# SzymonKnopp/morfem

Hardware: NVIDIA B200
Metric: reduced-sweep freq points/sec (higher is better)
Workload: dtype c128

## Files before the change

### include/morfem_b200.h

```cpp
#ifndef MORFEM_B200_H
#define MORFEM_B200_H

#include <stddef.h>
#include <stdint.h>

#ifdef __cplusplus
extern "C" {
#endif

typedef struct { double re, im; } mf_c128;

#define MF_VERSION 100
#define MF_MAX_PORTS 16

int mf_version(void);
const char* mf_last_error(void);
int64_t mf_launch_count(void);

size_t mf_gemm_tn_ws_bytes(int ra, int rb, int64_t n);
int mf_gemm_tn_c128(const mf_c128* A, int64_t lda, int ra, const mf_c128* B, int64_t ldb, int rb, int64_t n,
                    int conj_a, mf_c128* C, int64_t ldc, void* ws, size_t ws_bytes, void* stream);

int mf_gemm_nn_c128(const mf_c128* A, int64_t lda, int64_t n, int ra, const mf_c128* W, int64_t ldw, int rb,
                    mf_c128* Out, int64_t ldo, void* stream);
int mf_trmm_nn_c128(const mf_c128* A, int64_t lda, int64_t n, int r, const mf_c128* W, int64_t ldw,
                    mf_c128* Out, int64_t ldo, void* stream);

int mf_equilibrate_c128(mf_c128* G, int64_t ld, int r, double shift, double* d, double* stats, void* stream);
int mf_potrf_upper_c128(mf_c128* G, int64_t ld, int r, int* info, void* stream);
int mf_trtri_upper_c128(const mf_c128* R, int64_t ldr, int r, mf_c128* Rinv, int64_t ldi, void* stream);
size_t mf_chol_inv_ws_bytes(int r);
int mf_chol_inv_upper_c128(mf_c128* G, int64_t ldg, int r, mf_c128* Rinv, int64_t ldi, int* info,
                           void* ws, size_t ws_bytes, void* stream);
int mf_scale_cols_c128(mf_c128* X, int64_t ld, int rows, int cols, const double* d, int power, void* stream);
int mf_scale_rows_c128(mf_c128* X, int64_t ld, int rows, int cols, const double* d, int power, void* stream);
size_t mf_jacobi_svd_ws_bytes(int r);
int mf_jacobi_svd_c128(mf_c128* X, int64_t ld, int r, mf_c128* U, int64_t ldu, double* sigma, int max_sweeps,
                       double tol, int* sweeps_done, void* ws, size_t ws_bytes, void* stream);

int mf_spmm_csr_c128(const int32_t* rowptr, const int32_t* colidx, const void* vals, int val_is_real,
                     int64_t nrows, const mf_c128* Q, int64_t ldq, int r, mf_c128* Y, int64_t ldy, void* stream);
int mf_spmm_csr2_c128(const int32_t* rowptr, const int32_t* colidx, const void* vals0, const void* vals1, int val_is_real,
                      int64_t nrows, const mf_c128* Q, int64_t ldq, int r, mf_c128* Y0, int64_t ldy0, mf_c128* Y1, int64_t ldy1,
                      void* stream);
int mf_spmm_csr2_f64(const int32_t* rowptr, const int32_t* colidx, const double* vals0, const double* vals1, int64_t nrows,
                     const double* Q, int64_t ldq, int r, double* Y0, int64_t ldy0, double* Y1, int64_t ldy1, void* stream);

int mf_spmm_group_size(int r);
int mf_spmm_group_size_f64(int r);
int mf_spmm_group_count(const int32_t* rowptr, const int32_t* colidx, int64_t nrows, int G, int32_t* counts, void* stream);
int mf_spmm_group_fill(const int32_t* rowptr, const int32_t* colidx, const double* vals, int64_t nrows, int G,
                       const int64_t* ustart, int32_t* ucols, double* uvals, void* stream);
int mf_spmm_grouped_c128(const int64_t* ustart, const int32_t* ucols, const double* uvals, int64_t nrows, int G,
                         const mf_c128* Q, int64_t ldq, int r, mf_c128* Y, int64_t ldy, void* stream);

int mf_spmm_window_rows_per_block(void);
int mf_spmm_window_max_nnz_per_row(void);
int mf_spmm_window_max_rows(void);
int mf_spmm_window_c128(const int32_t* rowptr, const uint8_t* slot, const double* vals, const int32_t* wstart, const int32_t* ucol,
                        int64_t nrows, int wmax, const mf_c128* Q, int64_t ldq, int r, mf_c128* Y, int64_t ldy, void* stream);
int mf_spmm_window_f64(const int32_t* rowptr, const uint8_t* slot, const double* vals, const int32_t* wstart, const int32_t* ucol,
                       int64_t nrows, int wmax, const double* Q, int64_t ldq, int r, double* Y, int64_t ldy, void* stream);

int mf_project_rhs_c128(const int32_t* colptr, const int32_t* rowidx, const void* vals, int val_is_real, int m,
                        const mf_c128* Q, int64_t ldq, int r, int64_t row0, int64_t nlocal, int conj_q,
                        mf_c128* Br, int64_t ldb, void* stream);

size_t mf_gemm_tn_f64_ws_bytes(int ra, int rb, int64_t n);
int mf_gemm_tn_f64(const double* A, int64_t lda, int ra, const double* B, int64_t ldb, int rb, int64_t n,
                   double* C, int64_t ldc, void* ws, size_t ws_bytes, void* stream);
int mf_gemm_nn_f64(const double* A, int64_t lda, int64_t n, int ra, const double* W, int64_t ldw, int rb,
                   double* Out, int64_t ldo, void* stream);
int mf_trmm_nn_f64(const double* A, int64_t lda, int64_t n, int r, const double* W, int64_t ldw,
                   double* Out, int64_t ldo, void* stream);
int mf_spmm_csr_f64(const int32_t* rowptr, const int32_t* colidx, const double* vals, int64_t nrows,
                    const double* Q, int64_t ldq, int r, double* Y, int64_t ldy, void* stream);
int mf_spmm_grouped_f64(const int64_t* ustart, const int32_t* ucols, const double* uvals, int64_t nrows, int G,
                        const double* Q, int64_t ldq, int r, double* Y, int64_t ldy, void* stream);
int mf_sweep_f64_supported(int r, int m);
int mf_sweep_f64_variant_supported(int r, int m, int variant);
size_t mf_sweep_f64_ws_bytes(int r, int m, int64_t F, int variant);
int mf_sweep_lu_gsm_f64(const double* A0, const double* A1, const double* A2, int64_t lda, const double* Br, int64_t ldb, int r, int m,
                        const double* c0, const double* c1, const double* c2, const double* cb, const double* zscale, int64_t F,
                        double* X, mf_c128* S, int* info, int variant, void* ws, size_t ws_bytes, void* stream);
int mf_jacobi_svd_f64_supported(int r);
int mf_jacobi_svd_f64(const double* X, int64_t ld, int r, double* U, int64_t ldu, double* sigma, int max_sweeps,
                      double tol, int* sweeps_done, void* stream);
int mf_project_rhs_f64(const int32_t* colptr, const int32_t* rowidx, const double* vals, int m,
                       const double* Q, int64_t ldq, int r, int64_t row0, int64_t nlocal, double* Br, int64_t ldb, void* stream);

int mf_symmetrize_c128(const mf_c128* A, int64_t lda, int r, mf_c128* As, int64_t lds, void* stream);

size_t mf_sweep_ws_bytes(int r, int m, int64_t F, int variant);
int mf_sweep_variant_supported(int r, int m, int variant);
int mf_sweep_lu_gsm_c128(const mf_c128* A0, const mf_c128* A1, const mf_c128* A2, int64_t lda,
                         const mf_c128* Br, int64_t ldb, int r, int m,
                         const double* c0, const double* c1, const double* c2, const double* cb,
                         const double* zscale, int64_t F,
                         mf_c128* X, mf_c128* S, int* info, int variant,
                         void* ws, size_t ws_bytes, void* stream);

int mf_gsm_c128(const mf_c128* X, const mf_c128* Bmat, int64_t ldb, int r, int m, const double* cb,
                const double* zscale, int64_t F, mf_c128* S, void* stream);

int mf_estimator_c128(const mf_c128* X, int r, int m, int64_t F, const mf_c128* const* G_host,
                      const mf_c128* const* H_host, const mf_c128* BB,
                      const double* c0, const double* c1, const double* c2, const double* cb,
                      double* err, void* stream);

int mf_peak_dmma_tflops(int iters, double* tflops_host, void* stream);

#ifdef __cplusplus
}
#endif
#endif
```

### morfem_b200/_ffi.py

```python
from __future__ import annotations

import ctypes
import os
from ctypes import c_char_p, c_double, c_int, c_int64, c_size_t, c_void_p

_HERE = os.path.dirname(os.path.abspath(__file__))
LIB_PATH = os.path.join(_HERE, "libmorfem_b200.so")


class MorfemB200Error(RuntimeError):
    """A C-ABI call returned a non-zero status."""


SIGNATURES = {
    "mf_version": (c_int, []),
    "mf_last_error": (c_char_p, []),
    "mf_launch_count": (c_int64, []),
    "mf_gemm_tn_ws_bytes": (c_size_t, [c_int, c_int, c_int64]),
    "mf_gemm_tn_c128": (c_int, [c_void_p, c_int64, c_int, c_void_p, c_int64, c_int, c_int64, c_int, c_void_p, c_int64,
                                c_void_p, c_size_t, c_void_p]),
    "mf_gemm_nn_c128": (c_int, [c_void_p, c_int64, c_int64, c_int, c_void_p, c_int64, c_int, c_void_p, c_int64, c_void_p]),
    "mf_trmm_nn_c128": (c_int, [c_void_p, c_int64, c_int64, c_int, c_void_p, c_int64, c_void_p, c_int64, c_void_p]),
    "mf_trmm_nn_f64": (c_int, [c_void_p, c_int64, c_int64, c_int, c_void_p, c_int64, c_void_p, c_int64, c_void_p]),
    "mf_equilibrate_c128": (c_int, [c_void_p, c_int64, c_int, c_double, c_void_p, c_void_p, c_void_p]),
    "mf_potrf_upper_c128": (c_int, [c_void_p, c_int64, c_int, c_void_p, c_void_p]),
    "mf_trtri_upper_c128": (c_int, [c_void_p, c_int64, c_int, c_void_p, c_int64, c_void_p]),
    "mf_chol_inv_ws_bytes": (c_size_t, [c_int]),
    "mf_chol_inv_upper_c128": (c_int, [c_void_p, c_int64, c_int, c_void_p, c_int64, c_void_p, c_void_p, c_size_t, c_void_p]),
    "mf_scale_cols_c128": (c_int, [c_void_p, c_int64, c_int, c_int, c_void_p, c_int, c_void_p]),
    "mf_scale_rows_c128": (c_int, [c_void_p, c_int64, c_int, c_int, c_void_p, c_int, c_void_p]),
    "mf_jacobi_svd_ws_bytes": (c_size_t, [c_int]),
    "mf_jacobi_svd_c128": (c_int, [c_void_p, c_int64, c_int, c_void_p, c_int64, c_void_p, c_int, c_double, c_void_p,
                                   c_void_p, c_size_t, c_void_p]),
    "mf_spmm_csr_c128": (c_int, [c_void_p, c_void_p, c_void_p, c_int, c_int64, c_void_p, c_int64, c_int, c_void_p, c_int64,
                                 c_void_p]),
    "mf_spmm_csr2_c128": (c_int, [c_void_p, c_void_p, c_void_p, c_void_p, c_int, c_int64, c_void_p, c_int64, c_int, c_void_p, c_int64,
                                  c_void_p, c_int64, c_void_p]),
    "mf_spmm_csr2_f64": (c_int, [c_void_p, c_void_p, c_void_p, c_void_p, c_int64, c_void_p, c_int64, c_int, c_void_p, c_int64,
                                 c_void_p, c_int64, c_void_p]),
    "mf_spmm_group_size": (c_int, [c_int]),
    "mf_spmm_group_size_f64": (c_int, [c_int]),
    "mf_spmm_group_count": (c_int, [c_void_p, c_void_p, c_int64, c_int, c_void_p, c_void_p]),
    "mf_spmm_group_fill": (c_int, [c_void_p, c_void_p, c_void_p, c_int64, c_int, c_void_p, c_void_p, c_void_p, c_void_p]),
    "mf_spmm_grouped_c128": (c_int, [c_void_p, c_void_p, c_void_p, c_int64, c_int, c_void_p, c_int64, c_int, c_void_p, c_int64,
                                     c_void_p]),
    "mf_spmm_window_rows_per_block": (c_int, []),
    "mf_spmm_window_max_nnz_per_row": (c_int, []),
    "mf_spmm_window_max_rows": (c_int, []),
    "mf_spmm_window_c128": (c_int, [c_void_p, c_void_p, c_void_p, c_void_p, c_void_p, c_int64, c_int, c_void_p, c_int64, c_int, c_void_p, c_int64,
                                    c_void_p]),
    "mf_spmm_window_f64": (c_int, [c_void_p, c_void_p, c_void_p, c_void_p, c_void_p, c_int64, c_int, c_void_p, c_int64, c_int, c_void_p, c_int64,
                                   c_void_p]),
    "mf_project_rhs_c128": (c_int, [c_void_p, c_void_p, c_void_p, c_int, c_int, c_void_p, c_int64, c_int, c_int64, c_int64,
                                    c_int, c_void_p, c_int64, c_void_p]),
    "mf_gemm_tn_f64_ws_bytes": (c_size_t, [c_int, c_int, c_int64]),
    "mf_gemm_tn_f64": (c_int, [c_void_p, c_int64, c_int, c_void_p, c_int64, c_int, c_int64, c_void_p, c_int64, c_void_p, c_size_t, c_void_p]),
    "mf_gemm_nn_f64": (c_int, [c_void_p, c_int64, c_int64, c_int, c_void_p, c_int64, c_int, c_void_p, c_int64, c_void_p]),
    "mf_spmm_csr_f64": (c_int, [c_void_p, c_void_p, c_void_p, c_int64, c_void_p, c_int64, c_int, c_void_p, c_int64, c_void_p]),
    "mf_spmm_grouped_f64": (c_int, [c_void_p, c_void_p, c_void_p, c_int64, c_int, c_void_p, c_int64, c_int, c_void_p, c_int64, c_void_p]),
    "mf_sweep_f64_supported": (c_int, [c_int, c_int]),
    "mf_sweep_f64_variant_supported": (c_int, [c_int, c_int, c_int]),
    "mf_sweep_f64_ws_bytes": (c_size_t, [c_int, c_int, c_int64, c_int]),
    "mf_sweep_lu_gsm_f64": (c_int, [c_void_p, c_void_p, c_void_p, c_int64, c_void_p, c_int64, c_int, c_int,
                                    c_void_p, c_void_p, c_void_p, c_void_p, c_void_p, c_int64, c_void_p, c_void_p, c_void_p,
                                    c_int, c_void_p, c_size_t, c_void_p]),
    "mf_jacobi_svd_f64_supported": (c_int, [c_int]),
    "mf_jacobi_svd_f64": (c_int, [c_void_p, c_int64, c_int, c_void_p, c_int64, c_void_p, c_int, c_double, c_void_p, c_void_p]),
    "mf_project_rhs_f64": (c_int, [c_void_p, c_void_p, c_void_p, c_int, c_void_p, c_int64, c_int, c_int64, c_int64, c_void_p, c_int64,
                                   c_void_p]),
    "mf_symmetrize_c128": (c_int, [c_void_p, c_int64, c_int, c_void_p, c_int64, c_void_p]),
    "mf_sweep_ws_bytes": (c_size_t, [c_int, c_int, c_int64, c_int]),
    "mf_sweep_variant_supported": (c_int, [c_int, c_int, c_int]),
    "mf_sweep_lu_gsm_c128": (c_int, [c_void_p, c_void_p, c_void_p, c_int64, c_void_p, c_int64, c_int, c_int,
                                     c_void_p, c_void_p, c_void_p, c_void_p, c_void_p, c_int64,
                                     c_void_p, c_void_p, c_void_p, c_int, c_void_p, c_size_t, c_void_p]),
    "mf_gsm_c128": (c_int, [c_void_p, c_void_p, c_int64, c_int, c_int, c_void_p, c_void_p, c_int64, c_void_p, c_void_p]),
    "mf_peak_dmma_tflops": (c_int, [c_int, c_void_p, c_void_p]),
    "mf_estimator_c128": (c_int, [c_void_p, c_int, c_int, c_int64, c_void_p, c_void_p, c_void_p, c_void_p,
                                  c_void_p, c_void_p, c_void_p, c_void_p, c_void_p]),
}

_lib = None


def load() -> ctypes.CDLL:
    global _lib
    if _lib is not None:
        return _lib
    if not os.path.exists(LIB_PATH):
        raise MorfemB200Error(
            f"{LIB_PATH} not found: build it with `python -c 'import __graft_entry__ as g; g.build()'` "
            "(or `make -C morfem_b200/csrc`).  morfem_b200 has no CPU fallback.")
    lib = ctypes.CDLL(LIB_PATH)
    for name, (restype, argtypes) in SIGNATURES.items():
        fn = getattr(lib, name)
        fn.restype = restype
        fn.argtypes = argtypes
    _lib = lib
    return lib


def check(status: int, what: str = "") -> None:
    if status != 0:
        msg = load().mf_last_error()
        raise MorfemB200Error(f"{what or 'morfem_b200 call'} failed with status {status}: "
                              f"{msg.decode(errors='replace') if msg else ''}")


def launch_count() -> int:
    return int(load().mf_launch_count())
```

### morfem_b200/csrc/dense_gemm.cu

```cuda
#include "common.cuh"

namespace {

constexpr int KC = 16;
constexpr int STAGES = 3;

constexpr int TN_TI = 64, TN_TJ = 64, TN_THREADS = 128;
constexpr int TN_LDA = TN_TI + 2, TN_LDB = TN_TJ + 2;
constexpr int TN_STAGE_ELEMS = KC * (TN_LDA + TN_LDB);

__global__ void __launch_bounds__(TN_THREADS, 2)
gemm_tn_kernel(const cplx* __restrict__ A, long long lda, int ra, const cplx* __restrict__ B, long long ldb, int rb,
               long long n, long long rows_per_split, int conj_a, cplx* __restrict__ part, int herm) {
    extern __shared__ __align__(16) cplx smem[];
    const int tid = threadIdx.x, lane = tid & 31, warp = tid >> 5;
    const int g = lane >> 2, t = lane & 3;
    const int wi = warp >> 1, wj = warp & 1;
    const int ntj = (rb + TN_TJ - 1) / TN_TJ;
    const int ti = blockIdx.x / ntj, tj = blockIdx.x - ti * ntj;
    if (herm && ti > tj) return;
    const int i0 = ti * TN_TI, j0 = tj * TN_TJ;
    const long long n0 = (long long)blockIdx.y * rows_per_split;
    long long n1 = n0 + rows_per_split; if (n1 > n) n1 = n;
    const int nchunks = n1 > n0 ? (int)((n1 - n0 + KC - 1) / KC) : 0;

    auto load_stage = [&](int stage, int chunk) {
        cplx* As = smem + stage * TN_STAGE_ELEMS;
        cplx* Bs = As + KC * TN_LDA;
        const long long row_base = n0 + (long long)chunk * KC;
#pragma unroll
        for (int q = 0; q < (KC * TN_TI) / TN_THREADS; ++q) {
            int idx = tid + q * TN_THREADS;
            int rr = idx / TN_TI, cc = idx - rr * TN_TI;
            long long row = row_base + rr;
            bool ok = row < n1 && (i0 + cc) < ra;
            const cplx* src = A + (ok ? row * lda + i0 + cc : 0);
            cp_async16(As + rr * TN_LDA + cc, src, ok);
        }
#pragma unroll
        for (int q = 0; q < (KC * TN_TJ) / TN_THREADS; ++q) {
            int idx = tid + q * TN_THREADS;
            int rr = idx / TN_TJ, cc = idx - rr * TN_TJ;
            long long row = row_base + rr;
            bool ok = row < n1 && (j0 + cc) < rb;
            const cplx* src = B + (ok ? row * ldb + j0 + cc : 0);
            cp_async16(Bs + rr * TN_LDB + cc, src, ok);
        }
    };

    double cre[4][4][2], cim[4][4][2];
#pragma unroll
    for (int i = 0; i < 4; ++i)
#pragma unroll
        for (int j = 0; j < 4; ++j) { cre[i][j][0] = cre[i][j][1] = 0.0; cim[i][j][0] = cim[i][j][1] = 0.0; }

    for (int s = 0; s < STAGES - 1; ++s) { if (s < nchunks) load_stage(s, s); cp_async_commit(); }
    const double sgn = conj_a ? -1.0 : 1.0;
    for (int c = 0; c < nchunks; ++c) {
        cp_async_wait<STAGES - 2>();
        __syncthreads();
        { int nc = c + STAGES - 1; if (nc < nchunks) load_stage(nc % STAGES, nc); cp_async_commit(); }
        const cplx* As = smem + (c % STAGES) * TN_STAGE_ELEMS;
        const cplx* Bs = As + KC * TN_LDA;
#pragma unroll
        for (int kk = 0; kk < KC / 4; ++kk) {
            cplx a[4], b[4];
#pragma unroll
            for (int i = 0; i < 4; ++i) { a[i] = As[(kk * 4 + t) * TN_LDA + wi * 32 + i * 8 + g]; a[i].y *= sgn; }
#pragma unroll
            for (int j = 0; j < 4; ++j) b[j] = Bs[(kk * 4 + t) * TN_LDB + wj * 32 + j * 8 + g];
#pragma unroll
            for (int i = 0; i < 4; ++i)
#pragma unroll
                for (int j = 0; j < 4; ++j) {
                    dmma884(cre[i][j][0], cre[i][j][1], a[i].x, b[j].x);
                    dmma884(cre[i][j][0], cre[i][j][1], -a[i].y, b[j].y);
                    dmma884(cim[i][j][0], cim[i][j][1], a[i].x, b[j].y);
                    dmma884(cim[i][j][0], cim[i][j][1], a[i].y, b[j].x);
                }
        }
    }
    cp_async_wait<0>();
    cplx* out = part + (long long)blockIdx.y * ra * rb;
#pragma unroll
    for (int i = 0; i < 4; ++i)
#pragma unroll
        for (int j = 0; j < 4; ++j) {
            int row = i0 + wi * 32 + i * 8 + g;
            int col = j0 + wj * 32 + j * 8 + 2 * t;
            if (row < ra) {
                if (col < rb) out[(long long)row * rb + col] = cmake(cre[i][j][0], cim[i][j][0]);
                if (col + 1 < rb) out[(long long)row * rb + col + 1] = cmake(cre[i][j][1], cim[i][j][1]);
            }
        }
}

constexpr int RED_WARPS = 8;
__global__ void __launch_bounds__(RED_WARPS * 32)
reduce_partials_kernel(const cplx* __restrict__ part, int nsplit, int ra, int rb, cplx* __restrict__ C, long long ldc, int herm) {
    __shared__ cplx red[RED_WARPS][32];
    const int lane = threadIdx.x & 31, warp = threadIdx.x >> 5;
    const long long total = (long long)ra * rb;
    const long long oidx = (long long)blockIdx.x * 32 + lane;
    long long idx = oidx;
    bool mirror = false;
    if (herm && oidx < total) {
        const int i = (int)(oidx / rb), j = (int)(oidx - (long long)i * rb);
        if (i / TN_TI > j / TN_TJ) { idx = (long long)j * rb + i; mirror = true; }
    }
    cplx acc0 = cmake(0.0, 0.0), acc1 = cmake(0.0, 0.0);
    if (idx < total) {
        int s = warp;
        for (; s + RED_WARPS < nsplit; s += 2 * RED_WARPS) {
            const cplx v0 = part[(long long)s * total + idx], v1 = part[(long long)(s + RED_WARPS) * total + idx];
            acc0 = cadd(acc0, v0); acc1 = cadd(acc1, v1);
        }
        if (s < nsplit) acc0 = cadd(acc0, part[(long long)s * total + idx]);
    }
    red[warp][lane] = cadd(acc0, acc1);
    __syncthreads();
    if (warp == 0 && oidx < total) {
        cplx acc = red[0][lane];
#pragma unroll
        for (int w = 1; w < RED_WARPS; ++w) acc = cadd(acc, red[w][lane]);
        if (mirror) acc.y = -acc.y;
        const int i = (int)(oidx / rb), j = (int)(oidx - (long long)i * rb);
        C[i * ldc + j] = acc;
    }
}

void tn_plan(int ra, int rb, long long n, int& tiles, int& nsplit, long long& rows_per_split, bool symm = false) {
    tiles = ((ra + TN_TI - 1) / TN_TI) * ((rb + TN_TJ - 1) / TN_TJ);
    const int nt = (ra + TN_TI - 1) / TN_TI;
    const int work_tiles = symm ? nt * (nt + 1) / 2 : tiles;
    const int target = 148 * 2 * 2;
    long long max_split = (n + (long long)KC * 8 - 1) / ((long long)KC * 8);
    if (max_split < 1) max_split = 1;
    long long s = target / work_tiles; if (s < 1) s = 1; if (s > max_split) s = max_split;
    rows_per_split = (n + s - 1) / s;
    rows_per_split = (rows_per_split + KC - 1) / KC * KC;
    if (rows_per_split < KC) rows_per_split = KC;
    nsplit = (int)((n + rows_per_split - 1) / rows_per_split); if (nsplit < 1) nsplit = 1;
}

constexpr int NN_TM = 128, NN_TN = 64, NN_THREADS = 256;
constexpr int NN_LDA = KC + 4;
constexpr int NN_LDW = NN_TN + 2;
constexpr int NN_STAGE_ELEMS = NN_TM * NN_LDA + KC * NN_LDW;

__global__ void __launch_bounds__(NN_THREADS, 1)
gemm_nn_kernel(const cplx* __restrict__ A, long long lda, long long n, int ra, const cplx* __restrict__ W, long long ldw, int rb,
               cplx* __restrict__ Out, long long ldo, int w_upper) {
    extern __shared__ __align__(16) cplx smem[];
    const int tid = threadIdx.x, lane = tid & 31, warp = tid >> 5;
    const int g = lane >> 2, t = lane & 3;
    const int wm = warp >> 1, wn = warp & 1;
    const int ntn = (rb + NN_TN - 1) / NN_TN;
    const long long tm = blockIdx.x / ntn; const int tn = (int)(blockIdx.x - tm * ntn);
    const long long m0 = tm * NN_TM; const int j0 = tn * NN_TN;
    const int kmax = (w_upper && j0 + NN_TN < ra) ? j0 + NN_TN : ra;
    const int nchunks = (kmax + KC - 1) / KC;

    auto load_stage = [&](int stage, int chunk) {
        cplx* As = smem + stage * NN_STAGE_ELEMS;
        cplx* Ws = As + NN_TM * NN_LDA;
        const int k0 = chunk * KC;
#pragma unroll
        for (int q = 0; q < (NN_TM * KC) / NN_THREADS; ++q) {
            int idx = tid + q * NN_THREADS;
            int rr = idx / KC, cc = idx - rr * KC;
            bool ok = (m0 + rr) < n && (k0 + cc) < ra;
            const cplx* src = A + (ok ? (m0 + rr) * lda + k0 + cc : 0);
            cp_async16(As + rr * NN_LDA + cc, src, ok);
        }
#pragma unroll
        for (int q = 0; q < (KC * NN_TN) / NN_THREADS; ++q) {
            int idx = tid + q * NN_THREADS;
            int rr = idx / NN_TN, cc = idx - rr * NN_TN;
            bool ok = (k0 + rr) < ra && (j0 + cc) < rb;
            const cplx* src = W + (ok ? (long long)(k0 + rr) * ldw + j0 + cc : 0);
            cp_async16(Ws + rr * NN_LDW + cc, src, ok);
        }
    };

    double cre[4][4][2], cim[4][4][2];
#pragma unroll
    for (int i = 0; i < 4; ++i)
#pragma unroll
        for (int j = 0; j < 4; ++j) { cre[i][j][0] = cre[i][j][1] = 0.0; cim[i][j][0] = cim[i][j][1] = 0.0; }

    for (int s = 0; s < STAGES - 1; ++s) { if (s < nchunks) load_stage(s, s); cp_async_commit(); }
    for (int c = 0; c < nchunks; ++c) {
        cp_async_wait<STAGES - 2>();
        __syncthreads();
        { int nc = c + STAGES - 1; if (nc < nchunks) load_stage(nc % STAGES, nc); cp_async_commit(); }
        const cplx* As = smem + (c % STAGES) * NN_STAGE_ELEMS;
        const cplx* Ws = As + NN_TM * NN_LDA;
#pragma unroll
        for (int kk = 0; kk < KC / 4; ++kk) {
            cplx a[4], b[4];
#pragma unroll
            for (int i = 0; i < 4; ++i) a[i] = As[(wm * 32 + i * 8 + g) * NN_LDA + kk * 4 + t];
#pragma unroll
            for (int j = 0; j < 4; ++j) b[j] = Ws[(kk * 4 + t) * NN_LDW + wn * 32 + j * 8 + g];
#pragma unroll
            for (int i = 0; i < 4; ++i)
#pragma unroll
                for (int j = 0; j < 4; ++j) {
                    dmma884(cre[i][j][0], cre[i][j][1], a[i].x, b[j].x);
                    dmma884(cre[i][j][0], cre[i][j][1], -a[i].y, b[j].y);
                    dmma884(cim[i][j][0], cim[i][j][1], a[i].x, b[j].y);
                    dmma884(cim[i][j][0], cim[i][j][1], a[i].y, b[j].x);
                }
        }
    }
    cp_async_wait<0>();
#pragma unroll
    for (int i = 0; i < 4; ++i)
#pragma unroll
        for (int j = 0; j < 4; ++j) {
            long long row = m0 + wm * 32 + i * 8 + g;
            int col = j0 + wn * 32 + j * 8 + 2 * t;
            if (row < n) {
                if (col + 1 < rb) {
                    double4 v = make_double4(cre[i][j][0], cim[i][j][0], cre[i][j][1], cim[i][j][1]);
                    cplx* dst = Out + row * ldo + col;
                    if ((reinterpret_cast<uintptr_t>(dst) & 31) == 0) *reinterpret_cast<double4*>(dst) = v;
                    else { dst[0] = cmake(v.x, v.y); dst[1] = cmake(v.z, v.w); }
                } else if (col < rb) {
                    Out[row * ldo + col] = cmake(cre[i][j][0], cim[i][j][0]);
                }
            }
        }
}

}

extern "C" size_t mf_gemm_tn_ws_bytes(int ra, int rb, int64_t n) {
    if (ra <= 0 || rb <= 0 || n <= 0) return 16;
    int tiles, nsplit, nsplit2 = 0; long long rps;
    tn_plan(ra, rb, n, tiles, nsplit, rps);
    if (ra == rb) tn_plan(ra, rb, n, tiles, nsplit2, rps, true);
    return sizeof(cplx) * (size_t)(nsplit > nsplit2 ? nsplit : nsplit2) * ra * rb;
}

extern "C" int mf_gemm_tn_c128(const mf_c128* A, int64_t lda, int ra, const mf_c128* B, int64_t ldb, int rb, int64_t n,
                               int conj_a, mf_c128* C, int64_t ldc, void* ws, size_t ws_bytes, void* stream) {
    if (!A) MF_FAIL_ARG(1, "A is NULL");
    if (ra <= 0 || lda < ra) MF_FAIL_ARG(3, "need 0 < ra <= lda");
    if (!B) MF_FAIL_ARG(4, "B is NULL");
    if (rb <= 0 || ldb < rb) MF_FAIL_ARG(6, "need 0 < rb <= ldb");
    if (n < 0) MF_FAIL_ARG(7, "n < 0");
    if (!C || ldc < rb) MF_FAIL_ARG(9, "C is NULL or ldc < rb");
    if (!ws || ws_bytes < mf_gemm_tn_ws_bytes(ra, rb, n)) MF_FAIL_ARG(11, "workspace too small (mf_gemm_tn_ws_bytes)");
    cudaStream_t st = (cudaStream_t)stream;
    int tiles, nsplit; long long rps;
    const int herm = (conj_a && (const void*)A == (const void*)B && lda == ldb && ra == rb) ? 1 : 0;
    tn_plan(ra, rb, n > 0 ? n : 1, tiles, nsplit, rps, herm != 0);
    const size_t smem = sizeof(cplx) * STAGES * TN_STAGE_ELEMS;
    MF_CHECK_CUDA(cudaFuncSetAttribute(gemm_tn_kernel, cudaFuncAttributeMaxDynamicSharedMemorySize, (int)smem));
    dim3 grid(tiles, nsplit);
    gemm_tn_kernel<<<grid, TN_THREADS, smem, st>>>((const cplx*)A, lda, ra, (const cplx*)B, ldb, rb, n, rps, conj_a, (cplx*)ws, herm);
    MF_CHECK_LAUNCH();
    long long total = (long long)ra * rb;
    reduce_partials_kernel<<<(unsigned)((total + 31) / 32), RED_WARPS * 32, 0, st>>>((const cplx*)ws, nsplit, ra, rb, (cplx*)C, ldc, herm);
    MF_CHECK_LAUNCH();
    return 0;
}

static int gemm_nn_c128_impl(const mf_c128* A, int64_t lda, int64_t n, int ra, const mf_c128* W, int64_t ldw, int rb,
                            mf_c128* Out, int64_t ldo, void* stream, int w_upper) {
    if (!A) MF_FAIL_ARG(1, "A is NULL");
    if (ra <= 0 || lda < ra) MF_FAIL_ARG(4, "need 0 < ra <= lda");
    if (n < 0) MF_FAIL_ARG(3, "n < 0");
    if (!W || ldw < rb) MF_FAIL_ARG(5, "W is NULL or ldw < rb");
    if (rb <= 0) MF_FAIL_ARG(7, "rb <= 0");
    if (!Out || ldo < rb) MF_FAIL_ARG(8, "Out is NULL or ldo < rb");
    if ((const void*)Out == (const void*)A) MF_FAIL_ARG(8, "Out must not alias A");
    if (n == 0) return 0;
    cudaStream_t st = (cudaStream_t)stream;
    const size_t smem = sizeof(cplx) * STAGES * NN_STAGE_ELEMS;
    MF_CHECK_CUDA(cudaFuncSetAttribute(gemm_nn_kernel, cudaFuncAttributeMaxDynamicSharedMemorySize, (int)smem));
    long long tiles_m = (n + NN_TM - 1) / NN_TM;
    int tiles_n = (rb + NN_TN - 1) / NN_TN;
    long long grid = tiles_m * tiles_n;
    if (grid > 0x7fffffffLL) MF_FAIL_ARG(3, "n too large for one launch");
    gemm_nn_kernel<<<(unsigned)grid, NN_THREADS, smem, st>>>((const cplx*)A, lda, n, ra, (const cplx*)W, ldw, rb, (cplx*)Out, ldo, w_upper);
    MF_CHECK_LAUNCH();
    return 0;
}

extern "C" int mf_gemm_nn_c128(const mf_c128* A, int64_t lda, int64_t n, int ra, const mf_c128* W, int64_t ldw, int rb,
                               mf_c128* Out, int64_t ldo, void* stream) {
    return gemm_nn_c128_impl(A, lda, n, ra, W, ldw, rb, Out, ldo, stream, 0);
}

extern "C" int mf_trmm_nn_c128(const mf_c128* A, int64_t lda, int64_t n, int r, const mf_c128* W, int64_t ldw,
                               mf_c128* Out, int64_t ldo, void* stream) {
    return gemm_nn_c128_impl(A, lda, n, r, W, ldw, r, Out, ldo, stream, 1);
}
```

### morfem_b200/csrc/dense_gemm_f64.cu

```cuda
#include "common.cuh"

namespace {

constexpr int KC = 16;
constexpr int STAGES = 3;

constexpr int TN_TI = 64, TN_TJ = 64, TN_THREADS = 128;
constexpr int TN_LDA = TN_TI + 8, TN_LDB = TN_TJ + 8;
constexpr int TN_STAGE_ELEMS = KC * (TN_LDA + TN_LDB);

__device__ __forceinline__ void cp_async8(void* smem_dst, const void* gmem_src, bool valid) {
    unsigned s = (unsigned)__cvta_generic_to_shared(smem_dst);
    int bytes = valid ? 8 : 0;
    asm volatile("cp.async.ca.shared.global [%0], [%1], 8, %2;\n" :: "r"(s), "l"(gmem_src), "r"(bytes));
}

__global__ void __launch_bounds__(TN_THREADS, 2)
gemm_tn_f64_kernel(const double* __restrict__ A, long long lda, int ra, const double* __restrict__ B, long long ldb, int rb,
                   long long n, long long rows_per_split, double* __restrict__ part, int vec_ok, int symm) {
    extern __shared__ __align__(16) double smem_d[];
    const int tid = threadIdx.x, lane = tid & 31, warp = tid >> 5;
    const int g = lane >> 2, t = lane & 3;
    const int wi = warp >> 1, wj = warp & 1;
    const int ntj = (rb + TN_TJ - 1) / TN_TJ;
    const int ti = blockIdx.x / ntj, tj = blockIdx.x - ti * ntj;
    if (symm && ti > tj) return;
    const int i0 = ti * TN_TI, j0 = tj * TN_TJ;
    const long long n0 = (long long)blockIdx.y * rows_per_split;
    long long n1 = n0 + rows_per_split; if (n1 > n) n1 = n;
    const int nchunks = n1 > n0 ? (int)((n1 - n0 + KC - 1) / KC) : 0;

    auto load_stage = [&](int stage, int chunk) {
        double* As = smem_d + stage * TN_STAGE_ELEMS;
        double* Bs = As + KC * TN_LDA;
        const long long row_base = n0 + (long long)chunk * KC;
        if (vec_ok) {
#pragma unroll
            for (int q = 0; q < (KC * TN_TI / 2) / TN_THREADS; ++q) {
                const int idx = tid + q * TN_THREADS;
                const int rr = idx / (TN_TI / 2), cc = 2 * (idx - rr * (TN_TI / 2));
                const long long row = row_base + rr;
                const bool ok = row < n1 && (i0 + cc) < ra;
                cp_async16(As + rr * TN_LDA + cc, A + (ok ? row * lda + i0 + cc : 0), ok);
            }
#pragma unroll
            for (int q = 0; q < (KC * TN_TJ / 2) / TN_THREADS; ++q) {
                const int idx = tid + q * TN_THREADS;
                const int rr = idx / (TN_TJ / 2), cc = 2 * (idx - rr * (TN_TJ / 2));
                const long long row = row_base + rr;
                const bool ok = row < n1 && (j0 + cc) < rb;
                cp_async16(Bs + rr * TN_LDB + cc, B + (ok ? row * ldb + j0 + cc : 0), ok);
            }
        } else {
#pragma unroll
            for (int q = 0; q < (KC * TN_TI) / TN_THREADS; ++q) {
                const int idx = tid + q * TN_THREADS;
                const int rr = idx / TN_TI, cc = idx - rr * TN_TI;
                const long long row = row_base + rr;
                const bool ok = row < n1 && (i0 + cc) < ra;
                cp_async8(As + rr * TN_LDA + cc, A + (ok ? row * lda + i0 + cc : 0), ok);
            }
#pragma unroll
            for (int q = 0; q < (KC * TN_TJ) / TN_THREADS; ++q) {
                const int idx = tid + q * TN_THREADS;
                const int rr = idx / TN_TJ, cc = idx - rr * TN_TJ;
                const long long row = row_base + rr;
                const bool ok = row < n1 && (j0 + cc) < rb;
                cp_async8(Bs + rr * TN_LDB + cc, B + (ok ? row * ldb + j0 + cc : 0), ok);
            }
        }
    };

    double c[4][4][2];
#pragma unroll
    for (int i = 0; i < 4; ++i)
#pragma unroll
        for (int j = 0; j < 4; ++j) { c[i][j][0] = 0.0; c[i][j][1] = 0.0; }

    for (int s = 0; s < STAGES - 1; ++s) { if (s < nchunks) load_stage(s, s); cp_async_commit(); }
    for (int ch = 0; ch < nchunks; ++ch) {
        cp_async_wait<STAGES - 2>();
        __syncthreads();
        { const int nc = ch + STAGES - 1; if (nc < nchunks) load_stage(nc % STAGES, nc); cp_async_commit(); }
        const double* As = smem_d + (ch % STAGES) * TN_STAGE_ELEMS;
        const double* Bs = As + KC * TN_LDA;
#pragma unroll
        for (int kk = 0; kk < KC / 4; ++kk) {
            double a[4], b[4];
#pragma unroll
            for (int i = 0; i < 4; ++i) a[i] = As[(kk * 4 + t) * TN_LDA + wi * 32 + i * 8 + g];
#pragma unroll
            for (int j = 0; j < 4; ++j) b[j] = Bs[(kk * 4 + t) * TN_LDB + wj * 32 + j * 8 + g];
#pragma unroll
            for (int i = 0; i < 4; ++i)
#pragma unroll
                for (int j = 0; j < 4; ++j) dmma884(c[i][j][0], c[i][j][1], a[i], b[j]);
        }
    }
    cp_async_wait<0>();
    double* out = part + (long long)blockIdx.y * ra * rb;
#pragma unroll
    for (int i = 0; i < 4; ++i)
#pragma unroll
        for (int j = 0; j < 4; ++j) {
            const int row = i0 + wi * 32 + i * 8 + g;
            const int col = j0 + wj * 32 + j * 8 + 2 * t;
            if (row < ra) {
                if (col < rb) out[(long long)row * rb + col] = c[i][j][0];
                if (col + 1 < rb) out[(long long)row * rb + col + 1] = c[i][j][1];
            }
        }
}

constexpr int RED_WARPS = 8;
__global__ void __launch_bounds__(RED_WARPS * 32)
reduce_partials_f64_kernel(const double* __restrict__ part, int nsplit, int ra, int rb, double* __restrict__ C, long long ldc, int symm) {
    __shared__ double red[RED_WARPS][32];
    const int lane = threadIdx.x & 31, warp = threadIdx.x >> 5;
    const long long total = (long long)ra * rb;
    const long long oidx = (long long)blockIdx.x * 32 + lane;
    long long idx = oidx;
    if (symm && oidx < total) {
        const int i = (int)(oidx / rb), j = (int)(oidx - (long long)i * rb);
        if (i / TN_TI > j / TN_TJ) idx = (long long)j * rb + i;
    }
    double acc0 = 0.0, acc1 = 0.0;
    if (idx < total) {
        int s = warp;
        for (; s + RED_WARPS < nsplit; s += 2 * RED_WARPS) { acc0 += part[(long long)s * total + idx]; acc1 += part[(long long)(s + RED_WARPS) * total + idx]; }
        if (s < nsplit) acc0 += part[(long long)s * total + idx];
    }
    red[warp][lane] = acc0 + acc1;
    __syncthreads();
    if (warp == 0 && oidx < total) {
        double acc = red[0][lane];
#pragma unroll
        for (int w = 1; w < RED_WARPS; ++w) acc += red[w][lane];
        const int i = (int)(oidx / rb), j = (int)(oidx - (long long)i * rb);
        C[i * ldc + j] = acc;
    }
}

void tn_plan(int ra, int rb, long long n, int& tiles, int& nsplit, long long& rows_per_split, bool symm = false) {
    tiles = ((ra + TN_TI - 1) / TN_TI) * ((rb + TN_TJ - 1) / TN_TJ);
    const int nt = (ra + TN_TI - 1) / TN_TI;
    const int work_tiles = symm ? nt * (nt + 1) / 2 : tiles;
    const int target = 148 * 2 * 2;
    long long max_split = (n + (long long)KC * 8 - 1) / ((long long)KC * 8);
    if (max_split < 1) max_split = 1;
    long long s = target / work_tiles; if (s < 1) s = 1; if (s > max_split) s = max_split;
    rows_per_split = (n + s - 1) / s;
    rows_per_split = (rows_per_split + KC - 1) / KC * KC;
    if (rows_per_split < KC) rows_per_split = KC;
    nsplit = (int)((n + rows_per_split - 1) / rows_per_split); if (nsplit < 1) nsplit = 1;
}

constexpr int NN_TM = 128, NN_TN = 64, NN_THREADS = 256;
constexpr int NN_LDA = KC + 4;
constexpr int NN_LDW = NN_TN + 8;
constexpr int NN_STAGE_ELEMS = NN_TM * NN_LDA + KC * NN_LDW;

__global__ void __launch_bounds__(NN_THREADS, 2)
gemm_nn_f64_kernel(const double* __restrict__ A, long long lda, long long n, int ra, const double* __restrict__ W, long long ldw, int rb,
                   double* __restrict__ Out, long long ldo, int w_upper) {
    extern __shared__ __align__(16) double smem_d[];
    const int tid = threadIdx.x, lane = tid & 31, warp = tid >> 5;
    const int g = lane >> 2, t = lane & 3;
    const int wm = warp >> 1, wn = warp & 1;
    const int ntn = (rb + NN_TN - 1) / NN_TN;
    const long long tm = blockIdx.x / ntn; const int tn = (int)(blockIdx.x - tm * ntn);
    const long long m0 = tm * NN_TM; const int j0 = tn * NN_TN;
    const int kmax = (w_upper && j0 + NN_TN < ra) ? j0 + NN_TN : ra;
    const int nchunks = (kmax + KC - 1) / KC;

    auto load_stage = [&](int stage, int chunk) {
        double* As = smem_d + stage * NN_STAGE_ELEMS;
        double* Ws = As + NN_TM * NN_LDA;
        const int k0 = chunk * KC;
#pragma unroll
        for (int q = 0; q < (NN_TM * KC) / NN_THREADS; ++q) {
            const int idx = tid + q * NN_THREADS;
            const int rr = idx / KC, cc = idx - rr * KC;
            const bool ok = (m0 + rr) < n && (k0 + cc) < ra;
            cp_async8(As + rr * NN_LDA + cc, A + (ok ? (m0 + rr) * lda + k0 + cc : 0), ok);
        }
#pragma unroll
        for (int q = 0; q < (KC * NN_TN) / NN_THREADS; ++q) {
            const int idx = tid + q * NN_THREADS;
            const int rr = idx / NN_TN, cc = idx - rr * NN_TN;
            const bool ok = (k0 + rr) < ra && (j0 + cc) < rb;
            cp_async8(Ws + rr * NN_LDW + cc, W + (ok ? (long long)(k0 + rr) * ldw + j0 + cc : 0), ok);
        }
    };

    double c[4][4][2];
#pragma unroll
    for (int i = 0; i < 4; ++i)
#pragma unroll
        for (int j = 0; j < 4; ++j) { c[i][j][0] = 0.0; c[i][j][1] = 0.0; }

    for (int s = 0; s < STAGES - 1; ++s) { if (s < nchunks) load_stage(s, s); cp_async_commit(); }
    for (int ch = 0; ch < nchunks; ++ch) {
        cp_async_wait<STAGES - 2>();
        __syncthreads();
        { const int nc = ch + STAGES - 1; if (nc < nchunks) load_stage(nc % STAGES, nc); cp_async_commit(); }
        const double* As = smem_d + (ch % STAGES) * NN_STAGE_ELEMS;
        const double* Ws = As + NN_TM * NN_LDA;
#pragma unroll
        for (int kk = 0; kk < KC / 4; ++kk) {
            double a[4], b[4];
#pragma unroll
            for (int i = 0; i < 4; ++i) a[i] = As[(wm * 32 + i * 8 + g) * NN_LDA + kk * 4 + t];
#pragma unroll
            for (int j = 0; j < 4; ++j) b[j] = Ws[(kk * 4 + t) * NN_LDW + wn * 32 + j * 8 + g];
#pragma unroll
            for (int i = 0; i < 4; ++i)
#pragma unroll
                for (int j = 0; j < 4; ++j) dmma884(c[i][j][0], c[i][j][1], a[i], b[j]);
        }
    }
    cp_async_wait<0>();
#pragma unroll
    for (int i = 0; i < 4; ++i)
#pragma unroll
        for (int j = 0; j < 4; ++j) {
            const long long row = m0 + wm * 32 + i * 8 + g;
            const int col = j0 + wn * 32 + j * 8 + 2 * t;
            if (row < n) {
                double* dst = Out + row * ldo + col;
                if (col + 1 < rb && (reinterpret_cast<uintptr_t>(dst) & 15) == 0) *reinterpret_cast<double2*>(dst) = make_double2(c[i][j][0], c[i][j][1]);
                else { if (col < rb) dst[0] = c[i][j][0]; if (col + 1 < rb) dst[1] = c[i][j][1]; }
            }
        }
}

}

extern "C" size_t mf_gemm_tn_f64_ws_bytes(int ra, int rb, int64_t n) {
    if (ra <= 0 || rb <= 0 || n <= 0) return 16;
    int tiles, nsplit, nsplit2 = 0; long long rps;
    tn_plan(ra, rb, n, tiles, nsplit, rps);
    if (ra == rb) tn_plan(ra, rb, n, tiles, nsplit2, rps, true);
    return sizeof(double) * (size_t)(nsplit > nsplit2 ? nsplit : nsplit2) * ra * rb;
}

extern "C" int mf_gemm_tn_f64(const double* A, int64_t lda, int ra, const double* B, int64_t ldb, int rb, int64_t n,
                              double* C, int64_t ldc, void* ws, size_t ws_bytes, void* stream) {
    if (!A) MF_FAIL_ARG(1, "A is NULL");
    if (ra <= 0 || lda < ra) MF_FAIL_ARG(3, "need 0 < ra <= lda");
    if (!B) MF_FAIL_ARG(4, "B is NULL");
    if (rb <= 0 || ldb < rb) MF_FAIL_ARG(6, "need 0 < rb <= ldb");
    if (n < 0) MF_FAIL_ARG(7, "n < 0");
    if (!C || ldc < rb) MF_FAIL_ARG(8, "C is NULL or ldc < rb");
    if (!ws || ws_bytes < mf_gemm_tn_f64_ws_bytes(ra, rb, n)) MF_FAIL_ARG(10, "workspace too small (mf_gemm_tn_f64_ws_bytes)");
    cudaStream_t st = (cudaStream_t)stream;
    int tiles, nsplit; long long rps;
    const int symm = (A == B && lda == ldb && ra == rb) ? 1 : 0;
    tn_plan(ra, rb, n > 0 ? n : 1, tiles, nsplit, rps, symm != 0);
    const size_t smem = sizeof(double) * STAGES * TN_STAGE_ELEMS;
    MF_CHECK_CUDA(cudaFuncSetAttribute(gemm_tn_f64_kernel, cudaFuncAttributeMaxDynamicSharedMemorySize, (int)smem));
    const int vec_ok = ((reinterpret_cast<uintptr_t>(A) | reinterpret_cast<uintptr_t>(B)) & 15) == 0 && (lda % 2) == 0 && (ldb % 2) == 0 &&
                       (ra % 2) == 0 && (rb % 2) == 0;
    dim3 grid(tiles, nsplit);
    gemm_tn_f64_kernel<<<grid, TN_THREADS, smem, st>>>(A, lda, ra, B, ldb, rb, n, rps, (double*)ws, vec_ok, symm);
    MF_CHECK_LAUNCH();
    const long long total = (long long)ra * rb;
    reduce_partials_f64_kernel<<<(unsigned)((total + 31) / 32), RED_WARPS * 32, 0, st>>>((const double*)ws, nsplit, ra, rb, C, ldc, symm);
    MF_CHECK_LAUNCH();
    return 0;
}

static int gemm_nn_f64_impl(const double* A, int64_t lda, int64_t n, int ra, const double* W, int64_t ldw, int rb,
                           double* Out, int64_t ldo, void* stream, int w_upper) {
    if (!A) MF_FAIL_ARG(1, "A is NULL");
    if (ra <= 0 || lda < ra) MF_FAIL_ARG(4, "need 0 < ra <= lda");
    if (n < 0) MF_FAIL_ARG(3, "n < 0");
    if (!W || ldw < rb) MF_FAIL_ARG(5, "W is NULL or ldw < rb");
    if (rb <= 0) MF_FAIL_ARG(7, "rb <= 0");
    if (!Out || ldo < rb) MF_FAIL_ARG(8, "Out is NULL or ldo < rb");
    if ((const void*)Out == (const void*)A) MF_FAIL_ARG(8, "Out must not alias A");
    if (n == 0) return 0;
    cudaStream_t st = (cudaStream_t)stream;
    const size_t smem = sizeof(double) * STAGES * NN_STAGE_ELEMS;
    MF_CHECK_CUDA(cudaFuncSetAttribute(gemm_nn_f64_kernel, cudaFuncAttributeMaxDynamicSharedMemorySize, (int)smem));
    const long long tiles_m = (n + NN_TM - 1) / NN_TM;
    const int tiles_n = (rb + NN_TN - 1) / NN_TN;
    const long long grid = tiles_m * tiles_n;
    if (grid > 0x7fffffffLL) MF_FAIL_ARG(3, "n too large for one launch");
    gemm_nn_f64_kernel<<<(unsigned)grid, NN_THREADS, smem, st>>>(A, lda, n, ra, W, ldw, rb, Out, ldo, w_upper);
    MF_CHECK_LAUNCH();
    return 0;
}

extern "C" int mf_gemm_nn_f64(const double* A, int64_t lda, int64_t n, int ra, const double* W, int64_t ldw, int rb,
                              double* Out, int64_t ldo, void* stream) {
    return gemm_nn_f64_impl(A, lda, n, ra, W, ldw, rb, Out, ldo, stream, 0);
}

extern "C" int mf_trmm_nn_f64(const double* A, int64_t lda, int64_t n, int r, const double* W, int64_t ldw,
                              double* Out, int64_t ldo, void* stream) {
    return gemm_nn_f64_impl(A, lda, n, r, W, ldw, r, Out, ldo, stream, 1);
}
```

### morfem_b200/csrc/sparse.cu

```cuda
#include <stdlib.h>
#include "common.cuh"

namespace {

__device__ __forceinline__ cplx ldg_q(const cplx* p) {
    return __ldg(reinterpret_cast<const double2*>(p));
}

template <int CPL, bool REAL>
__global__ void __launch_bounds__(256)
spmm_csr_kernel(const int* __restrict__ rowptr, const int* __restrict__ colidx, const void* __restrict__ vals_v,
                long long nrows, const cplx* __restrict__ Q, long long ldq, int r, cplx* __restrict__ Y, long long ldy) {
    const long long row = ((long long)blockIdx.x * blockDim.x + threadIdx.x) >> 5;
    const int lane = threadIdx.x & 31;
    if (row >= nrows) return;
    const int s = rowptr[row], e = rowptr[row + 1];
    cplx acc[CPL];
#pragma unroll
    for (int c = 0; c < CPL; ++c) acc[c] = cmake(0.0, 0.0);
    for (int base = s; base < e; base += 32) {
        const int cnt = min(32, e - base);
        int my_col = 0; cplx my_val = cmake(0.0, 0.0);
        if (lane < cnt) {
            my_col = colidx[base + lane];
            if (REAL) my_val = cmake(reinterpret_cast<const double*>(vals_v)[base + lane], 0.0);
            else my_val = reinterpret_cast<const cplx*>(vals_v)[base + lane];
        }
        for (int k = 0; k < cnt; ++k) {
            const int col = __shfl_sync(0xffffffffu, my_col, k);
            cplx v;
            v.x = __shfl_sync(0xffffffffu, my_val.x, k);
            if (!REAL) v.y = __shfl_sync(0xffffffffu, my_val.y, k); else v.y = 0.0;
            const cplx* q = Q + (long long)col * ldq;
            cplx qv[CPL];
#pragma unroll
            for (int c = 0; c < CPL; ++c) { int idx = lane + 32 * c; qv[c] = idx < r ? ldg_q(q + idx) : cmake(0.0, 0.0); }
#pragma unroll
            for (int c = 0; c < CPL; ++c) {
                if (REAL) { acc[c].x = fma(v.x, qv[c].x, acc[c].x); acc[c].y = fma(v.x, qv[c].y, acc[c].y); }
                else cfma(acc[c], v, qv[c]);
            }
        }
    }
    cplx* y = Y + row * ldy;
#pragma unroll
    for (int c = 0; c < CPL; ++c) { int idx = lane + 32 * c; if (idx < r) y[idx] = acc[c]; }
}

template <bool REAL>
int spmm_dispatch(const int* rowptr, const int* colidx, const void* vals, long long nrows, const cplx* Q, long long ldq, int r,
                  cplx* Y, long long ldy, cudaStream_t st) {
    const int threads = 256;
    const long long warps = nrows;
    const long long blocks = (warps * 32 + threads - 1) / threads;
    if (blocks > 0x7fffffffLL) return -5;
#define SPMM_LAUNCH(C) spmm_csr_kernel<C, REAL><<<(unsigned)blocks, threads, 0, st>>>(rowptr, colidx, vals, nrows, Q, ldq, r, Y, ldy)
    if (r <= 32) SPMM_LAUNCH(1);
    else if (r <= 64) SPMM_LAUNCH(2);
    else if (r <= 128) SPMM_LAUNCH(4);
    else if (r <= 256) SPMM_LAUNCH(8);
    else if (r <= 512) SPMM_LAUNCH(16);
    else return -9;
#undef SPMM_LAUNCH
    return 0;
}

template <int CPL, bool REAL>
__global__ void __launch_bounds__(256)
spmm_csr2_kernel(const int* __restrict__ rowptr, const int* __restrict__ colidx, const void* __restrict__ vals0_v,
                 const void* __restrict__ vals1_v, long long nrows, const cplx* __restrict__ Q, long long ldq, int r,
                 cplx* __restrict__ Y0, long long ldy0, cplx* __restrict__ Y1, long long ldy1) {
    const long long row = ((long long)blockIdx.x * blockDim.x + threadIdx.x) >> 5;
    const int lane = threadIdx.x & 31;
    if (row >= nrows) return;
    const int s = rowptr[row], e = rowptr[row + 1];
    cplx acc0[CPL], acc1[CPL];
#pragma unroll
    for (int c = 0; c < CPL; ++c) { acc0[c] = cmake(0.0, 0.0); acc1[c] = cmake(0.0, 0.0); }
    for (int base = s; base < e; base += 32) {
        const int cnt = min(32, e - base);
        int my_col = 0; cplx my_v0 = cmake(0.0, 0.0), my_v1 = cmake(0.0, 0.0);
        if (lane < cnt) {
            my_col = colidx[base + lane];
            if (REAL) {
                my_v0 = cmake(reinterpret_cast<const double*>(vals0_v)[base + lane], 0.0);
                my_v1 = cmake(reinterpret_cast<const double*>(vals1_v)[base + lane], 0.0);
            } else {
                my_v0 = reinterpret_cast<const cplx*>(vals0_v)[base + lane];
                my_v1 = reinterpret_cast<const cplx*>(vals1_v)[base + lane];
            }
        }
#pragma unroll 2
        for (int k = 0; k < cnt; ++k) {
            const int col = __shfl_sync(0xffffffffu, my_col, k);
            cplx v0, v1;
            v0.x = __shfl_sync(0xffffffffu, my_v0.x, k); v1.x = __shfl_sync(0xffffffffu, my_v1.x, k);
            if (!REAL) { v0.y = __shfl_sync(0xffffffffu, my_v0.y, k); v1.y = __shfl_sync(0xffffffffu, my_v1.y, k); }
            else { v0.y = 0.0; v1.y = 0.0; }
            const cplx* q = Q + (long long)col * ldq;
            cplx qv[CPL];
#pragma unroll
            for (int c = 0; c < CPL; ++c) { const int idx = lane + 32 * c; qv[c] = idx < r ? ldg_q(q + idx) : cmake(0.0, 0.0); }
#pragma unroll
            for (int c = 0; c < CPL; ++c) {
                if (REAL) {
                    acc0[c].x = fma(v0.x, qv[c].x, acc0[c].x); acc0[c].y = fma(v0.x, qv[c].y, acc0[c].y);
                    acc1[c].x = fma(v1.x, qv[c].x, acc1[c].x); acc1[c].y = fma(v1.x, qv[c].y, acc1[c].y);
                } else { cfma(acc0[c], v0, qv[c]); cfma(acc1[c], v1, qv[c]); }
            }
        }
    }
    cplx* y0 = Y0 + row * ldy0; cplx* y1 = Y1 + row * ldy1;
#pragma unroll
    for (int c = 0; c < CPL; ++c) { const int idx = lane + 32 * c; if (idx < r) { y0[idx] = acc0[c]; y1[idx] = acc1[c]; } }
}

template <int CPL>
__global__ void __launch_bounds__(256)
spmm_csr2_f64_kernel(const int* __restrict__ rowptr, const int* __restrict__ colidx, const double* __restrict__ vals0,
                     const double* __restrict__ vals1, long long nrows, const double* __restrict__ Q, long long ldq, int r,
                     double* __restrict__ Y0, long long ldy0, double* __restrict__ Y1, long long ldy1) {
    const long long row = ((long long)blockIdx.x * blockDim.x + threadIdx.x) >> 5;
    const int lane = threadIdx.x & 31;
    if (row >= nrows) return;
    const int s = rowptr[row], e = rowptr[row + 1];
    double acc0[CPL], acc1[CPL];
#pragma unroll
    for (int c = 0; c < CPL; ++c) { acc0[c] = 0.0; acc1[c] = 0.0; }
    for (int base = s; base < e; base += 32) {
        const int cnt = min(32, e - base);
        int my_col = 0; double my_v0 = 0.0, my_v1 = 0.0;
        if (lane < cnt) { my_col = colidx[base + lane]; my_v0 = vals0[base + lane]; my_v1 = vals1[base + lane]; }
#pragma unroll 4
        for (int k = 0; k < cnt; ++k) {
            const int col = __shfl_sync(0xffffffffu, my_col, k);
            const double v0 = __shfl_sync(0xffffffffu, my_v0, k), v1 = __shfl_sync(0xffffffffu, my_v1, k);
            const double* q = Q + (long long)col * ldq;
#pragma unroll
            for (int c = 0; c < CPL; ++c) {
                const int idx = lane + 32 * c;
                if (idx < r) { const double qv = __ldg(q + idx); acc0[c] = fma(v0, qv, acc0[c]); acc1[c] = fma(v1, qv, acc1[c]); }
            }
        }
    }
    double* y0 = Y0 + row * ldy0; double* y1 = Y1 + row * ldy1;
#pragma unroll
    for (int c = 0; c < CPL; ++c) { const int idx = lane + 32 * c; if (idx < r) { y0[idx] = acc0[c]; y1[idx] = acc1[c]; } }
}


template <int G>
__device__ __forceinline__ int group_merge(const int* __restrict__ rowptr, const int* __restrict__ colidx, const double* __restrict__ vals,
                                           long long nrows, long long g, long long out0, int* __restrict__ ucols, double* __restrict__ uvals) {
    int p[G], e[G];
#pragma unroll
    for (int i = 0; i < G; ++i) {
        const long long row = g * G + i;
        p[i] = row < nrows ? rowptr[row] : 0;
        e[i] = row < nrows ? rowptr[row + 1] : 0;
    }
    int n = 0;
    while (true) {
        int c = 0x7fffffff;
#pragma unroll
        for (int i = 0; i < G; ++i) if (p[i] < e[i]) c = min(c, colidx[p[i]]);
        if (c == 0x7fffffff) break;
#pragma unroll
        for (int i = 0; i < G; ++i) {
            double v = 0.0;
            if (p[i] < e[i] && colidx[p[i]] == c) { if (uvals) v = vals[p[i]]; ++p[i]; }
            if (uvals) uvals[(out0 + n) * G + i] = v;
        }
        if (ucols) ucols[out0 + n] = c;
        ++n;
    }
    return n;
}

template <int G>
__global__ void spmm_group_count_kernel(const int* __restrict__ rowptr, const int* __restrict__ colidx, long long nrows, long long ngroups,
                                        int* __restrict__ counts) {
    const long long g = (long long)blockIdx.x * blockDim.x + threadIdx.x;
    if (g < ngroups) counts[g] = group_merge<G>(rowptr, colidx, nullptr, nrows, g, 0, nullptr, nullptr);
}

template <int G>
__global__ void spmm_group_fill_kernel(const int* __restrict__ rowptr, const int* __restrict__ colidx, const double* __restrict__ vals,
                                       long long nrows, long long ngroups, const long long* __restrict__ ustart, int* __restrict__ ucols,
                                       double* __restrict__ uvals) {
    const long long g = (long long)blockIdx.x * blockDim.x + threadIdx.x;
    if (g < ngroups) group_merge<G>(rowptr, colidx, vals, nrows, g, ustart[g], ucols, uvals);
}

template <int G, int CPL>
__global__ void __launch_bounds__(256)
spmm_grouped_kernel(const long long* __restrict__ ustart, const int* __restrict__ ucols, const double* __restrict__ uvals, long long nrows,
                    const cplx* __restrict__ Q, long long ldq, int r, cplx* __restrict__ Y, long long ldy) {
    const long long g = ((long long)blockIdx.x * blockDim.x + threadIdx.x) >> 5;
    const int lane = threadIdx.x & 31;
    Q += (long long)blockIdx.y * 32 * CPL; Y += (long long)blockIdx.y * 32 * CPL; r -= (int)blockIdx.y * 32 * CPL;
    __shared__ __align__(16) double cstage[8][32 * G];
    double* cw = cstage[(threadIdx.x >> 5) & 7];
    if (g * G >= nrows) return;
    const long long s = ustart[g], e = ustart[g + 1];
    cplx acc[G][CPL];
#pragma unroll
    for (int i = 0; i < G; ++i)
#pragma unroll
        for (int c = 0; c < CPL; ++c) acc[i][c] = cmake(0.0, 0.0);
    for (long long base = s; base < e; base += 32) {
        const int cnt = (int)min((long long)32, e - base);
        int my_col = 0;
        if (lane < cnt) {
            my_col = ucols[base + lane];
            const double2* src = reinterpret_cast<const double2*>(uvals + (base + lane) * G);
            double2* dst = reinterpret_cast<double2*>(cw + lane * G);
            dst[0] = src[0];
            if (G == 4) dst[1] = src[1];
        }
        __syncwarp();
#pragma unroll 4
        for (int k = 0; k < cnt; ++k) {
            const int col = __shfl_sync(0xffffffffu, my_col, k);
            const cplx* q = Q + (long long)col * ldq;
            cplx qv[CPL];
#pragma unroll
            for (int c = 0; c < CPL; ++c) { const int idx = lane + 32 * c; qv[c] = idx < r ? ldg_q(q + idx) : cmake(0.0, 0.0); }
            double v[G];
            {
                const double2* vp = reinterpret_cast<const double2*>(cw + k * G);
                const double2 t0 = vp[0];
                v[0] = t0.x; v[1] = t0.y;
                if (G == 4) { const double2 t1 = vp[1]; v[G > 2 ? 2 : 0] = t1.x; v[G > 3 ? 3 : 0] = t1.y; }
            }
#pragma unroll
            for (int i = 0; i < G; ++i) {
                if (v[i] != 0.0) {
#pragma unroll
                    for (int c = 0; c < CPL; ++c) { acc[i][c].x = fma(v[i], qv[c].x, acc[i][c].x); acc[i][c].y = fma(v[i], qv[c].y, acc[i][c].y); }
                }
            }
        }
        __syncwarp();
    }
#pragma unroll
    for (int i = 0; i < G; ++i) {
        const long long row = g * G + i;
        if (row < nrows) {
            cplx* y = Y + row * ldy;
#pragma unroll
            for (int c = 0; c < CPL; ++c) { const int idx = lane + 32 * c; if (idx < r) y[idx] = acc[i][c]; }
        }
    }
}

template <bool REAL>
__global__ void project_rhs_kernel(const int* __restrict__ colptr, const int* __restrict__ rowidx, const void* __restrict__ vals_v,
                                   const cplx* __restrict__ Q, long long ldq, int r, long long row0, long long nlocal, int conj_q,
                                   cplx* __restrict__ Br, long long ldb) {
    const int col = blockIdx.x;
    const int s = colptr[col], e = colptr[col + 1];
    for (int i = threadIdx.x; i < r; i += blockDim.x) {
        cplx acc = cmake(0.0, 0.0);
        for (int p = s; p < e; ++p) {
            long long row = rowidx[p];
            if (row < row0 || row >= row0 + nlocal) continue;
            cplx v = REAL ? cmake(reinterpret_cast<const double*>(vals_v)[p], 0.0) : reinterpret_cast<const cplx*>(vals_v)[p];
            cplx q = Q[(row - row0) * ldq + i];
            if (conj_q) q.y = -q.y;
            cfma(acc, q, v);
        }
        Br[i * ldb + col] = acc;
    }
}


template <int CPL>
__global__ void __launch_bounds__(256)
spmm_csr_f64_kernel(const int* __restrict__ rowptr, const int* __restrict__ colidx, const double* __restrict__ vals,
                    long long nrows, const double* __restrict__ Q, long long ldq, int r, double* __restrict__ Y, long long ldy) {
    const long long row = ((long long)blockIdx.x * blockDim.x + threadIdx.x) >> 5;
    const int lane = threadIdx.x & 31;
    if (row >= nrows) return;
    const int s = rowptr[row], e = rowptr[row + 1];
    double acc[CPL];
#pragma unroll
    for (int c = 0; c < CPL; ++c) acc[c] = 0.0;
    for (int base = s; base < e; base += 32) {
        const int cnt = min(32, e - base);
        int my_col = 0; double my_val = 0.0;
        if (lane < cnt) { my_col = colidx[base + lane]; my_val = vals[base + lane]; }
#pragma unroll 4
        for (int k = 0; k < cnt; ++k) {
            const int col = __shfl_sync(0xffffffffu, my_col, k);
            const double v = __shfl_sync(0xffffffffu, my_val, k);
            const double* q = Q + (long long)col * ldq;
#pragma unroll
            for (int c = 0; c < CPL; ++c) { const int idx = lane + 32 * c; if (idx < r) acc[c] = fma(v, __ldg(q + idx), acc[c]); }
        }
    }
    double* y = Y + row * ldy;
#pragma unroll
    for (int c = 0; c < CPL; ++c) { const int idx = lane + 32 * c; if (idx < r) y[idx] = acc[c]; }
}

template <int G, int CPL>
__global__ void __launch_bounds__(256)
spmm_grouped_f64_kernel(const long long* __restrict__ ustart, const int* __restrict__ ucols, const double* __restrict__ uvals, long long nrows,
                        const double* __restrict__ Q, long long ldq, int r, double* __restrict__ Y, long long ldy) {
    const long long g = ((long long)blockIdx.x * blockDim.x + threadIdx.x) >> 5;
    const int lane = threadIdx.x & 31;
    Q += (long long)blockIdx.y * 32 * CPL; Y += (long long)blockIdx.y * 32 * CPL; r -= (int)blockIdx.y * 32 * CPL;
    __shared__ __align__(16) double cstage[8][32 * G];
    double* cw = cstage[(threadIdx.x >> 5) & 7];
    if (g * G >= nrows) return;
    const long long s = ustart[g], e = ustart[g + 1];
    double acc[G][CPL];
#pragma unroll
    for (int i = 0; i < G; ++i)
#pragma unroll
        for (int c = 0; c < CPL; ++c) acc[i][c] = 0.0;
    for (long long base = s; base < e; base += 32) {
        const int cnt = (int)min((long long)32, e - base);
        int my_col = 0;
        if (lane < cnt) {
            my_col = ucols[base + lane];
            const double2* src = reinterpret_cast<const double2*>(uvals + (base + lane) * G);
            double2* dst = reinterpret_cast<double2*>(cw + lane * G);
            dst[0] = src[0];
            if (G == 4) dst[1] = src[1];
        }
        __syncwarp();
#pragma unroll 4
        for (int k = 0; k < cnt; ++k) {
            const int col = __shfl_sync(0xffffffffu, my_col, k);
            const double* q = Q + (long long)col * ldq;
            double qv[CPL];
#pragma unroll
            for (int c = 0; c < CPL; ++c) { const int idx = lane + 32 * c; qv[c] = idx < r ? __ldg(q + idx) : 0.0; }
            double v[G];
            {
                const double2* vp = reinterpret_cast<const double2*>(cw + k * G);
                const double2 t0 = vp[0];
                v[0] = t0.x; v[1] = t0.y;
                if (G == 4) { const double2 t1 = vp[1]; v[G > 2 ? 2 : 0] = t1.x; v[G > 3 ? 3 : 0] = t1.y; }
            }
#pragma unroll
            for (int i = 0; i < G; ++i) {
                if (v[i] != 0.0) {
#pragma unroll
                    for (int c = 0; c < CPL; ++c) acc[i][c] = fma(v[i], qv[c], acc[i][c]);
                }
            }
        }
        __syncwarp();
    }
#pragma unroll
    for (int i = 0; i < G; ++i) {
        const long long row = g * G + i;
        if (row < nrows) {
            double* y = Y + row * ldy;
#pragma unroll
            for (int c = 0; c < CPL; ++c) { const int idx = lane + 32 * c; if (idx < r) y[idx] = acc[i][c]; }
        }
    }
}

__global__ void project_rhs_f64_kernel(const int* __restrict__ colptr, const int* __restrict__ rowidx, const double* __restrict__ vals,
                                       const double* __restrict__ Q, long long ldq, int r, long long row0, long long nlocal,
                                       double* __restrict__ Br, long long ldb) {
    const int col = blockIdx.x;
    const int s = colptr[col], e = colptr[col + 1];
    for (int i = threadIdx.x; i < r; i += blockDim.x) {
        double acc = 0.0;
        for (int p = s; p < e; ++p) {
            const long long row = rowidx[p];
            if (row < row0 || row >= row0 + nlocal) continue;
            acc = fma(Q[(row - row0) * ldq + i], vals[p], acc);
        }
        Br[i * ldb + col] = acc;
    }
}

}

extern "C" int mf_spmm_csr_c128(const int32_t* rowptr, const int32_t* colidx, const void* vals, int val_is_real,
                                int64_t nrows, const mf_c128* Q, int64_t ldq, int r, mf_c128* Y, int64_t ldy, void* stream) {
    if (!rowptr) MF_FAIL_ARG(1, "rowptr is NULL");
    if (!colidx) MF_FAIL_ARG(2, "colidx is NULL");
    if (!vals) MF_FAIL_ARG(3, "vals is NULL");
    if (nrows < 0) MF_FAIL_ARG(5, "nrows < 0");
    if (!Q || ldq < r) MF_FAIL_ARG(6, "Q is NULL or ldq < r");
    if (r <= 0 || r > 512) MF_FAIL_ARG(8, "need 0 < r <= 512");
    if (!Y || ldy < r) MF_FAIL_ARG(9, "Y is NULL or ldy < r");
    if (nrows == 0) return 0;
    cudaStream_t st = (cudaStream_t)stream;
    int rc = val_is_real ? spmm_dispatch<true>(rowptr, colidx, vals, nrows, (const cplx*)Q, ldq, r, (cplx*)Y, ldy, st)
                         : spmm_dispatch<false>(rowptr, colidx, vals, nrows, (const cplx*)Q, ldq, r, (cplx*)Y, ldy, st);
    if (rc != 0) MF_FAIL_ARG(-rc, "size out of range for one launch");
    MF_CHECK_LAUNCH();
    return 0;
}

extern "C" int mf_project_rhs_c128(const int32_t* colptr, const int32_t* rowidx, const void* vals, int val_is_real, int m,
                                   const mf_c128* Q, int64_t ldq, int r, int64_t row0, int64_t nlocal, int conj_q,
                                   mf_c128* Br, int64_t ldb, void* stream) {
    if (!colptr) MF_FAIL_ARG(1, "colptr is NULL");
    if (!rowidx) MF_FAIL_ARG(2, "rowidx is NULL");
    if (!vals) MF_FAIL_ARG(3, "vals is NULL");
    if (m <= 0) MF_FAIL_ARG(5, "m <= 0");
    if (!Q || ldq < r) MF_FAIL_ARG(6, "Q is NULL or ldq < r");
    if (r <= 0) MF_FAIL_ARG(8, "r <= 0");
    if (!Br || ldb < m) MF_FAIL_ARG(12, "Br is NULL or ldb < m");
    cudaStream_t st = (cudaStream_t)stream;
    if (val_is_real) project_rhs_kernel<true><<<m, 256, 0, st>>>(colptr, rowidx, vals, (const cplx*)Q, ldq, r, row0, nlocal, conj_q, (cplx*)Br, ldb);
    else project_rhs_kernel<false><<<m, 256, 0, st>>>(colptr, rowidx, vals, (const cplx*)Q, ldq, r, row0, nlocal, conj_q, (cplx*)Br, ldb);
    MF_CHECK_LAUNCH();
    return 0;
}

extern "C" int mf_spmm_group_size(int r) { return r <= 128 ? 4 : 2; }
extern "C" int mf_spmm_group_size_f64(int r) { return r <= 256 ? 4 : 2; }

extern "C" int mf_spmm_group_count(const int32_t* rowptr, const int32_t* colidx, int64_t nrows, int G, int32_t* counts, void* stream) {
    if (!rowptr) MF_FAIL_ARG(1, "rowptr is NULL");
    if (!colidx) MF_FAIL_ARG(2, "colidx is NULL");
    if (nrows < 0) MF_FAIL_ARG(3, "nrows < 0");
    if (G != 2 && G != 4) MF_FAIL_ARG(4, "group size must be 2 or 4");
    if (!counts) MF_FAIL_ARG(5, "counts is NULL");
    if (nrows == 0) return 0;
    const long long ngroups = (nrows + G - 1) / G;
    const unsigned blocks = (unsigned)((ngroups + 127) / 128);
    if (G == 4) spmm_group_count_kernel<4><<<blocks, 128, 0, (cudaStream_t)stream>>>(rowptr, colidx, nrows, ngroups, counts);
    else spmm_group_count_kernel<2><<<blocks, 128, 0, (cudaStream_t)stream>>>(rowptr, colidx, nrows, ngroups, counts);
    MF_CHECK_LAUNCH();
    return 0;
}

extern "C" int mf_spmm_group_fill(const int32_t* rowptr, const int32_t* colidx, const double* vals, int64_t nrows, int G,
                                  const int64_t* ustart, int32_t* ucols, double* uvals, void* stream) {
    if (!rowptr) MF_FAIL_ARG(1, "rowptr is NULL");
    if (!colidx) MF_FAIL_ARG(2, "colidx is NULL");
    if (!vals) MF_FAIL_ARG(3, "vals is NULL");
    if (nrows < 0) MF_FAIL_ARG(4, "nrows < 0");
    if (G != 2 && G != 4) MF_FAIL_ARG(5, "group size must be 2 or 4");
    if (!ustart) MF_FAIL_ARG(6, "ustart is NULL");
    if (!ucols) MF_FAIL_ARG(7, "ucols is NULL");
    if (!uvals) MF_FAIL_ARG(8, "uvals is NULL");
    if (nrows == 0) return 0;
    const long long ngroups = (nrows + G - 1) / G;
    const unsigned blocks = (unsigned)((ngroups + 127) / 128);
    if (G == 4) spmm_group_fill_kernel<4><<<blocks, 128, 0, (cudaStream_t)stream>>>(rowptr, colidx, vals, nrows, ngroups, (const long long*)ustart, ucols, uvals);
    else spmm_group_fill_kernel<2><<<blocks, 128, 0, (cudaStream_t)stream>>>(rowptr, colidx, vals, nrows, ngroups, (const long long*)ustart, ucols, uvals);
    MF_CHECK_LAUNCH();
    return 0;
}

extern "C" int mf_spmm_grouped_c128(const int64_t* ustart, const int32_t* ucols, const double* uvals, int64_t nrows, int G,
                                    const mf_c128* Q, int64_t ldq, int r, mf_c128* Y, int64_t ldy, void* stream) {
    if (!ustart) MF_FAIL_ARG(1, "ustart is NULL");
    if (!ucols) MF_FAIL_ARG(2, "ucols is NULL");
    if (!uvals) MF_FAIL_ARG(3, "uvals is NULL");
    if (nrows < 0) MF_FAIL_ARG(4, "nrows < 0");
    if (r <= 0 || r > 512) MF_FAIL_ARG(8, "need 0 < r <= 512");
    if (G != mf_spmm_group_size(r)) MF_FAIL_ARG(5, "group size must equal mf_spmm_group_size(r)");
    if (!Q || ldq < r) MF_FAIL_ARG(6, "Q is NULL or ldq < r");
    if (!Y || ldy < r) MF_FAIL_ARG(9, "Y is NULL or ldy < r");
    if (nrows == 0) return 0;
    cudaStream_t st = (cudaStream_t)stream;
    const long long ngroups = (nrows + G - 1) / G;
    const long long blocks = (ngroups * 32 + 255) / 256;
    if (blocks > 0x7fffffffLL) MF_FAIL_ARG(4, "nrows too large for one launch");
#define GSPMM(GG, C, NY) spmm_grouped_kernel<GG, C><<<dim3((unsigned)blocks, NY), 256, 0, st>>>((const long long*)ustart, ucols, uvals, nrows, (const cplx*)Q, ldq, r, (cplx*)Y, ldy)
    if (r <= 32) GSPMM(4, 1, 1);
    else if (r <= 64) GSPMM(4, 2, 1);
    else if (r <= 128) GSPMM(4, 4, 1);
    else if (G == 4) GSPMM(4, 4, (r + 127) / 128);
    else if (r <= 256) GSPMM(2, 8, 1);
    else GSPMM(2, 16, 1);
#undef GSPMM
    MF_CHECK_LAUNCH();
    return 0;
}

extern "C" int mf_spmm_csr_f64(const int32_t* rowptr, const int32_t* colidx, const double* vals, int64_t nrows,
                               const double* Q, int64_t ldq, int r, double* Y, int64_t ldy, void* stream) {
    if (!rowptr) MF_FAIL_ARG(1, "rowptr is NULL");
    if (!colidx) MF_FAIL_ARG(2, "colidx is NULL");
    if (!vals) MF_FAIL_ARG(3, "vals is NULL");
    if (nrows < 0) MF_FAIL_ARG(4, "nrows < 0");
    if (!Q || ldq < r) MF_FAIL_ARG(5, "Q is NULL or ldq < r");
    if (r <= 0 || r > 512) MF_FAIL_ARG(7, "need 0 < r <= 512");
    if (!Y || ldy < r) MF_FAIL_ARG(8, "Y is NULL or ldy < r");
    if (nrows == 0) return 0;
    cudaStream_t st = (cudaStream_t)stream;
    const long long blocks = (nrows * 32 + 255) / 256;
    if (blocks > 0x7fffffffLL) MF_FAIL_ARG(4, "nrows too large for one launch");
#define RSPMM(C) spmm_csr_f64_kernel<C><<<(unsigned)blocks, 256, 0, st>>>(rowptr, colidx, vals, nrows, Q, ldq, r, Y, ldy)
    if (r <= 32) RSPMM(1); else if (r <= 64) RSPMM(2); else if (r <= 128) RSPMM(4); else if (r <= 256) RSPMM(8); else RSPMM(16);
#undef RSPMM
    MF_CHECK_LAUNCH();
    return 0;
}

extern "C" int mf_spmm_grouped_f64(const int64_t* ustart, const int32_t* ucols, const double* uvals, int64_t nrows, int G,
                                   const double* Q, int64_t ldq, int r, double* Y, int64_t ldy, void* stream) {
    if (!ustart) MF_FAIL_ARG(1, "ustart is NULL");
    if (!ucols) MF_FAIL_ARG(2, "ucols is NULL");
    if (!uvals) MF_FAIL_ARG(3, "uvals is NULL");
    if (nrows < 0) MF_FAIL_ARG(4, "nrows < 0");
    if (r <= 0 || r > 512) MF_FAIL_ARG(8, "need 0 < r <= 512");
    if (G != mf_spmm_group_size_f64(r)) MF_FAIL_ARG(5, "group size must equal mf_spmm_group_size_f64(r)");
    if (!Q || ldq < r) MF_FAIL_ARG(6, "Q is NULL or ldq < r");
    if (!Y || ldy < r) MF_FAIL_ARG(9, "Y is NULL or ldy < r");
    if (nrows == 0) return 0;
    cudaStream_t st = (cudaStream_t)stream;
    const long long ngroups = (nrows + G - 1) / G;
    const long long blocks = (ngroups * 32 + 255) / 256;
    if (blocks > 0x7fffffffLL) MF_FAIL_ARG(4, "nrows too large for one launch");
#define GRSPMM(GG, C, NY) spmm_grouped_f64_kernel<GG, C><<<dim3((unsigned)blocks, NY), 256, 0, st>>>((const long long*)ustart, ucols, uvals, nrows, Q, ldq, r, Y, ldy)
    if (r <= 32) GRSPMM(4, 1, 1); else if (r <= 64) GRSPMM(4, 2, 1); else if (r <= 128) GRSPMM(4, 4, 1);
    else if (G == 4) GRSPMM(4, 8, (r + 255) / 256);
    else if (r <= 256) GRSPMM(2, 8, 1); else GRSPMM(2, 16, 1);
#undef GRSPMM
    MF_CHECK_LAUNCH();
    return 0;
}

extern "C" int mf_project_rhs_f64(const int32_t* colptr, const int32_t* rowidx, const double* vals, int m,
                                  const double* Q, int64_t ldq, int r, int64_t row0, int64_t nlocal, double* Br, int64_t ldb, void* stream) {
    if (!colptr) MF_FAIL_ARG(1, "colptr is NULL");
    if (!rowidx) MF_FAIL_ARG(2, "rowidx is NULL");
    if (!vals) MF_FAIL_ARG(3, "vals is NULL");
    if (m <= 0) MF_FAIL_ARG(4, "m <= 0");
    if (!Q || ldq < r) MF_FAIL_ARG(5, "Q is NULL or ldq < r");
    if (r <= 0) MF_FAIL_ARG(7, "r <= 0");
    if (!Br || ldb < m) MF_FAIL_ARG(10, "Br is NULL or ldb < m");
    project_rhs_f64_kernel<<<m, 256, 0, (cudaStream_t)stream>>>(colptr, rowidx, vals, Q, ldq, r, row0, nlocal, Br, ldb);
    MF_CHECK_LAUNCH();
    return 0;
}

extern "C" int mf_spmm_csr2_c128(const int32_t* rowptr, const int32_t* colidx, const void* vals0, const void* vals1, int val_is_real,
                                 int64_t nrows, const mf_c128* Q, int64_t ldq, int r, mf_c128* Y0, int64_t ldy0, mf_c128* Y1, int64_t ldy1,
                                 void* stream) {
    if (!rowptr) MF_FAIL_ARG(1, "rowptr is NULL");
    if (!colidx) MF_FAIL_ARG(2, "colidx is NULL");
    if (!vals0) MF_FAIL_ARG(3, "vals0 is NULL");
    if (!vals1) MF_FAIL_ARG(4, "vals1 is NULL");
    if (nrows < 0) MF_FAIL_ARG(6, "nrows < 0");
    if (!Q || ldq < r) MF_FAIL_ARG(7, "Q is NULL or ldq < r");
    if (r <= 0 || r > 512) MF_FAIL_ARG(9, "need 0 < r <= 512");
    if (!Y0 || ldy0 < r) MF_FAIL_ARG(10, "Y0 is NULL or ldy0 < r");
    if (!Y1 || ldy1 < r) MF_FAIL_ARG(12, "Y1 is NULL or ldy1 < r");
    if (nrows == 0) return 0;
    cudaStream_t st = (cudaStream_t)stream;
    const long long blocks = (nrows * 32 + 255) / 256;
    if (blocks > 0x7fffffffLL) MF_FAIL_ARG(6, "nrows too large for one launch");
#define SPMM2(C, RL) spmm_csr2_kernel<C, RL><<<(unsigned)blocks, 256, 0, st>>>(rowptr, colidx, vals0, vals1, nrows, (const cplx*)Q, ldq, r, (cplx*)Y0, ldy0, (cplx*)Y1, ldy1)
#define SPMM2_R(RL) do { if (r <= 32) SPMM2(1, RL); else if (r <= 64) SPMM2(2, RL); else if (r <= 128) SPMM2(4, RL); else if (r <= 256) SPMM2(8, RL); else SPMM2(16, RL); } while (0)
    if (val_is_real) SPMM2_R(true); else SPMM2_R(false);
#undef SPMM2_R
#undef SPMM2
    MF_CHECK_LAUNCH();
    return 0;
}

extern "C" int mf_spmm_csr2_f64(const int32_t* rowptr, const int32_t* colidx, const double* vals0, const double* vals1, int64_t nrows,
                                const double* Q, int64_t ldq, int r, double* Y0, int64_t ldy0, double* Y1, int64_t ldy1, void* stream) {
    if (!rowptr) MF_FAIL_ARG(1, "rowptr is NULL");
    if (!colidx) MF_FAIL_ARG(2, "colidx is NULL");
    if (!vals0) MF_FAIL_ARG(3, "vals0 is NULL");
    if (!vals1) MF_FAIL_ARG(4, "vals1 is NULL");
    if (nrows < 0) MF_FAIL_ARG(5, "nrows < 0");
    if (!Q || ldq < r) MF_FAIL_ARG(6, "Q is NULL or ldq < r");
    if (r <= 0 || r > 512) MF_FAIL_ARG(8, "need 0 < r <= 512");
    if (!Y0 || ldy0 < r) MF_FAIL_ARG(9, "Y0 is NULL or ldy0 < r");
    if (!Y1 || ldy1 < r) MF_FAIL_ARG(11, "Y1 is NULL or ldy1 < r");
    if (nrows == 0) return 0;
    cudaStream_t st = (cudaStream_t)stream;
    const long long blocks = (nrows * 32 + 255) / 256;
    if (blocks > 0x7fffffffLL) MF_FAIL_ARG(5, "nrows too large for one launch");
#define RSPMM2(C) spmm_csr2_f64_kernel<C><<<(unsigned)blocks, 256, 0, st>>>(rowptr, colidx, vals0, vals1, nrows, Q, ldq, r, Y0, ldy0, Y1, ldy1)
    if (r <= 32) RSPMM2(1); else if (r <= 64) RSPMM2(2); else if (r <= 128) RSPMM2(4); else if (r <= 256) RSPMM2(8); else RSPMM2(16);
#undef RSPMM2
    MF_CHECK_LAUNCH();
    return 0;
}
```

### morfem_b200/device.py

```python
from __future__ import annotations

import ctypes
from dataclasses import dataclass
from typing import Optional

import numpy as np
import torch

from . import _ffi

C128 = torch.complex128


def require_cuda() -> torch.device:
    if not torch.cuda.is_available():
        raise _ffi.MorfemB200Error("morfem_b200 needs a CUDA device (sm_100a); there is no CPU fallback")
    return torch.device("cuda", torch.cuda.current_device())


def _ptr(t: Optional[torch.Tensor]):
    return None if t is None else ctypes.c_void_p(t.data_ptr())


def _stream():
    return ctypes.c_void_p(torch.cuda.current_stream().cuda_stream)


F64 = torch.float64


def _check_mat(t: torch.Tensor, name: str):
    if t.dtype not in (C128, F64) or not t.is_cuda or t.dim() != 2 or t.stride(1) != 1:
        raise ValueError(f"{name}: expected a row-major complex128 or float64 CUDA matrix, got {t.dtype} {tuple(t.shape)} strides {t.stride()}")


def _same_dtype(a: torch.Tensor, b: torch.Tensor, what: str) -> bool:
    if a.dtype != b.dtype:
        raise ValueError(f"{what}: operands must share a dtype (float64 or complex128), got {a.dtype} and {b.dtype}")
    return a.dtype == F64


def to_device_c128(a, device=None) -> torch.Tensor:
    device = device or require_cuda()
    arr = np.ascontiguousarray(np.asarray(a), dtype=np.complex128)
    return upload(arr, device)


def real_or_complex_to_device(a, device=None, widen: bool = False) -> torch.Tensor:
    device = device or require_cuda()
    if isinstance(a, torch.Tensor):
        t = a.to(device, non_blocking=True)
        if t.dtype == C128 or (t.dtype == F64 and not widen):
            return t
        return t.to(C128) if (widen or t.is_complex()) else t.to(F64)
    arr = np.asarray(a)
    if np.iscomplexobj(arr):
        return to_device_c128(arr, device)
    t = upload(np.ascontiguousarray(arr, dtype=np.float64), device)
    return t.to(C128) if widen else t


class _Workspaces:

    def __init__(self):
        self._bufs = {}
        self._pinned = set()
        self._retired = []

    def get(self, key: str, nbytes: int, device) -> torch.Tensor:
        k = (key, str(device))
        buf = self._bufs.get(k)
        if buf is None or buf.numel() < nbytes:
            if buf is not None and k in self._pinned:
                self._retired.append(buf)
                self._pinned.discard(k)
            buf = torch.empty(max(int(nbytes), 256), dtype=torch.uint8, device=device)
            self._bufs[k] = buf
        return buf

    def pin_all(self):
        self._pinned.update(self._bufs.keys())

    def clear(self):
        self._bufs.clear()
        self._pinned.clear()
        self._retired.clear()


workspaces = _Workspaces()


class KernelTimer:

    def __init__(self):
        self.records = []

    def summary(self):
        torch.cuda.synchronize()
        agg = {}
        for name, e0, e1, nbytes, flops in self.records:
            a = agg.setdefault(name, {"calls": 0, "ms": 0.0, "bytes": 0.0, "flops": 0.0})
            a["calls"] += 1
            a["ms"] += e0.elapsed_time(e1)
            a["bytes"] += nbytes
            a["flops"] += flops
        return agg


timer: Optional[KernelTimer] = None


class _timed:
    def __init__(self, name, nbytes=0.0, flops=0.0):
        self.name, self.nbytes, self.flops = name, float(nbytes), float(flops)

    def __enter__(self):
        if timer is not None:
            self.e0 = torch.cuda.Event(enable_timing=True)
            self.e0.record()
        return self

    def __exit__(self, *exc):
        if timer is not None and exc[0] is None:
            e1 = torch.cuda.Event(enable_timing=True)
            e1.record()
            timer.records.append((self.name, self.e0, e1, self.nbytes, self.flops))
        return False


def gemm_tn(a: torch.Tensor, b: torch.Tensor, conj: bool = False, out: Optional[torch.Tensor] = None) -> torch.Tensor:
    lib = _ffi.load()
    _check_mat(a, "a"); _check_mat(b, "b")
    real = _same_dtype(a, b, "gemm_tn")
    n, ra = a.shape
    rb = b.shape[1]
    if b.shape[0] != n:
        raise ValueError("gemm_tn: row counts differ")
    if out is None:
        out = torch.empty((ra, rb), dtype=a.dtype, device=a.device)
    same = a.data_ptr() == b.data_ptr() and ra == rb
    if real:
        nbytes = lib.mf_gemm_tn_f64_ws_bytes(ra, rb, n)
        ws = workspaces.get("gemm_tn", nbytes, a.device)
        with _timed("gemm_tn", nbytes=8.0 * n * (ra if same else ra + rb) + 8.0 * ra * rb, flops=2.0 * n * ra * rb):
            _ffi.check(lib.mf_gemm_tn_f64(_ptr(a), a.stride(0), ra, _ptr(b), b.stride(0), rb, n, _ptr(out), out.stride(0),
                                          _ptr(ws), ws.numel(), _stream()), "mf_gemm_tn_f64")
        return out
    nbytes = lib.mf_gemm_tn_ws_bytes(ra, rb, n)
    ws = workspaces.get("gemm_tn", nbytes, a.device)
    with _timed("gemm_tn", nbytes=16.0 * n * (ra if same else ra + rb) + 16.0 * ra * rb, flops=8.0 * n * ra * rb):
        _ffi.check(lib.mf_gemm_tn_c128(_ptr(a), a.stride(0), ra, _ptr(b), b.stride(0), rb, n, int(conj), _ptr(out), out.stride(0),
                                       _ptr(ws), ws.numel(), _stream()), "mf_gemm_tn_c128")
    return out


def gemm_nn(a: torch.Tensor, w: torch.Tensor, out: Optional[torch.Tensor] = None, w_upper: bool = False) -> torch.Tensor:
    lib = _ffi.load()
    _check_mat(a, "a"); _check_mat(w, "w")
    real = _same_dtype(a, w, "gemm_nn")
    n, ra = a.shape
    if w.shape[0] != ra:
        raise ValueError("gemm_nn: inner dimensions differ")
    rb = w.shape[1]
    if out is None:
        out = torch.empty((n, rb), dtype=a.dtype, device=a.device)
    if w_upper:
        if rb != ra:
            raise ValueError("gemm_nn: w_upper needs a square w")
        tiles = (ra + 63) // 64
        frac = (tiles + 1) / (2.0 * tiles)
        if real:
            with _timed("gemm_nn", nbytes=8.0 * n * (ra + rb) + 8.0 * ra * rb, flops=2.0 * n * ra * rb * frac):
                _ffi.check(lib.mf_trmm_nn_f64(_ptr(a), a.stride(0), n, ra, _ptr(w), w.stride(0), _ptr(out), out.stride(0), _stream()),
                           "mf_trmm_nn_f64")
        else:
            with _timed("gemm_nn", nbytes=16.0 * n * (ra + rb) + 16.0 * ra * rb, flops=8.0 * n * ra * rb * frac):
                _ffi.check(lib.mf_trmm_nn_c128(_ptr(a), a.stride(0), n, ra, _ptr(w), w.stride(0), _ptr(out), out.stride(0), _stream()),
                           "mf_trmm_nn_c128")
        return out
    if real:
        with _timed("gemm_nn", nbytes=8.0 * n * (ra + rb) + 8.0 * ra * rb, flops=2.0 * n * ra * rb):
            _ffi.check(lib.mf_gemm_nn_f64(_ptr(a), a.stride(0), n, ra, _ptr(w), w.stride(0), rb, _ptr(out), out.stride(0), _stream()),
                       "mf_gemm_nn_f64")
        return out
    with _timed("gemm_nn", nbytes=16.0 * n * (ra + rb) + 16.0 * ra * rb, flops=8.0 * n * ra * rb):
        _ffi.check(lib.mf_gemm_nn_c128(_ptr(a), a.stride(0), n, ra, _ptr(w), w.stride(0), rb, _ptr(out), out.stride(0), _stream()),
                   "mf_gemm_nn_c128")
    return out


def symmetrize(a: torch.Tensor) -> torch.Tensor:
    lib = _ffi.load()
    _check_mat(a, "a")
    r = a.shape[0]
    if a.dtype == F64:
        return ((a + a.T) * 0.5).contiguous()
    out = torch.empty((r, r), dtype=C128, device=a.device)
    _ffi.check(lib.mf_symmetrize_c128(_ptr(a), a.stride(0), r, _ptr(out), out.stride(0), _stream()), "mf_symmetrize_c128")
    return out


@dataclass
class DeviceCSR:
    rowptr: torch.Tensor
    colidx: torch.Tensor
    vals: torch.Tensor
    nrows: int
    ncols: int
    row0: int = 0
    grouped: Optional[tuple] = None
    sorted_indices: bool = False
    pattern_id: Optional[int] = None

    @property
    def nnz(self) -> int:
        return int(self.colidx.numel())

    @property
    def is_real(self) -> bool:
        return self.vals.dtype == torch.float64


transfer_bytes = {"h2d": 0, "d2h": 0}


def upload(arr: np.ndarray, device) -> torch.Tensor:
    t = torch.from_numpy(arr)
    transfer_bytes["h2d"] += t.numel() * t.element_size()
    return t.to(device, non_blocking=True)


def download(t: torch.Tensor, out: Optional[torch.Tensor] = None) -> np.ndarray:
    transfer_bytes["d2h"] += t.numel() * t.element_size()
    if out is not None:
        out.copy_(t, non_blocking=False)
        return out.numpy()
    return t.cpu().numpy()


def csr_of_transpose(a_csc, device=None, row_range=None, col_offset: int = 0, group_for_r: Optional[int] = None) -> DeviceCSR:
    import scipy.sparse as sp
    device = device or require_cuda()
    a = a_csc if sp.issparse(a_csc) and a_csc.format == "csc" else sp.csc_array(a_csc)
    n_rows_t = a.shape[1]
    lo, hi = (0, n_rows_t) if row_range is None else row_range
    indptr = np.asarray(a.indptr)
    s, e = int(indptr[lo]), int(indptr[hi])
    if e - s >= 2 ** 31 or a.shape[0] >= 2 ** 31:
        raise ValueError("operator too large for int32 indices")
    if lo == 0 and indptr.dtype == np.int32:
        rowptr = indptr[:hi + 1]
    else:
        rowptr = (indptr[lo:hi + 1] - indptr[lo]).astype(np.int32)
    colidx = np.ascontiguousarray(a.indices[s:e], dtype=np.int32)
    data = np.asarray(a.data[s:e])
    vals = np.ascontiguousarray(data, dtype=np.complex128 if np.iscomplexobj(data) else np.float64)
    if col_offset:
        colidx = colidx - np.int32(col_offset)
    csr = DeviceCSR(upload(np.ascontiguousarray(rowptr), device), upload(colidx, device), upload(vals, device),
                    hi - lo, a.shape[0], lo, None, bool(a.has_sorted_indices))
    if group_for_r is not None:
        group_rows(csr, group_for_r)
    return csr


def _group_size(r: int, real: bool) -> int:
    lib = _ffi.load()
    return int(lib.mf_spmm_group_size_f64(r) if real else lib.mf_spmm_group_size(r))


def group_rows(a: DeviceCSR, r: int, real: bool = False) -> None:
    lib = _ffi.load()
    g = _group_size(r, real)
    if not a.is_real or not a.sorted_indices or a.nrows == 0 or (a.grouped is not None and a.grouped[0] == g):
        return
    dev = a.colidx.device
    ngroups = (a.nrows + g - 1) // g
    counts = torch.empty(ngroups, dtype=torch.int32, device=dev)
    _ffi.check(lib.mf_spmm_group_count(_ptr(a.rowptr), _ptr(a.colidx), a.nrows, g, _ptr(counts), _stream()), "mf_spmm_group_count")
    ustart = torch.zeros(ngroups + 1, dtype=torch.int64, device=dev)
    torch.cumsum(counts, 0, out=ustart[1:])
    total = a.nnz
    ucols = torch.empty(total, dtype=torch.int32, device=dev)
    uvals = torch.empty(total * g, dtype=torch.float64, device=dev)
    _ffi.check(lib.mf_spmm_group_fill(_ptr(a.rowptr), _ptr(a.colidx), _ptr(a.vals), a.nrows, g, _ptr(ustart), _ptr(ucols), _ptr(uvals),
                                      _stream()), "mf_spmm_group_fill")
    a.grouped = (g, ustart, ucols, uvals)


def spmm(a: DeviceCSR, q: torch.Tensor, out: Optional[torch.Tensor] = None, col_offset: int = 0) -> torch.Tensor:
    lib = _ffi.load()
    _check_mat(q, "q")
    r = q.shape[1]
    real = q.dtype == F64
    if real and not a.is_real:
        raise ValueError("spmm: a real float64 Q needs a real operator (convert Q to complex128 for complex operators)")
    if out is None:
        out = torch.empty((a.nrows, r), dtype=q.dtype, device=q.device)
    w = 8.0 if real else 16.0
    if a.grouped is not None and col_offset == 0 and a.grouped[0] == _group_size(r, real):
        g, ustart, ucols, uvals = a.grouped
        nunion = (int(ustart[-1].item()) if timer is not None else 0)
        if real:
            nbytes = nunion * (4.0 + 8.0 * g) + 8.0 * ustart.numel() + w * r * (a.nrows + q.shape[0])
            with _timed("spmm_csr", nbytes=nbytes, flops=2.0 * a.nnz * r):
                _ffi.check(lib.mf_spmm_grouped_f64(_ptr(ustart), _ptr(ucols), _ptr(uvals), a.nrows, g, _ptr(q), q.stride(0), r,
                                                   _ptr(out), out.stride(0), _stream()), "mf_spmm_grouped_f64")
            return out
        nbytes = nunion * (4.0 + 8.0 * g) + 8.0 * ustart.numel() + 16.0 * r * (a.nrows + q.shape[0])
        with _timed("spmm_csr", nbytes=nbytes, flops=4.0 * a.nnz * r):
            _ffi.check(lib.mf_spmm_grouped_c128(_ptr(ustart), _ptr(ucols), _ptr(uvals), a.nrows, g, _ptr(q), q.stride(0), r,
                                                _ptr(out), out.stride(0), _stream()), "mf_spmm_grouped_c128")
        return out
    colidx = a.colidx if col_offset == 0 else a.colidx - col_offset
    if real:
        with _timed("spmm_csr", nbytes=a.nnz * 12.0 + 4.0 * (a.nrows + 1) + w * r * (a.nrows + q.shape[0]), flops=2.0 * a.nnz * r):
            _ffi.check(lib.mf_spmm_csr_f64(_ptr(a.rowptr), _ptr(colidx), _ptr(a.vals), a.nrows, _ptr(q), q.stride(0), r,
                                           _ptr(out), out.stride(0), _stream()), "mf_spmm_csr_f64")
        return out
    valb = 8.0 if a.is_real else 16.0
    with _timed("spmm_csr", nbytes=a.nnz * (valb + 4.0) + 4.0 * (a.nrows + 1) + 16.0 * r * (a.nrows + q.shape[0]),
                flops=(4.0 if a.is_real else 8.0) * a.nnz * r):
        _ffi.check(lib.mf_spmm_csr_c128(_ptr(a.rowptr), _ptr(colidx), _ptr(a.vals), int(a.is_real), a.nrows, _ptr(q), q.stride(0), r,
                                        _ptr(out), out.stride(0), _stream()), "mf_spmm_csr_c128")
    return out


@dataclass
class DeviceWindows:
    rowptr: torch.Tensor
    slot: torch.Tensor
    vals: torch.Tensor
    wstart: torch.Tensor
    ucol: torch.Tensor
    nrows: int
    wmax: int
    nnz: int


def build_windows(a_csc, device=None, row_range=None, col_offset: int = 0) -> Optional[DeviceWindows]:
    import scipy.sparse as sp
    lib = _ffi.load()
    device = device or require_cuda()
    a = a_csc if sp.issparse(a_csc) and a_csc.format == "csc" else sp.csc_array(a_csc)
    if np.iscomplexobj(a.data):
        return None
    rb = int(lib.mf_spmm_window_rows_per_block())
    lo, hi = (0, a.shape[1]) if row_range is None else row_range
    indptr = np.asarray(a.indptr)
    s, e = int(indptr[lo]), int(indptr[hi])
    rowptr = (indptr[lo:hi + 1] - indptr[lo]).astype(np.int64)
    cols = np.asarray(a.indices[s:e]).astype(np.int64) - col_offset
    nrows = hi - lo
    counts = np.diff(rowptr)
    if nrows == 0 or counts.max(initial=0) > int(lib.mf_spmm_window_max_nnz_per_row()):
        return None
    nblocks = (nrows + rb - 1) // rb
    blk = np.repeat(np.arange(nrows, dtype=np.int64) // rb, counts)
    ncols = int(a.shape[0])
    key = blk * ncols + cols
    ukey, inv = np.unique(key, return_inverse=True)
    ublk = ukey // ncols
    wstart = np.searchsorted(ublk, np.arange(nblocks + 1, dtype=np.int64)).astype(np.int64)
    wmax = int(np.diff(wstart).max(initial=0))
    if wmax > int(lib.mf_spmm_window_max_rows()):
        return None
    slot = (inv - wstart[blk]).astype(np.uint8)
    return DeviceWindows(upload(np.ascontiguousarray(rowptr.astype(np.int32)), device), upload(np.ascontiguousarray(slot), device),
                         upload(np.ascontiguousarray(a.data[s:e], dtype=np.float64), device),
                         upload(np.ascontiguousarray(wstart.astype(np.int32)), device),
                         upload(np.ascontiguousarray((ukey % ncols).astype(np.int32)), device), nrows, max(wmax, 1), int(e - s))


def spmm_window(a: DeviceWindows, q: torch.Tensor, out: Optional[torch.Tensor] = None) -> torch.Tensor:
    lib = _ffi.load()
    _check_mat(q, "q")
    r = q.shape[1]
    real = q.dtype == F64
    if out is None:
        out = torch.empty((a.nrows, r), dtype=q.dtype, device=q.device)
    w = 8.0 if real else 16.0
    fn = lib.mf_spmm_window_f64 if real else lib.mf_spmm_window_c128
    with _timed("spmm_window", nbytes=a.nnz * 9.0 + 4.0 * (a.nrows + 1) + 4.0 * a.ucol.numel() + w * r * (a.nrows + q.shape[0]),
                flops=(2.0 if real else 4.0) * a.nnz * r):
        _ffi.check(fn(_ptr(a.rowptr), _ptr(a.slot), _ptr(a.vals), _ptr(a.wstart), _ptr(a.ucol), a.nrows, a.wmax, _ptr(q), q.stride(0), r,
                      _ptr(out), out.stride(0), _stream()), "mf_spmm_window")
    return out


SPMM2_MAX_R = 128


def same_pattern(a: DeviceCSR, b: DeviceCSR) -> bool:
    return a is not b and a.pattern_id is not None and a.pattern_id == b.pattern_id


def mark_same_pattern(a: DeviceCSR, b: DeviceCSR, a_host, b_host, row_range=None) -> bool:
    if a is None or b is None or a.nrows != b.nrows or a.nnz != b.nnz or a.is_real != b.is_real:
        return False
    lo, hi = (0, a_host.shape[1]) if row_range is None else row_range
    pa, pb = np.asarray(a_host.indptr), np.asarray(b_host.indptr)
    if not np.array_equal(pa[lo:hi + 1], pb[lo:hi + 1]):
        return False
    s0, e0 = int(pa[lo]), int(pa[hi])
    if not np.array_equal(np.asarray(a_host.indices)[s0:e0], np.asarray(b_host.indices)[s0:e0]):
        return False
    a.pattern_id = b.pattern_id = id(a)
    return True


def spmm2(a0: DeviceCSR, a1: DeviceCSR, q: torch.Tensor, col_offset: int = 0):
    lib = _ffi.load()
    _check_mat(q, "q")
    if not same_pattern(a0, a1):
        raise ValueError("spmm2: the operands were not marked as sharing a sparsity pattern")
    r = q.shape[1]
    real = q.dtype == F64
    if real and not a0.is_real:
        raise ValueError("spmm2: a real float64 Q needs real operators")
    y0 = torch.empty((a0.nrows, r), dtype=q.dtype, device=q.device)
    y1 = torch.empty((a0.nrows, r), dtype=q.dtype, device=q.device)
    colidx = a0.colidx if col_offset == 0 else a0.colidx - col_offset
    w = 8.0 if real else 16.0
    valb = 8.0 if a0.is_real else 16.0
    nbytes = a0.nnz * (2 * valb + 4.0) + 4.0 * (a0.nrows + 1) + w * r * (2 * a0.nrows + q.shape[0])
    flops = 2 * (2.0 if real else (4.0 if a0.is_real else 8.0)) * a0.nnz * r
    with _timed("spmm_csr", nbytes=nbytes, flops=flops):
        if real:
            _ffi.check(lib.mf_spmm_csr2_f64(_ptr(a0.rowptr), _ptr(colidx), _ptr(a0.vals), _ptr(a1.vals), a0.nrows, _ptr(q), q.stride(0), r,
                                            _ptr(y0), y0.stride(0), _ptr(y1), y1.stride(0), _stream()), "mf_spmm_csr2_f64")
        else:
            _ffi.check(lib.mf_spmm_csr2_c128(_ptr(a0.rowptr), _ptr(colidx), _ptr(a0.vals), _ptr(a1.vals), int(a0.is_real), a0.nrows,
                                             _ptr(q), q.stride(0), r, _ptr(y0), y0.stride(0), _ptr(y1), y1.stride(0), _stream()),
                       "mf_spmm_csr2_c128")
    return y0, y1


@dataclass
class DeviceCSC:
    colptr: torch.Tensor
    rowidx: torch.Tensor
    vals: torch.Tensor
    nrows: int
    ncols: int

    @property
    def is_real(self) -> bool:
        return self.vals.dtype == torch.float64


def csc_to_device(b_csc, device=None) -> DeviceCSC:
    import scipy.sparse as sp
    device = device or require_cuda()
    b = b_csc if sp.issparse(b_csc) and b_csc.format == "csc" else sp.csc_array(b_csc)
    data = np.asarray(b.data)
    vals = np.ascontiguousarray(data, dtype=np.complex128 if np.iscomplexobj(data) else np.float64)
    return DeviceCSC(upload(np.ascontiguousarray(b.indptr, dtype=np.int32), device),
                     upload(np.ascontiguousarray(b.indices, dtype=np.int32), device),
                     upload(vals, device), b.shape[0], b.shape[1])


def project_rhs(b: DeviceCSC, q: torch.Tensor, row0: int = 0, conj: bool = False) -> torch.Tensor:
    lib = _ffi.load()
    _check_mat(q, "q")
    r = q.shape[1]
    if q.dtype == F64:
        if not b.is_real:
            raise ValueError("project_rhs: a real float64 Q needs a real port matrix")
        out = torch.empty((r, b.ncols), dtype=F64, device=q.device)
        _ffi.check(lib.mf_project_rhs_f64(_ptr(b.colptr), _ptr(b.rowidx), _ptr(b.vals), b.ncols, _ptr(q), q.stride(0), r,
                                          row0, q.shape[0], _ptr(out), out.stride(0), _stream()), "mf_project_rhs_f64")
        return out
    out = torch.empty((r, b.ncols), dtype=C128, device=q.device)
    _ffi.check(lib.mf_project_rhs_c128(_ptr(b.colptr), _ptr(b.rowidx), _ptr(b.vals), int(b.is_real), b.ncols, _ptr(q), q.stride(0), r,
                                       row0, q.shape[0], int(conj), _ptr(out), out.stride(0), _stream()), "mf_project_rhs_c128")
    return out


def _allreduce(t: torch.Tensor, group) -> None:
    if group is None:
        return
    import torch.distributed as dist
    dist.all_reduce(torch.view_as_real(t) if t.is_complex() else t, op=dist.ReduceOp.SUM, group=group)


def _small_c128(t: torch.Tensor) -> torch.Tensor:
    return t if t.dtype == C128 else t.to(C128)


def _like_block(small: torch.Tensor, x: torch.Tensor) -> torch.Tensor:
    return small if x.dtype == C128 else small.real.contiguous()


class BasisInfo:

    def __init__(self, sigma, passes, shifts, jacobi_sweeps, kept):
        self._sigma = sigma
        self.passes = passes
        self.shifts = shifts
        self._sweeps = jacobi_sweeps
        self.kept = kept
        self.flags = None
        self.converged = True
        self.departure = None
        self.q_ready = None
        self.keepalive = None

    @property
    def sigma(self) -> np.ndarray:
        if isinstance(self._sigma, torch.Tensor):
            self._sigma = self._sigma.cpu().numpy()
        return self._sigma

    @property
    def jacobi_sweeps(self) -> int:
        if isinstance(self._sweeps, torch.Tensor):
            self._sweeps = int(self._sweeps.item())
        return self._sweeps



_SMALL_NB = 64


_FUSED_CHOL_MIN_R = 113


def _potrf_upper(g: torch.Tensor, info: torch.Tensor, want_inverse: bool = False) -> Optional[torch.Tensor]:
    lib = _ffi.load()
    r = g.shape[0]
    if r < _FUSED_CHOL_MIN_R:
        _ffi.check(lib.mf_potrf_upper_c128(_ptr(g), g.stride(0), r, _ptr(info), _stream()), "mf_potrf_upper_c128")
        return None
    rinv = torch.empty((r, r), dtype=C128, device=g.device)
    nbytes = lib.mf_chol_inv_ws_bytes(r)
    ws = workspaces.get("chol_inv", nbytes, g.device)
    _ffi.check(lib.mf_chol_inv_upper_c128(_ptr(g), g.stride(0), r, _ptr(rinv), rinv.stride(0), _ptr(info), _ptr(ws), nbytes, _stream()),
               "mf_chol_inv_upper_c128")
    return rinv if want_inverse else None


def _unequilibrate(g: torch.Tensor, d: torch.Tensor, rinv_eq: Optional[torch.Tensor]) -> torch.Tensor:
    lib = _ffi.load()
    r = g.shape[0]
    _ffi.check(lib.mf_scale_cols_c128(_ptr(g), g.stride(0), r, r, _ptr(d), -1, _stream()), "mf_scale_cols_c128")
    if rinv_eq is None:
        return _trtri_upper(g)
    _ffi.check(lib.mf_scale_rows_c128(_ptr(rinv_eq), rinv_eq.stride(0), r, r, _ptr(d), 1, _stream()), "mf_scale_rows_c128")
    return rinv_eq


def _trtri_upper(rm: torch.Tensor) -> torch.Tensor:
    lib = _ffi.load()
    r = rm.shape[0]
    out = torch.zeros((r, r), dtype=C128, device=rm.device)

    def rec(lo: int, hi: int) -> None:
        n = hi - lo
        if n <= 96:
            blk = rm[lo:hi, lo:hi]
            tgt = out[lo:hi, lo:hi]
            _ffi.check(lib.mf_trtri_upper_c128(_ptr(blk), rm.stride(0), n, _ptr(tgt), out.stride(0), _stream()), "mf_trtri_upper_c128")
            return
        mid = lo + (n // 2 + _SMALL_NB - 1) // _SMALL_NB * _SMALL_NB
        rec(lo, mid)
        rec(mid, hi)
        t = gemm_nn(out[lo:mid, lo:mid].contiguous(), rm[lo:mid, mid:hi].contiguous())
        out[lo:mid, mid:hi] = -gemm_nn(t, out[mid:hi, mid:hi].contiguous())

    if r <= 96:
        _ffi.check(lib.mf_trtri_upper_c128(_ptr(rm), rm.stride(0), r, _ptr(out), out.stride(0), _stream()), "mf_trtri_upper_c128")
    else:
        rec(0, r)
    return out

@dataclass
class CholQR:
    x: torch.Tensor
    r_tot: torch.Tensor
    rinv: torch.Tensor
    passes: int
    shifts: list
    flags: Optional[torch.Tensor] = None
    converged: bool = True
    departure: Optional[float] = None


def flags_ok(flags_host: torch.Tensor) -> bool:
    ok = True
    n = flags_host.shape[0]
    for p in range(n):
        ok = ok and int(flags_host[p, 16:20].view(torch.int32)[0]) == 0
    dep = float(flags_host[n - 1, :8].view(torch.float64)[0])
    return ok and dep < 0.1


def _cholesky_qr2_optimistic(s: torch.Tensor, group=None) -> CholQR:
    lib = _ffi.load()
    dev = s.device
    n_loc, r = s.shape
    d = torch.empty(r, dtype=torch.float64, device=dev)
    flags = torch.zeros((2, 32), dtype=torch.uint8, device=dev)
    x, r_tot, rinv = s, None, None
    for p in range(2):
        g = gemm_tn(x, x, conj=True)
        _allreduce(g, group)
        g = _small_c128(g)
        stats = flags[p, :16].view(torch.float64)
        info = flags[p, 16:20].view(torch.int32)
        _ffi.check(lib.mf_equilibrate_c128(_ptr(g), g.stride(0), r, 0.0, _ptr(d), _ptr(stats), _stream()), "mf_equilibrate_c128")
        rinv = _unequilibrate(g, d, _potrf_upper(g, info, want_inverse=True))
        r_tot = g if r_tot is None else gemm_nn(g, r_tot)
        if p == 0:
            x = gemm_nn(x, _like_block(rinv, x), w_upper=True)
    return CholQR(x, r_tot, rinv, 2, [0.0, 0.0], flags)


def cholesky_qr(s: torch.Tensor, group=None, max_passes: int = 6, optimistic: bool = False) -> CholQR:
    lib = _ffi.load()
    _check_mat(s, "s")
    if optimistic:
        return _cholesky_qr2_optimistic(s, group)
    dev = s.device
    n_loc, r = s.shape
    eps = np.finfo(np.float64).eps
    d = torch.empty(r, dtype=torch.float64, device=dev)
    flags = torch.zeros(32, dtype=torch.uint8, device=dev)
    stats = flags[:16].view(torch.float64)
    info = flags[16:20].view(torch.int32)
    x = s
    r_tot = None
    shifts = []
    bufs = [None, None]
    for p in range(max_passes):
        g = gemm_tn(x, x, conj=True)
        _allreduce(g, group)
        g = _small_c128(g)
        shift = 0.0
        while True:
            gw = g.clone()
            _ffi.check(lib.mf_equilibrate_c128(_ptr(gw), gw.stride(0), r, shift, _ptr(d), _ptr(stats), _stream()), "mf_equilibrate_c128")
            rinv_eq = _potrf_upper(gw, info, want_inverse=True)
            host_flags = flags.cpu()
            if int(host_flags[16:20].view(torch.int32)[0]) == 0:
                break
            shift = 64.0 * eps * r if shift == 0.0 else shift * 100.0
            if shift > 1e-2:
                raise _ffi.MorfemB200Error("orthonormalize: Cholesky breakdown persists (snapshot block numerically rank deficient "
                                           "beyond what shifted CholeskyQR can repair)")
        shifts.append(shift)
        departure = float(host_flags[:8].view(torch.float64)[0])
        rinv = _unequilibrate(gw, d, rinv_eq)
        r_tot = gw if r_tot is None else gemm_nn(gw, r_tot)
        converged = departure < 0.1 and shift == 0.0
        if converged or p == max_passes - 1:
            if not converged:
                import warnings
                warnings.warn(f"orthonormalize: the Cholesky-QR passes did not reach a near-orthonormal block after {max_passes} passes "
                              f"(departure {departure:.2e}, last shift {shift:.1e}); the basis may be less orthonormal than the reference's SVD "
                              "(snapshot block numerically rank deficient)", RuntimeWarning, stacklevel=3)
            return CholQR(x, r_tot, rinv, p + 1, shifts, None, converged, departure)
        tgt = p % 2
        if bufs[tgt] is None:
            bufs[tgt] = torch.empty((n_loc, r), dtype=s.dtype, device=dev)
        x = gemm_nn(x, _like_block(rinv, x), out=bufs[tgt], w_upper=True)
    raise AssertionError("unreachable")


def basis_rotation(cq: CholQR, truncation_tol: float = 0.0) -> tuple[torch.Tensor, BasisInfo]:
    lib = _ffi.load()
    r_tot = cq.r_tot
    dev = r_tot.device
    r = r_tot.shape[0]
    eps = np.finfo(np.float64).eps
    u = torch.empty((r, r), dtype=C128, device=dev)
    sigma = torch.empty(r, dtype=torch.float64, device=dev)
    sweeps = torch.zeros(1, dtype=torch.int32, device=dev)
    nbytes = lib.mf_jacobi_svd_ws_bytes(r)
    ws = workspaces.get("jacobi", nbytes, dev)
    if cq.x.dtype == F64 and lib.mf_jacobi_svd_f64_supported(r):
        r_real = r_tot.real.contiguous()
        u_real = torch.empty((r, r), dtype=F64, device=dev)
        with _timed("jacobi_svd"):
            _ffi.check(lib.mf_jacobi_svd_f64(_ptr(r_real), r_real.stride(0), r, _ptr(u_real), u_real.stride(0), _ptr(sigma), 40, 4.0 * eps,
                                             _ptr(sweeps), _stream()), "mf_jacobi_svd_f64")
        u = u_real.to(C128)
    else:
        r_work = r_tot.clone()
        with _timed("jacobi_svd"):
            _ffi.check(lib.mf_jacobi_svd_c128(_ptr(r_work), r_work.stride(0), r, _ptr(u), u.stride(0), _ptr(sigma), 40, 4.0 * eps,
                                              _ptr(sweeps), _ptr(ws), ws.numel(), _stream()), "mf_jacobi_svd_c128")
    keep = r
    if truncation_tol > 0.0:
        sig = sigma.cpu().numpy()
        if sig[0] > 0.0:
            keep = max(1, int(np.count_nonzero(sig > truncation_tol * sig[0])))
    w = gemm_nn(cq.rinv, u[:, :keep] if keep < r else u)
    info = BasisInfo(sigma, cq.passes, cq.shifts, sweeps, keep)
    info.converged, info.departure = cq.converged, cq.departure
    return w, info


def orthonormalize(s: torch.Tensor, truncation_tol: float = 0.0, group=None, n_global: Optional[int] = None,
                   max_passes: int = 6) -> tuple[torch.Tensor, BasisInfo]:
    cq = cholesky_qr(s, group=group, max_passes=max_passes)
    w, info = basis_rotation(cq, truncation_tol)
    q = gemm_nn(cq.x, _like_block(w, cq.x))
    return q, info


_side_streams = {}
_upload_streams = {}


def upload_stream(dev) -> "torch.cuda.Stream":
    st = _upload_streams.get(str(dev))
    if st is None:
        st = _upload_streams[str(dev)] = torch.cuda.Stream(device=dev)
    return st



def basis_and_projection(s: torch.Tensor, project_block, group=None, truncation_tol: float = 0.0, optimistic: bool = False,
                         defer_q: bool = False, want_q: bool = True):
    dev = s.device
    cq = cholesky_qr(s, group=group, optimistic=optimistic)
    main = torch.cuda.current_stream()
    side = _side_streams.get(str(dev))
    if side is None:
        side = _side_streams[str(dev)] = torch.cuda.Stream(device=dev)
    ev0 = torch.cuda.Event()
    ev0.record(main)
    g_list, bt = project_block(cq.x)
    side.wait_event(ev0)
    with torch.cuda.stream(side):
        w, info = basis_rotation(cq, truncation_tol)
        w = _like_block(w, cq.x)
        ev_w = torch.cuda.Event()
        ev_w.record(side)
        q = gemm_nn(cq.x, w) if want_q else None
        ev1 = torch.cuda.Event()
        ev1.record(side)
    main.wait_event(ev_w)
    if not torch.cuda.is_current_stream_capturing():
        for t in (w, q, info._sigma, info._sweeps):
            if isinstance(t, torch.Tensor):
                t.record_stream(main)
    reduced = [None if g is None else gemm_nn(gemm_tn(w, g, conj=False), w) for g in g_list]
    b_r = gemm_tn(w, bt, conj=False)
    info.flags = cq.flags
    info.q_ready = None
    info.keepalive = None
    if defer_q and want_q:
        info.q_ready = ev1
        info.keepalive = cq
    else:
        main.wait_event(ev1)
    return q, reduced, b_r, info


@dataclass
class SweepResult:
    x: Optional[torch.Tensor]
    gsm: Optional[torch.Tensor]
    info: torch.Tensor


def sweep(a0s: Optional[torch.Tensor], a1s: Optional[torch.Tensor], a2s: Optional[torch.Tensor], br: torch.Tensor,
          c0: torch.Tensor, c1: torch.Tensor, c2: torch.Tensor, cb: torch.Tensor, zscale: Optional[torch.Tensor],
          want_x: bool = True, want_gsm: bool = True, variant: int = 0,
          x_out: Optional[torch.Tensor] = None, gsm_out: Optional[torch.Tensor] = None) -> SweepResult:
    lib = _ffi.load()
    ops = [o for o in (a0s, a1s, a2s) if o is not None]
    if not ops:
        raise ValueError("sweep: all operators are None")
    for o in ops:
        _check_mat(o, "operator")
    _check_mat(br, "br")
    r, m = br.shape
    if all(o.dtype == F64 for o in ops) and br.dtype == F64:
        if variant in (0, 3, 5) and lib.mf_sweep_f64_variant_supported(r, m, variant):
            return _sweep_f64(lib, a0s, a1s, a2s, br, c0, c1, c2, cb, zscale, want_x, want_gsm, variant)
        a0s, a1s, a2s = (None if o is None else o.to(C128) for o in (a0s, a1s, a2s))
        br = br.to(C128)
        ops = [o for o in (a0s, a1s, a2s) if o is not None]
    elif any(o.dtype != C128 for o in ops) or br.dtype != C128:
        raise ValueError("sweep: operators and port matrix must share a dtype (all float64 or all complex128)")
    lda = ops[0].stride(0)
    if any(o.stride(0) != lda or o.shape != (r, r) for o in ops):
        raise ValueError("sweep: operators must share shape (r, r) and leading dimension")
    nf = int(c0.numel())
    dev = br.device
    for c in (c0, c1, c2, cb) + ((zscale,) if zscale is not None else ()):
        if c.dtype != torch.float64 or not c.is_cuda or c.numel() != nf or not c.is_contiguous():
            raise ValueError("sweep: coefficient arrays must be contiguous float64 CUDA tensors of equal length")
    x = (x_out if x_out is not None else torch.empty((nf, r, m), dtype=C128, device=dev)) if want_x else None
    gsm = (gsm_out if gsm_out is not None else torch.empty((nf, m, m), dtype=C128, device=dev)) if want_gsm else None
    info = torch.zeros(nf, dtype=torch.int32, device=dev)
    nbytes = lib.mf_sweep_ws_bytes(r, m, nf, variant)
    ws = workspaces.get("sweep", nbytes, dev)
    flops_pt = (8.0 / 3.0) * r ** 3 + 8.0 * r * r * m + 16.0 * r * r + 8.0 * r * m * m
    bytes_pt = 16.0 * m * m * (gsm is not None) + 16.0 * r * m * (x is not None) + 40.0 + 4.0
    with _timed("sweep_lu_gsm", nbytes=bytes_pt * nf, flops=flops_pt * nf):
        _ffi.check(lib.mf_sweep_lu_gsm_c128(_ptr(a0s), _ptr(a1s), _ptr(a2s), lda, _ptr(br), br.stride(0), r, m,
                                            _ptr(c0), _ptr(c1), _ptr(c2), _ptr(cb), _ptr(zscale), nf,
                                            _ptr(x), _ptr(gsm), _ptr(info), variant, _ptr(ws), ws.numel(), _stream()),
                   "mf_sweep_lu_gsm_c128")
    return SweepResult(x, gsm, info)


def _sweep_f64(lib, a0s, a1s, a2s, br, c0, c1, c2, cb, zscale, want_x, want_gsm, variant=0) -> SweepResult:
    ops = [o for o in (a0s, a1s, a2s) if o is not None]
    r, m = br.shape
    lda = ops[0].stride(0)
    if any(o.stride(0) != lda or o.shape != (r, r) for o in ops):
        raise ValueError("sweep: operators must share shape (r, r) and leading dimension")
    nf = int(c0.numel())
    dev = br.device
    x = torch.empty((nf, r, m), dtype=F64, device=dev) if want_x else None
    gsm_ = torch.empty((nf, m, m), dtype=C128, device=dev) if want_gsm else None
    info = torch.zeros(nf, dtype=torch.int32, device=dev)
    flops_pt = (2.0 / 3.0) * r ** 3 + 2.0 * r * r * m + 4.0 * r * r + 2.0 * r * m * m
    bytes_pt = 16.0 * m * m * (gsm_ is not None) + 8.0 * r * m * (x is not None) + 40.0 + 4.0
    nbytes = lib.mf_sweep_f64_ws_bytes(r, m, nf, variant)
    ws = workspaces.get("sweep", nbytes, dev)
    with _timed("sweep_lu_gsm", nbytes=bytes_pt * nf, flops=flops_pt * nf):
        _ffi.check(lib.mf_sweep_lu_gsm_f64(_ptr(a0s), _ptr(a1s), _ptr(a2s), lda, _ptr(br), br.stride(0), r, m,
                                           _ptr(c0), _ptr(c1), _ptr(c2), _ptr(cb), _ptr(zscale), nf, _ptr(x), _ptr(gsm_), _ptr(info),
                                           variant, _ptr(ws), ws.numel(), _stream()),
                   "mf_sweep_lu_gsm_f64")
    return SweepResult(x, gsm_, info)


def gsm(x: torch.Tensor, bmat: torch.Tensor, cb: torch.Tensor, zscale: torch.Tensor) -> torch.Tensor:
    lib = _ffi.load()
    nf, r, m = x.shape
    out = torch.empty((nf, m, m), dtype=C128, device=x.device)
    _ffi.check(lib.mf_gsm_c128(_ptr(x), _ptr(bmat), bmat.stride(0), r, m, _ptr(cb), _ptr(zscale), nf, _ptr(out), _stream()), "mf_gsm_c128")
    return out


def estimator(x: torch.Tensor, g_blocks, h_blocks, bb: Optional[torch.Tensor],
              c0: torch.Tensor, c1: torch.Tensor, c2: torch.Tensor, cb: torch.Tensor) -> torch.Tensor:
    lib = _ffi.load()
    nf, r, m = x.shape
    garr = (ctypes.c_void_p * 9)(*[None if g_blocks[a][b] is None else g_blocks[a][b].data_ptr() for a in range(3) for b in range(3)])
    harr = (ctypes.c_void_p * 3)(*[None if h is None else h.data_ptr() for h in h_blocks])
    err = torch.empty(nf, dtype=torch.float64, device=x.device)
    _ffi.check(lib.mf_estimator_c128(_ptr(x), r, m, nf, ctypes.cast(garr, ctypes.c_void_p), ctypes.cast(harr, ctypes.c_void_p), _ptr(bb),
                                     _ptr(c0), _ptr(c1), _ptr(c2), _ptr(cb), _ptr(err), _stream()), "mf_estimator_c128")
    return err
```

### morfem_b200/dist.py

```python
from __future__ import annotations

from dataclasses import dataclass, field
from typing import List, Optional, Tuple

import numpy as np
import torch
import torch.distributed as dist


def even_split(total: int, world: int, rank: int) -> Tuple[int, int]:
    if world <= 0 or not (0 <= rank < world):
        raise ValueError("even_split: need 0 <= rank < world")
    base, extra = divmod(int(total), world)
    lo = rank * base + min(rank, extra)
    return lo, lo + base + (1 if rank < extra else 0)


def owner_ranges(total: int, world: int) -> List[Tuple[int, int]]:
    return [even_split(total, world, r) for r in range(world)]


def column_window(indptr: np.ndarray, indices: np.ndarray, lo: int, hi: int, ncols: int) -> Tuple[int, int]:
    s, e = int(indptr[lo]), int(indptr[hi])
    w0, w1 = min(lo, ncols), min(hi, ncols)
    if e > s:
        cols = indices[s:e]
        w0, w1 = min(w0, int(cols.min())), max(w1, int(cols.max()) + 1)
    return w0, w1


@dataclass
class HaloPlan:
    rank: int
    world: int
    row0: int
    row1: int
    win0: int
    win1: int
    recv: List[Tuple[int, int, int]] = field(default_factory=list)
    send: List[Tuple[int, int, int]] = field(default_factory=list)

    @property
    def halo_rows(self) -> int:
        return sum(hi - lo for _, lo, hi in self.recv)


def build_halo_plan(rank: int, world: int, n_rows: int, windows: List[Tuple[int, int]]) -> HaloPlan:
    owned = owner_ranges(n_rows, world)
    row0, row1 = owned[rank]
    win0, win1 = windows[rank]
    plan = HaloPlan(rank, world, row0, row1, win0, win1)
    for p in range(world):
        if p == rank:
            continue
        lo, hi = max(win0, owned[p][0]), min(win1, owned[p][1])
        if hi > lo:
            plan.recv.append((p, lo, hi))
        lo, hi = max(windows[p][0], row0), min(windows[p][1], row1)
        if hi > lo:
            plan.send.append((p, lo, hi))
    return plan


def gather_windows(window: Tuple[int, int], group=None) -> List[Tuple[int, int]]:
    world = dist.get_world_size(group)
    out: List[Optional[Tuple[int, int]]] = [None] * world
    dist.all_gather_object(out, (int(window[0]), int(window[1])), group=group)
    return [tuple(w) for w in out]


def _as_real(t: torch.Tensor) -> torch.Tensor:
    return torch.view_as_real(t) if t.is_complex() else t


def allreduce_sum_(t: torch.Tensor, group=None) -> torch.Tensor:
    if dist.is_initialized() and dist.get_world_size(group) > 1:
        dist.all_reduce(_as_real(t), op=dist.ReduceOp.SUM, group=group)
    return t


def exchange_halo(q_local: torch.Tensor, plan: HaloPlan, out: Optional[torch.Tensor] = None, group=None) -> torch.Tensor:
    r = q_local.shape[1]
    nwin = plan.win1 - plan.win0
    if out is None or out.shape[0] < nwin or out.shape[1] != r or out.dtype != q_local.dtype or out.device != q_local.device:
        out = torch.empty((nwin, r), dtype=q_local.dtype, device=q_local.device)
    win = out[:nwin]
    win[plan.row0 - plan.win0:plan.row1 - plan.win0].copy_(q_local)
    ops = []
    for peer, lo, hi in plan.send:
        ops.append(dist.P2POp(dist.isend, _as_real(q_local[lo - plan.row0:hi - plan.row0]), peer, group=group))
    for peer, lo, hi in plan.recv:
        ops.append(dist.P2POp(dist.irecv, _as_real(win[lo - plan.win0:hi - plan.win0]), peer, group=group))
    if ops:
        for req in dist.batch_isend_irecv(ops):
            req.wait()
    return win


def slab_halo_rows(rank_windows: List[Tuple[int, int]], owned: List[Tuple[int, int]]) -> Optional[int]:
    world = len(owned)
    h = 0
    for p in range(world):
        (w0, w1), (r0, r1) = rank_windows[p], owned[p]
        h = max(h, r0 - w0, w1 - r1)
    if h == 0:
        return 0
    if any(hi - lo < h for lo, hi in owned):
        return None
    for p in range(world):
        w0, w1 = rank_windows[p]
        for q in range(world):
            if q == p:
                continue
            lo, hi = max(w0, owned[q][0]), min(w1, owned[q][1])
            if hi <= lo:
                continue
            in_top = hi <= owned[q][0] + h
            in_bottom = lo >= owned[q][1] - h
            if not (in_top or in_bottom):
                return None
    return h


def exchange_halo_slabs(q_local: torch.Tensor, plan: HaloPlan, h: int, owned: List[Tuple[int, int]],
                        out: Optional[torch.Tensor] = None, group=None) -> torch.Tensor:
    r = q_local.shape[1]
    nwin = plan.win1 - plan.win0
    if out is None or out.shape[0] < nwin or out.shape[1] != r or out.dtype != q_local.dtype or out.device != q_local.device:
        out = torch.empty((nwin, r), dtype=q_local.dtype, device=q_local.device)
    win = out[:nwin]
    win[plan.row0 - plan.win0:plan.row1 - plan.win0].copy_(q_local)
    if h == 0:
        return win
    slab = torch.empty((2 * h, r), dtype=q_local.dtype, device=q_local.device)
    slab[:h].copy_(q_local[:h])
    slab[h:].copy_(q_local[q_local.shape[0] - h:])
    gathered = torch.empty((plan.world * 2 * h, r), dtype=q_local.dtype, device=q_local.device)
    dist.all_gather_into_tensor(_as_real(gathered), _as_real(slab), group=group)
    for peer, lo, hi in plan.recv:
        p0, p1 = owned[peer]
        base = 2 * h * peer
        if hi <= p0 + h:
            src = gathered[base + lo - p0:base + hi - p0]
        else:
            src = gathered[base + h + lo - (p1 - h):base + h + hi - (p1 - h)]
        win[lo - plan.win0:hi - plan.win0].copy_(src)
    return win


def gather_points(local: torch.Tensor, f_total: int, group=None) -> torch.Tensor:
    if not dist.is_initialized() or dist.get_world_size(group) == 1:
        return local
    world = dist.get_world_size(group)
    counts = [hi - lo for lo, hi in owner_ranges(f_total, world)]
    cmax = max(counts)
    tail = tuple(local.shape[1:])
    padded = torch.zeros((cmax,) + tail, dtype=local.dtype, device=local.device)
    padded[:local.shape[0]].copy_(local)
    gathered = torch.empty((world * cmax,) + tail, dtype=local.dtype, device=local.device)
    dist.all_gather_into_tensor(_as_real(gathered), _as_real(padded), group=group)
    if all(c == cmax for c in counts):
        return gathered
    return torch.cat([gathered[p * cmax:p * cmax + counts[p]] for p in range(world)], dim=0)


class ShardedHotPath:

    def __init__(self, operators, b, n_rows: int, f_total: int, coeffs_global, group=None):
        from . import device as dv
        self.dv = dv
        self.group = group if group is not None else (dist.group.WORLD if dist.is_initialized() else None)
        self.rank = dist.get_rank(group) if dist.is_initialized() else 0
        self.world = dist.get_world_size(group) if dist.is_initialized() else 1
        self.dev = dv.require_cuda()
        self.n_rows = n_rows
        self.row0, self.row1 = even_split(n_rows, self.world, self.rank)
        self.f_total = f_total
        self.f0, self.f1 = even_split(f_total, self.world, self.rank)
        self.ops = []
        self.plans = []
        self._windows = {}
        for a in operators:
            if a is None or a.nnz == 0:
                self.ops.append(None)
                self.plans.append(None)
                continue
            window = column_window(np.asarray(a.indptr), np.asarray(a.indices), self.row0, self.row1, a.shape[0])
            windows = gather_windows(window, group) if self.world > 1 else [window]
            plan = build_halo_plan(self.rank, self.world, n_rows, windows)
            self._windows[id(plan)] = windows
            csr = dv.csr_of_transpose(a, self.dev, row_range=(self.row0, self.row1), col_offset=plan.win0)
            self.ops.append(csr)
            self.plans.append(plan)
        self.owned = owner_ranges(n_rows, self.world)
        self.halo_h = 0
        self.halo_mode = "none"
        if self.world > 1:
            hs = []
            for a, plan in zip(operators, self.plans):
                if plan is None:
                    continue
                hs.append(slab_halo_rows(self._windows[id(plan)], self.owned))
            if any(h is None for h in hs):
                self.halo_mode = "p2p"
            else:
                self.halo_h = max(hs) if hs else 0
                self.halo_mode = "allgather"
        live = [i for i, c in enumerate(self.ops) if c is not None]
        self.pair = None
        if len(live) == 2 and self.plans[live[0]].win0 == self.plans[live[1]].win0 and self.plans[live[0]].win1 == self.plans[live[1]].win1:
            i0, i1 = live
            if dv.mark_same_pattern(self.ops[i0], self.ops[i1], operators[i0], operators[i1], row_range=(self.row0, self.row1)):
                self.pair = (i0, i1)
        self.b = dv.csc_to_device(b, self.dev)
        self.coeffs = [dv.upload(np.ascontiguousarray(c[self.f0:self.f1], dtype=np.float64), self.dev) for c in coeffs_global]
        self._win = None
        self.stage_events = None
        self._graph = None
        self.launches_per_graph = 0
        self._pending = []


    @property
    def graph_capable(self) -> bool:
        return self.world == 1 or self.halo_mode == "allgather"

    def drop_graph(self) -> None:
        self._graph = None

    def _exchange(self, x: torch.Tensor, plan: HaloPlan, buf: Optional[torch.Tensor], group) -> torch.Tensor:
        if self.halo_mode == "allgather":
            return exchange_halo_slabs(x, plan, self.halo_h, self.owned, buf, group)
        return exchange_halo(x, plan, buf, group)

    def _mark(self, ev):
        if ev is not None:
            e = torch.cuda.Event(enable_timing=True)
            e.record()
            ev.append(e)

    def step_graph(self, s_local: torch.Tensor, want_x: bool = False, skip_sweep: bool = False):
        if not self.graph_capable:
            raise RuntimeError("step_graph: this rank's halo exchange needs point-to-point messages, which a CUDA graph cannot "
                               "capture; use step() / step_deferred()")
        gather = self.world > 1 and not skip_sweep
        key = (tuple(s_local.shape), s_local.dtype, bool(want_x), bool(skip_sweep))
        if self._graph is None or self._graph["key"] != key:
            static_s = s_local.clone()
            for _ in range(2):
                self.step(static_s, want_x=want_x, gather=gather, optimistic=True, skip_sweep=skip_sweep)
            torch.cuda.synchronize()
            if self.world > 1:
                dist.barrier(group=self.group)
                torch.cuda.synchronize()
            from . import _ffi
            graph = torch.cuda.CUDAGraph()
            launches0 = _ffi.launch_count()
            with torch.cuda.graph(graph, capture_error_mode="thread_local" if self.world > 1 else "global"):
                out = self.step(static_s, want_x=want_x, gather=gather, optimistic=True, skip_sweep=skip_sweep)
            self.launches_per_graph = _ffi.launch_count() - launches0
            self.dv.workspaces.pin_all()
            flags_host = torch.empty((2, 32), dtype=torch.uint8).pin_memory()
            self._graph = {"key": key, "graph": graph, "s": static_s, "out": out, "flags_host": flags_host, "want_x": want_x}
        gr = self._graph
        if s_local.data_ptr() != gr["s"].data_ptr():
            gr["s"].copy_(s_local)
        gr["graph"].replay()
        gr["flags_host"].copy_(gr["out"][4].flags, non_blocking=True)
        return gr["out"][:4]

    def step_deferred(self, s_local: torch.Tensor, want_x: bool = False, gather: bool = True):
        out = self.step(s_local, want_x=want_x, gather=gather, optimistic=True)
        self._pending.append(out[4].flags)
        return out[:4]

    def verify_deferred(self) -> bool:
        ok = all(self.dv.flags_ok(f.cpu()) for f in self._pending)
        self._pending = []
        return ok

    def verify(self):
        gr = self._graph
        if gr is None:
            return None
        torch.cuda.current_stream().synchronize()
        if self.dv.flags_ok(gr["flags_host"]):
            return None
        return self.step(gr["s"], want_x=gr["want_x"], gather=self.world > 1)

    def step(self, s_local: torch.Tensor, want_x: bool = False, gather: bool = True, optimistic: bool = False, skip_sweep: bool = False):
        dv = self.dv
        group = self.group if self.world > 1 else None
        ev = [] if self.stage_events is not None else None
        self._mark(ev)
        def project_block(x):
            r = x.shape[1]
            m = self.b.ncols
            live = [i for i, csr in enumerate(self.ops) if csr is not None]
            nlive = len(live)
            flat = torch.empty(nlive * r * r + r * m, dtype=x.dtype, device=x.device)
            g_list = [None] * len(self.ops)
            windows = {}
            if self.pair is not None and r <= dv.SPMM2_MAX_R:
                i0, i1 = self.pair
                plan = self.plans[i0]
                xin = x
                if self.world > 1:
                    self._win = self._exchange(x, plan, self._win, group)
                    xin = self._win[:plan.win1 - plan.win0]
                y0, y1 = dv.spmm2(self.ops[i0], self.ops[i1], xin)
                for k, (i, y) in enumerate(((i0, y0), (i1, y1))):
                    g_list[i] = dv.gemm_tn(y, x, conj=False, out=flat[k * r * r:(k + 1) * r * r].view(r, r))
                live = []
            for k, i in enumerate(live):
                csr, plan = self.ops[i], self.plans[i]
                dv.group_rows(csr, r, real=x.dtype == torch.float64)
                if self.world > 1:
                    key = (plan.win0, plan.win1, tuple(plan.send), tuple(plan.recv))
                    if key not in windows:
                        windows[key] = self._exchange(x, plan, self._win if not windows else None, group)
                        if len(windows) == 1:
                            self._win = windows[key]
                    y = dv.spmm(csr, windows[key][:plan.win1 - plan.win0])
                else:
                    y = dv.spmm(csr, x)
                g_list[i] = dv.gemm_tn(y, x, conj=False, out=flat[k * r * r:(k + 1) * r * r].view(r, r))
            bt = flat[nlive * r * r:].view(r, m)
            bt.copy_(dv.project_rhs(self.b, x, self.row0, conj=False))
            allreduce_sum_(flat, group)
            return g_list, bt

        q, reduced, b_r, info = dv.basis_and_projection(s_local, project_block, group=group, optimistic=optimistic, defer_q=True)
        sym = [None if o is None else dv.symmetrize(o) for o in reduced]
        c0, c1, c2, cb, zs = self.coeffs

        def join_q():
            if info.q_ready is not None:
                torch.cuda.current_stream().wait_event(info.q_ready)
                info.q_ready = None
            info.keepalive = None

        if skip_sweep:
            join_q()
            self._mark(ev)
            out = (None, q, (reduced[0], reduced[1], reduced[2], b_r), None)
            return out + (info,) if optimistic else out
        self._mark(ev)
        res = dv.sweep(sym[0], sym[1], sym[2], b_r, c0, c1, c2, cb, zs, want_x=want_x, want_gsm=True)
        join_q()
        self._mark(ev)
        gsm = gather_points(res.gsm, self.f_total, group) if (gather and self.world > 1) else res.gsm
        self._mark(ev)
        if ev is not None:
            self.stage_events.append(ev)
        if optimistic:
            return gsm, q, (reduced[0], reduced[1], reduced[2], b_r), res, info
        return gsm, q, (reduced[0], reduced[1], reduced[2], b_r), res
```

### morfem_b200/implementation.py

```python
from __future__ import annotations

import math
import time
import warnings
from typing import Callable, Optional

import numpy as np
from scipy.sparse import csc_array, issparse

from . import full_order

ERROR_THRESHOLD = 1e-6
USE_EQUALLY_DISTRIBUTED = False
EQUALLY_DISTRIBUTED_REDUCTION_RATE = 0.97
PLOT_GREEDY_ITERATIONS = False
USE_OPM = False
TRUNCATION_TOL = 0.0
VERBOSE = False
FULL_ORDER_THREADS = None


class ModelDefinition:

    def __init__(self, domain, a0, a1, a2, b, t_a0: Callable, t_a1: Callable, t_a2: Callable, t_b: Callable):
        self.domain = domain
        self.a0 = a0
        self.a1 = a1
        self.a2 = a2
        self.b = b
        self.t_a0 = t_a0
        self.t_a1 = t_a1
        self.t_a2 = t_a2
        self.t_b = t_b


def coefficient_array(fn: Callable, domain: np.ndarray) -> np.ndarray:
    domain = np.asarray(domain, dtype=np.float64)
    n = domain.size
    if n == 0:
        return np.zeros(0)
    try:
        with warnings.catch_warnings():
            warnings.simplefilter("ignore")
            vec = np.asarray(fn(domain), dtype=np.float64)
        if vec.shape == ():
            vec = np.full(n, float(vec))
        if vec.shape == (n,):
            probes = sorted({0, n // 2, n - 1})
            eps = np.finfo(np.float64).eps
            if all(abs(float(fn(float(domain[i]))) - vec[i]) <= 2 * eps * abs(vec[i]) for i in probes):
                return np.ascontiguousarray(vec)
    except (TypeError, ValueError):
        pass
    return np.array([float(fn(float(t))) for t in domain], dtype=np.float64)


def _is_zero_operator(a) -> bool:
    if a is None:
        return True
    if issparse(a):
        return a.nnz == 0
    return not np.any(a)


def h(array):
    if array.ndim != 2:
        raise Exception("array has to be two-dimensional")
    return array.conj().T


def system_matrix(t: float, md: ModelDefinition):
    a = md.t_a0(t) * md.a0 + md.t_a1(t) * md.a1 + md.t_a2(t) * md.a2
    return (a + a.T) / 2


def impulse_vector(t: float, md: ModelDefinition):
    b = md.t_b(t) * md.b
    return b.todense() if issparse(b) else b


def _real_inputs(*arrs) -> bool:
    return not any(np.iscomplexobj(a.data if issparse(a) else a) for a in arrs if a is not None)


def _device_tensors(obj):
    import torch
    out = []
    for v in vars(obj).values():
        for t in (v if isinstance(v, tuple) else (v,)):
            if isinstance(t, torch.Tensor) and t.is_cuda:
                out.append(t)
    return out


class _DeviceOperators:

    def __init__(self, md: ModelDefinition, side_stream: bool = False, group_for_r: Optional[int] = None):
        from . import device as dv
        import torch
        self.dv = dv
        self.dev = dv.require_cuda()
        self.ops = [md.a0, md.a1, md.a2]
        self.zero = [_is_zero_operator(a) for a in self.ops]
        self.grouped = group_for_r is not None
        self._ready = {}
        stream = dv.upload_stream(self.dev) if side_stream else torch.cuda.current_stream()

        def mark(key):
            if side_stream:
                ev = torch.cuda.Event()
                ev.record(stream)
                self._ready[key] = ev

        with torch.cuda.stream(stream):
            self.b = dv.csc_to_device(md.b, self.dev)
            mark("b")
            self.at = []
            for i, (a, z) in enumerate(zip(self.ops, self.zero)):
                self.at.append(None if z else dv.csr_of_transpose(a, self.dev, group_for_r=group_for_r))
                if not z:
                    mark(i)
        self._a = [None, None, None]
        self.b_host = csc_array(md.b)
        self.pair = None
        live = [i for i, z in enumerate(self.zero) if not z]
        if self.grouped and len(live) == 2 and all(issparse(self.ops[i]) for i in live):
            i0, i1 = live
            if dv.mark_same_pattern(self.at[i0], self.at[i1], csc_array(self.ops[i0]), csc_array(self.ops[i1])):
                self.pair = (i0, i1)

    def wait_ready(self, key=None):
        import torch
        keys = list(self._ready) if key is None else ([key] if key in self._ready else [])
        cur = torch.cuda.current_stream()
        for k in keys:
            cur.wait_event(self._ready.pop(k))
            obj = self.b if k == "b" else self.at[k]
            for t in _device_tensors(obj):
                t.record_stream(cur)

    def a_csr(self, i):
        if self._a[i] is None and not self.zero[i]:
            a = self.ops[i]
            self._a[i] = self.dv.csr_of_transpose(csc_array(a.T if issparse(a) else np.asarray(a).T), self.dev)
        return self._a[i]

    def project_block(self, x):
        dv = self.dv
        if self.pair is not None and x.shape[1] <= dv.SPMM2_MAX_R:
            i0, i1 = self.pair
            self.wait_ready(i0)
            self.wait_ready(i1)
            y0, y1 = dv.spmm2(self.at[i0], self.at[i1], x)
            g_list = [None, None, None]
            g_list[i0] = dv.gemm_tn(y0, x, conj=False)
            g_list[i1] = dv.gemm_tn(y1, x, conj=False)
            self.wait_ready("b")
            return g_list, dv.project_rhs(self.b, x, 0, conj=False)
        g_list = []
        for i, (at, z) in enumerate(zip(self.at, self.zero)):
            if z:
                g_list.append(None)
                continue
            self.wait_ready(i)
            if self.grouped:
                dv.group_rows(at, x.shape[1], real=x.dtype == dv.F64)
            g_list.append(dv.gemm_tn(dv.spmm(at, x), x, conj=False))
        self.wait_ready("b")
        return g_list, dv.project_rhs(self.b, x, 0, conj=False)

    def project(self, q):
        dv = self.dv
        self.wait_ready()
        r = q.shape[1]
        out = []
        for at, z in zip(self.at, self.zero):
            if z:
                out.append(None)
                continue
            y = dv.spmm(at, q)
            out.append(dv.gemm_tn(y, q, conj=False))
        b_r = dv.project_rhs(self.b, q, 0, conj=False)
        return out[0], out[1], out[2], b_r


def _sweep_device(domain, ops_r, b_r, t_a0, t_a1, t_a2, t_b, want_x=True, want_gsm=False, variant=0):
    from . import device as dv
    import torch
    from scipy.constants import pi, epsilon_0
    dev = b_r.device
    domain = np.asarray(domain, dtype=np.float64)
    coeffs = [coefficient_array(f, domain) for f in (t_a0, t_a1, t_a2, t_b)]
    zs = 2 * pi * domain * epsilon_0
    c0, c1, c2, cb, zsd = (dv.upload(np.ascontiguousarray(c, dtype=np.float64), dev) for c in (*coeffs, zs))
    sym = [None if o is None else dv.symmetrize(o) for o in ops_r]
    return dv.sweep(sym[0], sym[1], sym[2], b_r, c0, c1, c2, cb, zsd, want_x=want_x, want_gsm=want_gsm, variant=variant)


def _warn_singular(info_host: np.ndarray):
    bad = np.nonzero(info_host)[0]
    if bad.size:
        from scipy.linalg import LinAlgWarning
        warnings.warn(f"Diagonal number {int(info_host[bad[0]])} is exactly zero. Singular matrix. "
                      f"(first of {bad.size} affected domain points: index {int(bad[0])})", LinAlgWarning, stacklevel=3)


def solve_fem_point(t: float, md: ModelDefinition):
    if issparse(md.a0) or issparse(md.a1) or issparse(md.a2):
        return full_order.solver_for(md).solve(t)
    one = ModelDefinition(np.array([t], dtype=np.float64), md.a0, md.a1, md.a2, md.b, md.t_a0, md.t_a1, md.t_a2, md.t_b)
    return solve_finite_element_method(one)[0]


def solve_finite_element_method(md: ModelDefinition):
    domain = np.asarray(md.domain)
    if issparse(md.a0) or issparse(md.a1) or issparse(md.a2):
        return full_order.solver_for(md).solve_many(domain, threads=FULL_ORDER_THREADS)
    from . import device as dv
    real = _real_inputs(md.a0, md.a1, md.a2, md.b)
    up = (lambda a: dv.real_or_complex_to_device(np.asarray(a))) if real else dv.to_device_c128
    ops = [None if _is_zero_operator(a) else up(a) for a in (md.a0, md.a1, md.a2)]
    b_r = up(md.b.toarray() if issparse(md.b) else md.b)
    res = _sweep_device(domain, ops, b_r, md.t_a0, md.t_a1, md.t_a2, md.t_b, want_x=True, want_gsm=False)
    x = res.x.cpu().numpy()
    _warn_singular(res.info.cpu().numpy())
    return np.ascontiguousarray(x.real) if real else x


def _block_to_device(arr, md: ModelDefinition):
    from . import device as dv
    real = _real_inputs(md.a0, md.a1, md.a2, md.b) and not np.iscomplexobj(arr)
    return dv.real_or_complex_to_device(np.asarray(arr), widen=not real)


def _orthonormal_basis_device(snapshots: np.ndarray, md: Optional[ModelDefinition] = None):
    from . import device as dv
    s = dv.to_device_c128(snapshots) if md is None else _block_to_device(snapshots, md)
    q, info = dv.orthonormalize(s, truncation_tol=TRUNCATION_TOL)
    return q, info


def projection_base_equally_distributed(md: ModelDefinition):
    reduction_indices = np.linspace(0, md.domain.size - 1,
                                    math.floor(md.domain.size * (1 - EQUALLY_DISTRIBUTED_REDUCTION_RATE)), dtype=int)
    vector_count = md.b.shape[1]
    if issparse(md.a0) or issparse(md.a1) or issparse(md.a2):
        x = full_order.solver_for(md).solve_many(md.domain[reduction_indices], threads=FULL_ORDER_THREADS)
        q = np.ascontiguousarray(x.transpose(1, 0, 2).reshape(md.b.shape[0], vector_count * reduction_indices.size))
    else:
        q = np.empty((md.b.shape[0], vector_count * reduction_indices.size))
        for i in range(reduction_indices.size):
            q[:, vector_count * i:vector_count * i + vector_count] = solve_fem_point(md.domain[reduction_indices[i]], md)
    qd, _ = _orthonormal_basis_device(q, md)
    return _basis_to_host(qd, md)


def _basis_to_host(qd, md) -> np.ndarray:
    q = qd.cpu().numpy()
    return np.ascontiguousarray(q.real) if _real_inputs(md.a0, md.a1, md.a2, md.b) else q


def error_estimator(md: ModelDefinition, q, opm=None, time_stats=None, _ops: Optional[_DeviceOperators] = None):
    from . import device as dv
    import torch
    ops = _ops or _DeviceOperators(md)
    qd = q if isinstance(q, torch.Tensor) else _block_to_device(q, md)
    c128 = lambda t: t if (t is None or t.is_complex()) else t.to(torch.complex128)
    ys = [None if ops.zero[i] else dv.spmm(ops.a_csr(i), qd) for i in range(3)]
    g = [[None if (ys[a] is None or ys[b] is None) else c128(dv.gemm_tn(ys[a], ys[b], conj=True)) for b in range(3)] for a in range(3)]
    hb = [None if y is None else c128(dv.project_rhs(ops.b, y, 0, conj=True)) for y in ys]
    bb = dv.to_device_c128((h(ops.b_host) @ ops.b_host).toarray())
    a0_r, a1_r, a2_r, b_r = ops.project(qd)
    res = _sweep_device(md.domain, [a0_r, a1_r, a2_r], b_r, md.t_a0, md.t_a1, md.t_a2, md.t_b, want_x=True, want_gsm=False)
    dom = np.asarray(md.domain, dtype=np.float64)
    c = [torch.from_numpy(coefficient_array(f, dom)).to(qd.device) for f in (md.t_a0, md.t_a1, md.t_a2, md.t_b)]
    err = dv.estimator(res.x if res.x.is_complex() else res.x.to(torch.complex128), g, hb, bb, c[0], c[1], c[2], c[3])
    return err.cpu().numpy()


class _GreedyState:

    def __init__(self, md: ModelDefinition, ops: "_DeviceOperators", first_block):
        from . import device as dv
        import torch
        self.dv, self.torch, self.md, self.ops = dv, torch, md, ops
        self.live = [i for i in range(3) if not ops.zero[i]]
        qd, _ = _orthonormal_basis_device(first_block, md)
        self.n, self.dtype, self.dev = qd.shape[0], qd.dtype, qd.device
        self.m = md.b.shape[1]
        self.cap, self.r = 0, 0
        self.q = None
        self.yt = {i: None for i in self.live}
        self.y = {i: None for i in self.live}
        self.a_r = {i: torch.zeros((0, 0), dtype=self.dtype, device=self.dev) for i in self.live}
        self.g = {(a, b): torch.zeros((0, 0), dtype=self.dtype, device=self.dev) for a in self.live for b in self.live}
        self.hb = {i: torch.zeros((0, self.m), dtype=self.dtype, device=self.dev) for i in self.live}
        self.b_r = torch.zeros((0, self.m), dtype=self.dtype, device=self.dev)
        self.bb = dv.to_device_c128((h(ops.b_host) @ ops.b_host).toarray())
        self._append_orthonormal(qd)

    def _reserve(self, cols: int):
        if cols <= self.cap:
            return
        torch = self.torch
        cap = max(cols, 2 * self.cap, 16)

        def grow(old):
            new = torch.empty((self.n, cap), dtype=self.dtype, device=self.dev)
            if old is not None and self.r:
                new[:, :self.r].copy_(old[:, :self.r])
            return new
        self.q = grow(self.q)
        for i in self.live:
            self.yt[i], self.y[i] = grow(self.yt[i]), grow(self.y[i])
        self.cap = cap

    def _append_orthonormal(self, v):
        dv, torch = self.dv, self.torch
        r, k = self.r, v.shape[1]
        self._reserve(r + k)
        self.q[:, r:r + k].copy_(v)
        v = self.q[:, r:r + k]
        q_old, q_all = self.q[:, :r], self.q[:, :r + k]
        for i in self.live:
            dv.spmm(self.ops.at[i], v.contiguous(), out=self.yt[i][:, r:r + k])
            dv.spmm(self.ops.a_csr(i), v.contiguous(), out=self.y[i][:, r:r + k])

        def grown(old, right, bottom_left):
            new = torch.empty((r + k, r + k), dtype=self.dtype, device=self.dev)
            new[:r, :r].copy_(old)
            new[:, r:].copy_(right)
            if r:
                new[r:, :r].copy_(bottom_left)
            return new
        vc = v.contiguous()
        for i in self.live:
            right = dv.gemm_tn(self.yt[i][:, :r + k], vc, conj=False)
            bl = dv.gemm_tn(self.yt[i][:, r:r + k].contiguous(), q_old, conj=False) if r else None
            self.a_r[i] = grown(self.a_r[i], right, bl)
        for a in self.live:
            for b in self.live:
                right = dv.gemm_tn(self.y[a][:, :r + k], self.y[b][:, r:r + k].contiguous(), conj=True)
                bl = dv.gemm_tn(self.y[a][:, r:r + k].contiguous(), self.y[b][:, :r], conj=True) if r else None
                self.g[(a, b)] = grown(self.g[(a, b)], right, bl)
            self.hb[a] = torch.cat((self.hb[a], dv.project_rhs(self.ops.b, self.y[a][:, r:r + k].contiguous(), 0, conj=True)), dim=0)
        self.b_r = torch.cat((self.b_r, dv.project_rhs(self.ops.b, vc, 0, conj=False)), dim=0)
        self.r = r + k

    def append(self, vectors):
        dv = self.dv
        v = _block_to_device(vectors, self.md)
        if v.dtype != self.dtype:
            raise _ffi_error("incremental greedy search: a complex solution joined a real basis (set USE_OPM = False for such models)")
        q_old = self.q[:, :self.r]
        for _ in range(2):
            c = dv.gemm_tn(q_old, v, conj=True)
            v = v - dv.gemm_nn(q_old, c)
        v, _ = dv.orthonormalize(v.contiguous(), truncation_tol=TRUNCATION_TOL)
        self._append_orthonormal(v)

    def error_estimator(self):
        dv, torch, md = self.dv, self.torch, self.md
        ops_r = [self.a_r.get(i) for i in range(3)]
        res = _sweep_device(md.domain, ops_r, self.b_r, md.t_a0, md.t_a1, md.t_a2, md.t_b, want_x=True, want_gsm=False)
        dom = np.asarray(md.domain, dtype=np.float64)
        c = [torch.from_numpy(coefficient_array(f, dom)).to(self.dev) for f in (md.t_a0, md.t_a1, md.t_a2, md.t_b)]
        c128 = lambda t: t if (t is None or t.is_complex()) else t.to(torch.complex128)
        g = [[c128(self.g[(a, b)].contiguous()) if (a in self.live and b in self.live) else None for b in range(3)] for a in range(3)]
        hb = [c128(self.hb[a].contiguous()) if a in self.live else None for a in range(3)]
        err = dv.estimator(res.x if res.x.is_complex() else res.x.to(torch.complex128), g, hb, self.bb, c[0], c[1], c[2], c[3])
        return err.cpu().numpy()

    def basis(self):
        return self.q[:, :self.r].contiguous()


def _ffi_error(msg):
    from ._ffi import MorfemB200Error
    return MorfemB200Error(msg)


def new_solution_for_projection_base(md: ModelDefinition, q, opm=None, time_stats=None, _ops=None):
    error = error_estimator(md, q, opm, time_stats, _ops=_ops)
    idx_max = error.argmax()
    if error[idx_max] < ERROR_THRESHOLD:
        return None, error
    return solve_fem_point(md.domain[idx_max], md), error


def projection_base(md: ModelDefinition, _return_device: bool = False, _ops: Optional[_DeviceOperators] = None):
    from . import device as dv
    ops = _ops or _DeviceOperators(md)
    if issparse(md.a0) or issparse(md.a1) or issparse(md.a2):
        ends = full_order.solver_for(md).solve_many(md.domain[[0, -1]], threads=FULL_ORDER_THREADS)
        initial_vectors = np.hstack((ends[0], ends[1]))
    else:
        initial_vectors = np.hstack((solve_fem_point(md.domain[0], md), solve_fem_point(md.domain[-1], md)))
    if USE_OPM:
        state = _GreedyState(md, ops, initial_vectors)
        projection_base.last_errors = []
        while True:
            error = state.error_estimator()
            projection_base.last_errors.append(error)
            idx_max = error.argmax()
            if error[idx_max] < ERROR_THRESHOLD:
                break
            state.append(solve_fem_point(md.domain[idx_max], md))
        qd = state.basis()
        return qd if _return_device else _basis_to_host(qd, md)
    qd, _ = _orthonormal_basis_device(initial_vectors, md)
    while True:
        q_new, _error = new_solution_for_projection_base(md, qd, _ops=ops)
        if q_new is None:
            break
        import torch
        new = _block_to_device(q_new, md)
        if new.dtype != qd.dtype:
            qd, new = qd.to(torch.complex128), new.to(torch.complex128)
        stacked = torch.cat((qd, new), dim=1).contiguous()
        qd, _ = dv.orthonormalize(stacked, truncation_tol=TRUNCATION_TOL)
    return qd if _return_device else _basis_to_host(qd, md)


class OfflinePhaseMatrices:
    qh_a0h_a0_q = qh_a0h_a1_q = qh_a0h_a2_q = qh_a0h_b = None
    qh_a1h_a0_q = qh_a1h_a1_q = qh_a1h_a2_q = qh_a1h_b = None
    qh_a2h_a0_q = qh_a2h_a1_q = qh_a2h_a2_q = qh_a2h_b = None
    bh_a0_q = bh_a1_q = bh_a2_q = bh_b = None


class TimeStatistics:
    times = {}

    def __init__(self):
        self.clock = time.time()

    def start_clock(self):
        self.clock = time.time()

    def add_time(self, name):
        now = time.time()
        self.times[name] = self.times.get(name, 0.0) + now - self.clock
        self.clock = now

    def add_custom_time(self, name, since):
        self.times[name] = self.times.get(name, 0.0) + time.time() - since

    def print_statistics(self):
        whole = self.times.get("Whole", sum(self.times.values())) or 1.0
        for name, t in self.times.items():
            print(f"{name}: {t:.3f} s ({100.0 * t / whole:.1f} %)")


def orthonormalize_vector_to_base(vector: np.ndarray, base: np.ndarray) -> np.ndarray:
    if vector.ndim != 1 or base.ndim != 2:
        raise Exception("vector has to be one-dimensional and base has to be two-dimensional")
    out = vector - base @ (base.T @ vector)
    return out / np.linalg.norm(out)


def orthonormalize_to_base(vectors: np.ndarray, base: np.ndarray) -> np.ndarray:
    if vectors.ndim != 2:
        raise Exception("new_vectors has to be two-dimensional")
    if base is not None and base.ndim != 2:
        raise Exception("base has to be two-dimensional or None")
    cols = []
    for i in range(vectors.shape[1]):
        col = orthonormalize_vector_to_base(vectors[:, i], base)
        base = np.hstack((base, col[:, None]))
        cols.append(col)
    return np.stack(cols, axis=1)


def expand_matrix(original: np.ndarray, old_q: np.ndarray, middle, new_part_q: np.ndarray):
    return np.block([[original, h(old_q) @ middle @ new_part_q],
                     [h(new_part_q) @ middle @ old_q, h(new_part_q) @ middle @ new_part_q]])


def residual_norm(md: ModelDefinition, q: np.ndarray) -> np.ndarray:
    ops = _DeviceOperators(md)
    qd = _block_to_device(q, md)
    a0_r, a1_r, a2_r, b_r = ops.project(qd)
    res = _sweep_device(md.domain, [a0_r, a1_r, a2_r], b_r, md.t_a0, md.t_a1, md.t_a2, md.t_b, want_x=True, want_gsm=False)
    x = res.x.cpu().numpy()
    out = np.empty(np.asarray(md.domain).size)
    for i, t in enumerate(np.asarray(md.domain)):
        out[i] = np.linalg.norm(system_matrix(t, md) @ (np.asarray(q) @ x[i]) - impulse_vector(t, md))
    return out


def morfem_from_snapshots(snapshots: np.ndarray, domain: np.ndarray, a0: csc_array, a1: csc_array, a2: csc_array, b: csc_array,
                          t_a0: Callable[[float], float] = lambda t: 1.,
                          t_a1: Callable[[float], float] = lambda t: t,
                          t_a2: Callable[[float], float] = lambda t: t ** 2,
                          t_b: Callable[[float], float] = lambda t: t):
    from . import device as dv
    md = ModelDefinition(domain, a0, a1, a2, b, t_a0, t_a1, t_a2, t_b)
    ops = _DeviceOperators(md)
    all_real = _real_inputs(a0, a1, a2, b) and not np.iscomplexobj(snapshots)
    qd, (a0_r, a1_r, a2_r), b_r, _ = dv.basis_and_projection(dv.real_or_complex_to_device(snapshots, widen=not all_real),
                                                             ops.project_block, truncation_tol=TRUNCATION_TOL)
    res = _sweep_device(domain, [a0_r, a1_r, a2_r], b_r, t_a0, t_a1, t_a2, t_b, want_x=True, want_gsm=False)
    _warn_singular(res.info.cpu().numpy())
    real = _real_inputs(a0, a1, a2, b) and not np.iscomplexobj(snapshots)
    r = qd.shape[1]

    def host(t):
        if t is None:
            return np.zeros((r, r)) if real else np.zeros((r, r), dtype=complex)
        arr = t.cpu().numpy()
        return np.ascontiguousarray(arr.real) if real else arr

    return host(res.x), host(qd), host(a0_r), host(a1_r), host(a2_r), host(b_r)


def morfem(domain: np.ndarray, a0: csc_array, a1: csc_array, a2: csc_array, b: csc_array,
           t_a0: Callable[[float], float] = lambda t: 1.,
           t_a1: Callable[[float], float] = lambda t: t,
           t_a2: Callable[[float], float] = lambda t: t ** 2,
           t_b: Callable[[float], float] = lambda t: t):
    from . import device as dv
    import torch
    md = ModelDefinition(domain, a0, a1, a2, b, t_a0, t_a1, t_a2, t_b)
    start = time.time()
    ops = _DeviceOperators(md)
    if USE_EQUALLY_DISTRIBUTED:
        qd = _block_to_device(projection_base_equally_distributed(md), md)
    else:
        qd = projection_base(md, _return_device=True, _ops=ops)
    if VERBOSE:
        print("Projection base: ", time.time() - start, " s")
    a0_r, a1_r, a2_r, b_r = ops.project(qd)
    res = _sweep_device(domain, [a0_r, a1_r, a2_r], b_r, t_a0, t_a1, t_a2, t_b, want_x=True, want_gsm=False)
    _warn_singular(res.info.cpu().numpy())
    real = _real_inputs(a0, a1, a2, b)
    r = qd.shape[1]

    def host(t):
        if t is None:
            return np.zeros((r, r)) if real else np.zeros((r, r), dtype=complex)
        arr = t.cpu().numpy()
        return np.ascontiguousarray(arr.real) if real else arr

    return host(res.x), host(qd), host(a0_r), host(a1_r), host(a2_r), host(b_r)
```

Baseline: 241,700.

## Exploit operator symmetry to compute only upper tiles of projected Gram products

Adds a GPU check that tells whether each sparse operator is exactly symmetric. When it is, the projection Q^T A Q is built by a new symmetric gemm_tn mode that computes only upper-triangular tiles and mirrors them elementwise in the reduction, with no conjugation. This roughly halves the tile work of the dense projection GEMMs. In exchange it adds a one-time symmetry-check kernel plus a host synchronisation when the flag is first read.

```diff
diff --git a/include/morfem_b200.h b/include/morfem_b200.h
--- a/include/morfem_b200.h
+++ b/include/morfem_b200.h
@@ -20,6 +20,8 @@
 size_t mf_gemm_tn_ws_bytes(int ra, int rb, int64_t n);
 int mf_gemm_tn_c128(const mf_c128* A, int64_t lda, int ra, const mf_c128* B, int64_t ldb, int rb, int64_t n,
                     int conj_a, mf_c128* C, int64_t ldc, void* ws, size_t ws_bytes, void* stream);
+int mf_gemm_tn_symm_c128(const mf_c128* A, int64_t lda, int ra, const mf_c128* B, int64_t ldb, int rb, int64_t n,
+                         mf_c128* C, int64_t ldc, void* ws, size_t ws_bytes, void* stream);
 
 int mf_gemm_nn_c128(const mf_c128* A, int64_t lda, int64_t n, int ra, const mf_c128* W, int64_t ldw, int rb,
                     mf_c128* Out, int64_t ldo, void* stream);
@@ -46,6 +48,9 @@
 int mf_spmm_csr2_f64(const int32_t* rowptr, const int32_t* colidx, const double* vals0, const double* vals1, int64_t nrows,
                      const double* Q, int64_t ldq, int r, double* Y0, int64_t ldy0, double* Y1, int64_t ldy1, void* stream);
 
+int mf_csr_symmetric(const int32_t* rowptr, const int32_t* colidx, const void* vals, int val_is_real, int64_t n,
+                     int32_t* asymmetric, void* stream);
+
 int mf_spmm_group_size(int r);
 int mf_spmm_group_size_f64(int r);
 int mf_spmm_group_count(const int32_t* rowptr, const int32_t* colidx, int64_t nrows, int G, int32_t* counts, void* stream);
@@ -69,6 +74,8 @@
 size_t mf_gemm_tn_f64_ws_bytes(int ra, int rb, int64_t n);
 int mf_gemm_tn_f64(const double* A, int64_t lda, int ra, const double* B, int64_t ldb, int rb, int64_t n,
                    double* C, int64_t ldc, void* ws, size_t ws_bytes, void* stream);
+int mf_gemm_tn_symm_f64(const double* A, int64_t lda, int ra, const double* B, int64_t ldb, int rb, int64_t n,
+                        double* C, int64_t ldc, void* ws, size_t ws_bytes, void* stream);
 int mf_gemm_nn_f64(const double* A, int64_t lda, int64_t n, int ra, const double* W, int64_t ldw, int rb,
                    double* Out, int64_t ldo, void* stream);
 int mf_trmm_nn_f64(const double* A, int64_t lda, int64_t n, int r, const double* W, int64_t ldw,
diff --git a/morfem_b200/_ffi.py b/morfem_b200/_ffi.py
--- a/morfem_b200/_ffi.py
+++ b/morfem_b200/_ffi.py
@@ -19,6 +19,8 @@
     "mf_gemm_tn_ws_bytes": (c_size_t, [c_int, c_int, c_int64]),
     "mf_gemm_tn_c128": (c_int, [c_void_p, c_int64, c_int, c_void_p, c_int64, c_int, c_int64, c_int, c_void_p, c_int64,
                                 c_void_p, c_size_t, c_void_p]),
+    "mf_gemm_tn_symm_c128": (c_int, [c_void_p, c_int64, c_int, c_void_p, c_int64, c_int, c_int64, c_void_p, c_int64,
+                                     c_void_p, c_size_t, c_void_p]),
     "mf_gemm_nn_c128": (c_int, [c_void_p, c_int64, c_int64, c_int, c_void_p, c_int64, c_int, c_void_p, c_int64, c_void_p]),
     "mf_trmm_nn_c128": (c_int, [c_void_p, c_int64, c_int64, c_int, c_void_p, c_int64, c_void_p, c_int64, c_void_p]),
     "mf_trmm_nn_f64": (c_int, [c_void_p, c_int64, c_int64, c_int, c_void_p, c_int64, c_void_p, c_int64, c_void_p]),
@@ -38,6 +40,7 @@
                                   c_void_p, c_int64, c_void_p]),
     "mf_spmm_csr2_f64": (c_int, [c_void_p, c_void_p, c_void_p, c_void_p, c_int64, c_void_p, c_int64, c_int, c_void_p, c_int64,
                                  c_void_p, c_int64, c_void_p]),
+    "mf_csr_symmetric": (c_int, [c_void_p, c_void_p, c_void_p, c_int, c_int64, c_void_p, c_void_p]),
     "mf_spmm_group_size": (c_int, [c_int]),
     "mf_spmm_group_size_f64": (c_int, [c_int]),
     "mf_spmm_group_count": (c_int, [c_void_p, c_void_p, c_int64, c_int, c_void_p, c_void_p]),
@@ -55,6 +58,8 @@
                                     c_int, c_void_p, c_int64, c_void_p]),
     "mf_gemm_tn_f64_ws_bytes": (c_size_t, [c_int, c_int, c_int64]),
     "mf_gemm_tn_f64": (c_int, [c_void_p, c_int64, c_int, c_void_p, c_int64, c_int, c_int64, c_void_p, c_int64, c_void_p, c_size_t, c_void_p]),
+    "mf_gemm_tn_symm_f64": (c_int, [c_void_p, c_int64, c_int, c_void_p, c_int64, c_int, c_int64, c_void_p, c_int64, c_void_p, c_size_t,
+                                    c_void_p]),
     "mf_gemm_nn_f64": (c_int, [c_void_p, c_int64, c_int64, c_int, c_void_p, c_int64, c_int, c_void_p, c_int64, c_void_p]),
     "mf_spmm_csr_f64": (c_int, [c_void_p, c_void_p, c_void_p, c_int64, c_void_p, c_int64, c_int, c_void_p, c_int64, c_void_p]),
     "mf_spmm_grouped_f64": (c_int, [c_void_p, c_void_p, c_void_p, c_int64, c_int, c_void_p, c_int64, c_int, c_void_p, c_int64, c_void_p]),
diff --git a/morfem_b200/csrc/dense_gemm.cu b/morfem_b200/csrc/dense_gemm.cu
--- a/morfem_b200/csrc/dense_gemm.cu
+++ b/morfem_b200/csrc/dense_gemm.cu
@@ -11,14 +11,14 @@
 
 __global__ void __launch_bounds__(TN_THREADS, 2)
 gemm_tn_kernel(const cplx* __restrict__ A, long long lda, int ra, const cplx* __restrict__ B, long long ldb, int rb,
-               long long n, long long rows_per_split, int conj_a, cplx* __restrict__ part, int herm) {
+               long long n, long long rows_per_split, int conj_a, cplx* __restrict__ part, int mirror_mode) {
     extern __shared__ __align__(16) cplx smem[];
     const int tid = threadIdx.x, lane = tid & 31, warp = tid >> 5;
     const int g = lane >> 2, t = lane & 3;
     const int wi = warp >> 1, wj = warp & 1;
     const int ntj = (rb + TN_TJ - 1) / TN_TJ;
     const int ti = blockIdx.x / ntj, tj = blockIdx.x - ti * ntj;
-    if (herm && ti > tj) return;
+    if (mirror_mode && ti > tj) return;
     const int i0 = ti * TN_TI, j0 = tj * TN_TJ;
     const long long n0 = (long long)blockIdx.y * rows_per_split;
     long long n1 = n0 + rows_per_split; if (n1 > n) n1 = n;
@@ -95,18 +95,20 @@
         }
 }
 
+enum { MIRROR_NONE = 0, MIRROR_HERM = 1, MIRROR_SYMM = 2 };
+
 constexpr int RED_WARPS = 8;
 __global__ void __launch_bounds__(RED_WARPS * 32)
-reduce_partials_kernel(const cplx* __restrict__ part, int nsplit, int ra, int rb, cplx* __restrict__ C, long long ldc, int herm) {
+reduce_partials_kernel(const cplx* __restrict__ part, int nsplit, int ra, int rb, cplx* __restrict__ C, long long ldc, int mirror_mode) {
     __shared__ cplx red[RED_WARPS][32];
     const int lane = threadIdx.x & 31, warp = threadIdx.x >> 5;
     const long long total = (long long)ra * rb;
     const long long oidx = (long long)blockIdx.x * 32 + lane;
     long long idx = oidx;
     bool mirror = false;
-    if (herm && oidx < total) {
+    if (mirror_mode && oidx < total) {
         const int i = (int)(oidx / rb), j = (int)(oidx - (long long)i * rb);
-        if (i / TN_TI > j / TN_TJ) { idx = (long long)j * rb + i; mirror = true; }
+        if (mirror_mode == MIRROR_SYMM ? i > j : i / TN_TI > j / TN_TJ) { idx = (long long)j * rb + i; mirror = true; }
     }
     cplx acc0 = cmake(0.0, 0.0), acc1 = cmake(0.0, 0.0);
     if (idx < total) {
@@ -123,7 +125,7 @@
         cplx acc = red[0][lane];
 #pragma unroll
         for (int w = 1; w < RED_WARPS; ++w) acc = cadd(acc, red[w][lane]);
-        if (mirror) acc.y = -acc.y;
+        if (mirror && mirror_mode == MIRROR_HERM) acc.y = -acc.y;
         const int i = (int)(oidx / rb), j = (int)(oidx - (long long)i * rb);
         C[i * ldc + j] = acc;
     }
@@ -244,6 +246,22 @@
     return sizeof(cplx) * (size_t)(nsplit > nsplit2 ? nsplit : nsplit2) * ra * rb;
 }
 
+static int gemm_tn_c128_launch(const mf_c128* A, int64_t lda, int ra, const mf_c128* B, int64_t ldb, int rb, int64_t n,
+                               int conj_a, mf_c128* C, int64_t ldc, void* ws, void* stream, int mirror_mode) {
+    cudaStream_t st = (cudaStream_t)stream;
+    int tiles, nsplit; long long rps;
+    tn_plan(ra, rb, n > 0 ? n : 1, tiles, nsplit, rps, mirror_mode != MIRROR_NONE);
+    const size_t smem = sizeof(cplx) * STAGES * TN_STAGE_ELEMS;
+    MF_CHECK_CUDA(cudaFuncSetAttribute(gemm_tn_kernel, cudaFuncAttributeMaxDynamicSharedMemorySize, (int)smem));
+    dim3 grid(tiles, nsplit);
+    gemm_tn_kernel<<<grid, TN_THREADS, smem, st>>>((const cplx*)A, lda, ra, (const cplx*)B, ldb, rb, n, rps, conj_a, (cplx*)ws, mirror_mode);
+    MF_CHECK_LAUNCH();
+    long long total = (long long)ra * rb;
+    reduce_partials_kernel<<<(unsigned)((total + 31) / 32), RED_WARPS * 32, 0, st>>>((const cplx*)ws, nsplit, ra, rb, (cplx*)C, ldc, mirror_mode);
+    MF_CHECK_LAUNCH();
+    return 0;
+}
+
 extern "C" int mf_gemm_tn_c128(const mf_c128* A, int64_t lda, int ra, const mf_c128* B, int64_t ldb, int rb, int64_t n,
                                int conj_a, mf_c128* C, int64_t ldc, void* ws, size_t ws_bytes, void* stream) {
     if (!A) MF_FAIL_ARG(1, "A is NULL");
@@ -253,19 +271,20 @@
     if (n < 0) MF_FAIL_ARG(7, "n < 0");
     if (!C || ldc < rb) MF_FAIL_ARG(9, "C is NULL or ldc < rb");
     if (!ws || ws_bytes < mf_gemm_tn_ws_bytes(ra, rb, n)) MF_FAIL_ARG(11, "workspace too small (mf_gemm_tn_ws_bytes)");
-    cudaStream_t st = (cudaStream_t)stream;
-    int tiles, nsplit; long long rps;
-    const int herm = (conj_a && (const void*)A == (const void*)B && lda == ldb && ra == rb) ? 1 : 0;
-    tn_plan(ra, rb, n > 0 ? n : 1, tiles, nsplit, rps, herm != 0);
-    const size_t smem = sizeof(cplx) * STAGES * TN_STAGE_ELEMS;
-    MF_CHECK_CUDA(cudaFuncSetAttribute(gemm_tn_kernel, cudaFuncAttributeMaxDynamicSharedMemorySize, (int)smem));
-    dim3 grid(tiles, nsplit);
-    gemm_tn_kernel<<<grid, TN_THREADS, smem, st>>>((const cplx*)A, lda, ra, (const cplx*)B, ldb, rb, n, rps, conj_a, (cplx*)ws, herm);
-    MF_CHECK_LAUNCH();
-    long long total = (long long)ra * rb;
-    reduce_partials_kernel<<<(unsigned)((total + 31) / 32), RED_WARPS * 32, 0, st>>>((const cplx*)ws, nsplit, ra, rb, (cplx*)C, ldc, herm);
-    MF_CHECK_LAUNCH();
-    return 0;
+    const int herm = (conj_a && (const void*)A == (const void*)B && lda == ldb && ra == rb) ? MIRROR_HERM : MIRROR_NONE;
+    return gemm_tn_c128_launch(A, lda, ra, B, ldb, rb, n, conj_a, C, ldc, ws, stream, herm);
+}
+
+extern "C" int mf_gemm_tn_symm_c128(const mf_c128* A, int64_t lda, int ra, const mf_c128* B, int64_t ldb, int rb, int64_t n,
+                                    mf_c128* C, int64_t ldc, void* ws, size_t ws_bytes, void* stream) {
+    if (!A) MF_FAIL_ARG(1, "A is NULL");
+    if (ra <= 0 || lda < ra) MF_FAIL_ARG(3, "need 0 < ra <= lda");
+    if (!B) MF_FAIL_ARG(4, "B is NULL");
+    if (rb != ra || ldb < rb) MF_FAIL_ARG(6, "need rb == ra and ldb >= rb");
+    if (n < 0) MF_FAIL_ARG(7, "n < 0");
+    if (!C || ldc < rb) MF_FAIL_ARG(8, "C is NULL or ldc < rb");
+    if (!ws || ws_bytes < mf_gemm_tn_ws_bytes(ra, rb, n)) MF_FAIL_ARG(10, "workspace too small (mf_gemm_tn_ws_bytes)");
+    return gemm_tn_c128_launch(A, lda, ra, B, ldb, rb, n, 0, C, ldc, ws, stream, MIRROR_SYMM);
 }
 
 static int gemm_nn_c128_impl(const mf_c128* A, int64_t lda, int64_t n, int ra, const mf_c128* W, int64_t ldw, int rb,
diff --git a/morfem_b200/csrc/dense_gemm_f64.cu b/morfem_b200/csrc/dense_gemm_f64.cu
--- a/morfem_b200/csrc/dense_gemm_f64.cu
+++ b/morfem_b200/csrc/dense_gemm_f64.cu
@@ -112,6 +112,7 @@
         }
 }
 
+enum { MIRROR_GRAM = 1, MIRROR_ELEMS = 2 };
 constexpr int RED_WARPS = 8;
 __global__ void __launch_bounds__(RED_WARPS * 32)
 reduce_partials_f64_kernel(const double* __restrict__ part, int nsplit, int ra, int rb, double* __restrict__ C, long long ldc, int symm) {
@@ -122,7 +123,7 @@
     long long idx = oidx;
     if (symm && oidx < total) {
         const int i = (int)(oidx / rb), j = (int)(oidx - (long long)i * rb);
-        if (i / TN_TI > j / TN_TJ) idx = (long long)j * rb + i;
+        if (symm == MIRROR_ELEMS ? i > j : i / TN_TI > j / TN_TJ) idx = (long long)j * rb + i;
     }
     double acc0 = 0.0, acc1 = 0.0;
     if (idx < total) {
@@ -244,18 +245,10 @@
     return sizeof(double) * (size_t)(nsplit > nsplit2 ? nsplit : nsplit2) * ra * rb;
 }
 
-extern "C" int mf_gemm_tn_f64(const double* A, int64_t lda, int ra, const double* B, int64_t ldb, int rb, int64_t n,
-                              double* C, int64_t ldc, void* ws, size_t ws_bytes, void* stream) {
-    if (!A) MF_FAIL_ARG(1, "A is NULL");
-    if (ra <= 0 || lda < ra) MF_FAIL_ARG(3, "need 0 < ra <= lda");
-    if (!B) MF_FAIL_ARG(4, "B is NULL");
-    if (rb <= 0 || ldb < rb) MF_FAIL_ARG(6, "need 0 < rb <= ldb");
-    if (n < 0) MF_FAIL_ARG(7, "n < 0");
-    if (!C || ldc < rb) MF_FAIL_ARG(8, "C is NULL or ldc < rb");
-    if (!ws || ws_bytes < mf_gemm_tn_f64_ws_bytes(ra, rb, n)) MF_FAIL_ARG(10, "workspace too small (mf_gemm_tn_f64_ws_bytes)");
+static int gemm_tn_f64_launch(const double* A, int64_t lda, int ra, const double* B, int64_t ldb, int rb, int64_t n,
+                              double* C, int64_t ldc, void* ws, void* stream, int symm) {
     cudaStream_t st = (cudaStream_t)stream;
     int tiles, nsplit; long long rps;
-    const int symm = (A == B && lda == ldb && ra == rb) ? 1 : 0;
     tn_plan(ra, rb, n > 0 ? n : 1, tiles, nsplit, rps, symm != 0);
     const size_t smem = sizeof(double) * STAGES * TN_STAGE_ELEMS;
     MF_CHECK_CUDA(cudaFuncSetAttribute(gemm_tn_f64_kernel, cudaFuncAttributeMaxDynamicSharedMemorySize, (int)smem));
@@ -268,6 +261,31 @@
     reduce_partials_f64_kernel<<<(unsigned)((total + 31) / 32), RED_WARPS * 32, 0, st>>>((const double*)ws, nsplit, ra, rb, C, ldc, symm);
     MF_CHECK_LAUNCH();
     return 0;
+}
+
+extern "C" int mf_gemm_tn_f64(const double* A, int64_t lda, int ra, const double* B, int64_t ldb, int rb, int64_t n,
+                              double* C, int64_t ldc, void* ws, size_t ws_bytes, void* stream) {
+    if (!A) MF_FAIL_ARG(1, "A is NULL");
+    if (ra <= 0 || lda < ra) MF_FAIL_ARG(3, "need 0 < ra <= lda");
+    if (!B) MF_FAIL_ARG(4, "B is NULL");
+    if (rb <= 0 || ldb < rb) MF_FAIL_ARG(6, "need 0 < rb <= ldb");
+    if (n < 0) MF_FAIL_ARG(7, "n < 0");
+    if (!C || ldc < rb) MF_FAIL_ARG(8, "C is NULL or ldc < rb");
+    if (!ws || ws_bytes < mf_gemm_tn_f64_ws_bytes(ra, rb, n)) MF_FAIL_ARG(10, "workspace too small (mf_gemm_tn_f64_ws_bytes)");
+    const int gram = (A == B && lda == ldb && ra == rb) ? MIRROR_GRAM : 0;
+    return gemm_tn_f64_launch(A, lda, ra, B, ldb, rb, n, C, ldc, ws, stream, gram);
+}
+
+extern "C" int mf_gemm_tn_symm_f64(const double* A, int64_t lda, int ra, const double* B, int64_t ldb, int rb, int64_t n,
+                                   double* C, int64_t ldc, void* ws, size_t ws_bytes, void* stream) {
+    if (!A) MF_FAIL_ARG(1, "A is NULL");
+    if (ra <= 0 || lda < ra) MF_FAIL_ARG(3, "need 0 < ra <= lda");
+    if (!B) MF_FAIL_ARG(4, "B is NULL");
+    if (rb != ra || ldb < rb) MF_FAIL_ARG(6, "need rb == ra and ldb >= rb");
+    if (n < 0) MF_FAIL_ARG(7, "n < 0");
+    if (!C || ldc < rb) MF_FAIL_ARG(8, "C is NULL or ldc < rb");
+    if (!ws || ws_bytes < mf_gemm_tn_f64_ws_bytes(ra, rb, n)) MF_FAIL_ARG(10, "workspace too small (mf_gemm_tn_f64_ws_bytes)");
+    return gemm_tn_f64_launch(A, lda, ra, B, ldb, rb, n, C, ldc, ws, stream, MIRROR_ELEMS);
 }
 
 static int gemm_nn_f64_impl(const double* A, int64_t lda, int64_t n, int ra, const double* W, int64_t ldw, int rb,
diff --git a/morfem_b200/csrc/sparse.cu b/morfem_b200/csrc/sparse.cu
--- a/morfem_b200/csrc/sparse.cu
+++ b/morfem_b200/csrc/sparse.cu
@@ -382,6 +382,26 @@
     }
 }
 
+__global__ void __launch_bounds__(256)
+csr_symmetric_kernel(const int* __restrict__ rowptr, const int* __restrict__ colidx, const unsigned long long* __restrict__ vals,
+                     int words, long long n, int* __restrict__ asym) {
+    const long long row = ((long long)blockIdx.x * blockDim.x + threadIdx.x) >> 5;
+    const int lane = threadIdx.x & 31;
+    if (row >= n) return;
+    const int s = rowptr[row], e = rowptr[row + 1];
+    bool bad = false;
+    for (int k = s + lane; k < e && !bad; k += 32) {
+        const int j = colidx[k];
+        if (j < 0 || j >= n || (k > s && colidx[k - 1] >= j)) { bad = true; break; }
+        const int je = rowptr[j + 1];
+        int lo = rowptr[j], hi = je;
+        while (lo < hi) { const int mid = (lo + hi) >> 1; if (colidx[mid] < row) lo = mid + 1; else hi = mid; }
+        if (lo == je || colidx[lo] != row) { bad = true; break; }
+        for (int w = 0; w < words; ++w) bad |= vals[(long long)k * words + w] != vals[(long long)lo * words + w];
+    }
+    if (__any_sync(0xffffffffu, bad) && lane == 0) *asym = 1;
+}
+
 }
 
 extern "C" int mf_spmm_csr_c128(const int32_t* rowptr, const int32_t* colidx, const void* vals, int val_is_real,
@@ -587,3 +607,19 @@
     MF_CHECK_LAUNCH();
     return 0;
 }
+
+extern "C" int mf_csr_symmetric(const int32_t* rowptr, const int32_t* colidx, const void* vals, int val_is_real, int64_t n,
+                                int32_t* asymmetric, void* stream) {
+    if (!rowptr) MF_FAIL_ARG(1, "rowptr is NULL");
+    if (!colidx) MF_FAIL_ARG(2, "colidx is NULL");
+    if (!vals) MF_FAIL_ARG(3, "vals is NULL");
+    if (n < 0 || n >= (1LL << 31)) MF_FAIL_ARG(5, "need 0 <= n < 2^31");
+    if (!asymmetric) MF_FAIL_ARG(6, "asymmetric is NULL");
+    cudaStream_t st = (cudaStream_t)stream;
+    MF_CHECK_CUDA(cudaMemsetAsync(asymmetric, 0, sizeof(int32_t), st));
+    if (n == 0) return 0;
+    csr_symmetric_kernel<<<(unsigned)((n * 32 + 255) / 256), 256, 0, st>>>(rowptr, colidx, (const unsigned long long*)vals,
+                                                                            val_is_real ? 1 : 2, n, asymmetric);
+    MF_CHECK_LAUNCH();
+    return 0;
+}
diff --git a/morfem_b200/device.py b/morfem_b200/device.py
--- a/morfem_b200/device.py
+++ b/morfem_b200/device.py
@@ -128,7 +128,8 @@
         return False
 
 
-def gemm_tn(a: torch.Tensor, b: torch.Tensor, conj: bool = False, out: Optional[torch.Tensor] = None) -> torch.Tensor:
+def gemm_tn(a: torch.Tensor, b: torch.Tensor, conj: bool = False, out: Optional[torch.Tensor] = None,
+            symmetric: bool = False) -> torch.Tensor:
     lib = _ffi.load()
     _check_mat(a, "a"); _check_mat(b, "b")
     real = _same_dtype(a, b, "gemm_tn")
@@ -136,18 +137,26 @@
     rb = b.shape[1]
     if b.shape[0] != n:
         raise ValueError("gemm_tn: row counts differ")
+    if symmetric and (conj or ra != rb):
+        raise ValueError("gemm_tn: the symmetric mode needs the plain transpose and a square result")
     if out is None:
         out = torch.empty((ra, rb), dtype=a.dtype, device=a.device)
     same = a.data_ptr() == b.data_ptr() and ra == rb
     if real:
         nbytes = lib.mf_gemm_tn_f64_ws_bytes(ra, rb, n)
         ws = workspaces.get("gemm_tn", nbytes, a.device)
+        fn, name = (lib.mf_gemm_tn_symm_f64, "mf_gemm_tn_symm_f64") if symmetric else (lib.mf_gemm_tn_f64, "mf_gemm_tn_f64")
         with _timed("gemm_tn", nbytes=8.0 * n * (ra if same else ra + rb) + 8.0 * ra * rb, flops=2.0 * n * ra * rb):
-            _ffi.check(lib.mf_gemm_tn_f64(_ptr(a), a.stride(0), ra, _ptr(b), b.stride(0), rb, n, _ptr(out), out.stride(0),
-                                          _ptr(ws), ws.numel(), _stream()), "mf_gemm_tn_f64")
+            _ffi.check(fn(_ptr(a), a.stride(0), ra, _ptr(b), b.stride(0), rb, n, _ptr(out), out.stride(0), _ptr(ws), ws.numel(), _stream()),
+                       name)
         return out
     nbytes = lib.mf_gemm_tn_ws_bytes(ra, rb, n)
     ws = workspaces.get("gemm_tn", nbytes, a.device)
+    if symmetric:
+        with _timed("gemm_tn", nbytes=16.0 * n * (ra + rb) + 16.0 * ra * rb, flops=8.0 * n * ra * rb):
+            _ffi.check(lib.mf_gemm_tn_symm_c128(_ptr(a), a.stride(0), ra, _ptr(b), b.stride(0), rb, n, _ptr(out), out.stride(0),
+                                                _ptr(ws), ws.numel(), _stream()), "mf_gemm_tn_symm_c128")
+        return out
     with _timed("gemm_tn", nbytes=16.0 * n * (ra if same else ra + rb) + 16.0 * ra * rb, flops=8.0 * n * ra * rb):
         _ffi.check(lib.mf_gemm_tn_c128(_ptr(a), a.stride(0), ra, _ptr(b), b.stride(0), rb, n, int(conj), _ptr(out), out.stride(0),
                                        _ptr(ws), ws.numel(), _stream()), "mf_gemm_tn_c128")
@@ -211,10 +220,19 @@
     grouped: Optional[tuple] = None
     sorted_indices: bool = False
     pattern_id: Optional[int] = None
+    symm_state: object = False
 
     @property
     def nnz(self) -> int:
         return int(self.colidx.numel())
+
+    @property
+    def symmetric(self) -> bool:
+        if isinstance(self.symm_state, tuple):
+            host, ev, _ = self.symm_state
+            ev.synchronize()
+            self.symm_state = int(host[0]) == 0
+        return bool(self.symm_state)
 
     @property
     def is_real(self) -> bool:
@@ -407,6 +425,31 @@
         return False
     a.pattern_id = b.pattern_id = id(a)
     return True
+
+
+def check_symmetric(a: DeviceCSR) -> None:
+    lib = _ffi.load()
+    if a.row0 != 0 or a.nrows != a.ncols:
+        raise ValueError("check_symmetric: needs the whole square operator, not a row slice")
+    flag = torch.empty(1, dtype=torch.int32, device=a.colidx.device)
+    _ffi.check(lib.mf_csr_symmetric(_ptr(a.rowptr), _ptr(a.colidx), _ptr(a.vals), int(a.is_real), a.nrows, _ptr(flag), _stream()),
+               "mf_csr_symmetric")
+    host = torch.empty(1, dtype=torch.int32).pin_memory()
+    host.copy_(flag, non_blocking=True)
+    ev = torch.cuda.Event()
+    ev.record()
+    a.symm_state = (host, ev, flag)
+
+
+def host_symmetric(a) -> bool:
+    import scipy.sparse as sp
+    a = a if sp.issparse(a) and a.format == "csc" else sp.csc_array(a)
+    if a.shape[0] != a.shape[1] or not a.has_canonical_format:
+        return False
+    t = a.T.tocsc()
+    bits = lambda d: np.ascontiguousarray(d, dtype=np.complex128 if np.iscomplexobj(d) else np.float64).view(np.uint64)
+    return (np.array_equal(a.indptr, t.indptr) and np.array_equal(a.indices, t.indices)
+            and np.array_equal(bits(a.data), bits(t.data)))
 
 
 def spmm2(a0: DeviceCSR, a1: DeviceCSR, q: torch.Tensor, col_offset: int = 0):
diff --git a/morfem_b200/dist.py b/morfem_b200/dist.py
--- a/morfem_b200/dist.py
+++ b/morfem_b200/dist.py
@@ -190,6 +190,11 @@
             plan = build_halo_plan(self.rank, self.world, n_rows, windows)
             self._windows[id(plan)] = windows
             csr = dv.csr_of_transpose(a, self.dev, row_range=(self.row0, self.row1), col_offset=plan.win0)
+            if self.world == 1:
+                dv.check_symmetric(csr)
+                csr.symm_state = csr.symmetric
+            else:
+                csr.symm_state = dv.host_symmetric(a)
             self.ops.append(csr)
             self.plans.append(plan)
         self.owned = owner_ranges(n_rows, self.world)
@@ -310,7 +315,7 @@
                     xin = self._win[:plan.win1 - plan.win0]
                 y0, y1 = dv.spmm2(self.ops[i0], self.ops[i1], xin)
                 for k, (i, y) in enumerate(((i0, y0), (i1, y1))):
-                    g_list[i] = dv.gemm_tn(y, x, conj=False, out=flat[k * r * r:(k + 1) * r * r].view(r, r))
+                    g_list[i] = dv.gemm_tn(y, x, conj=False, out=flat[k * r * r:(k + 1) * r * r].view(r, r), symmetric=self.ops[i].symmetric)
                 live = []
             for k, i in enumerate(live):
                 csr, plan = self.ops[i], self.plans[i]
@@ -324,7 +329,7 @@
                     y = dv.spmm(csr, windows[key][:plan.win1 - plan.win0])
                 else:
                     y = dv.spmm(csr, x)
-                g_list[i] = dv.gemm_tn(y, x, conj=False, out=flat[k * r * r:(k + 1) * r * r].view(r, r))
+                g_list[i] = dv.gemm_tn(y, x, conj=False, out=flat[k * r * r:(k + 1) * r * r].view(r, r), symmetric=csr.symmetric)
             bt = flat[nlive * r * r:].view(r, m)
             bt.copy_(dv.project_rhs(self.b, x, self.row0, conj=False))
             allreduce_sum_(flat, group)
diff --git a/morfem_b200/implementation.py b/morfem_b200/implementation.py
--- a/morfem_b200/implementation.py
+++ b/morfem_b200/implementation.py
@@ -119,6 +119,7 @@
             for i, (a, z) in enumerate(zip(self.ops, self.zero)):
                 self.at.append(None if z else dv.csr_of_transpose(a, self.dev, group_for_r=group_for_r))
                 if not z:
+                    dv.check_symmetric(self.at[i])
                     mark(i)
         self._a = [None, None, None]
         self.b_host = csc_array(md.b)
@@ -153,8 +154,8 @@
             self.wait_ready(i1)
             y0, y1 = dv.spmm2(self.at[i0], self.at[i1], x)
             g_list = [None, None, None]
-            g_list[i0] = dv.gemm_tn(y0, x, conj=False)
-            g_list[i1] = dv.gemm_tn(y1, x, conj=False)
+            g_list[i0] = dv.gemm_tn(y0, x, conj=False, symmetric=self.at[i0].symmetric)
+            g_list[i1] = dv.gemm_tn(y1, x, conj=False, symmetric=self.at[i1].symmetric)
             self.wait_ready("b")
             return g_list, dv.project_rhs(self.b, x, 0, conj=False)
         g_list = []
@@ -165,7 +166,7 @@
             self.wait_ready(i)
             if self.grouped:
                 dv.group_rows(at, x.shape[1], real=x.dtype == dv.F64)
-            g_list.append(dv.gemm_tn(dv.spmm(at, x), x, conj=False))
+            g_list.append(dv.gemm_tn(dv.spmm(at, x), x, conj=False, symmetric=at.symmetric))
         self.wait_ready("b")
         return g_list, dv.project_rhs(self.b, x, 0, conj=False)
 
@@ -179,7 +180,7 @@
                 out.append(None)
                 continue
             y = dv.spmm(at, q)
-            out.append(dv.gemm_tn(y, q, conj=False))
+            out.append(dv.gemm_tn(y, q, conj=False, symmetric=at.symmetric))
         b_r = dv.project_rhs(self.b, q, 0, conj=False)
         return out[0], out[1], out[2], b_r
 
```

After: 248,600 (median of 6 runs). 1.03x the previous value.
